# XuanHuang0/VANeRF

Measured on AMD Instinct MI355X. Metric: rendered rays/sec (64 samples/ray) + PSNR vs ref, 512x334 view, higher is better.
Workload: dtype bf16x3 (bf16 MFMA on hi+lo split operands, f32 accumulate; per-sample outputs within 3.3e-5 of the f32 kernel); 1 GPU; configs/vanerf.json eval view 512x334, 64 coarse + 64 importance samples/ray, two-hand mesh 1558 verts / 3108 faces, 1 source view 256x256, random trained-like weights; rays=171008, parallelism=single

## Files before the change

### vanerf_amd/csrc/api.cpp

```cpp
#include <algorithm>
#include <cstddef>

#include <cstring>

#include "common.h"

namespace vanerf {
static thread_local std::string g_last_error;
void set_last_error(const char* msg) { g_last_error = msg ? msg : ""; }
}

using namespace vanerf;

extern "C" int vanerf_abi_version(void) { return VANERF_ABI_VERSION; }

extern "C" const char* vanerf_last_error(void) { return g_last_error.c_str(); }

extern "C" int vanerf_weights_pack(const VanerfWeightTable* w, int mode, VanerfWeights** out)
{
    return guarded([&] {
        if (!w || !out) throw_error("vanerf_weights_pack: null argument");
        if (mode != 0 && mode != 1) throw_error("vanerf_weights_pack: mode %d not supported (0 = fp32 MFMA, 1 = split-bf16 x3)", mode);
        const float* const* ptrs = reinterpret_cast<const float* const*>(w);
        constexpr size_t n_ptrs = offsetof(VanerfWeightTable, sigmoid_beta) / sizeof(const float*);
        for (size_t i = 0; i < n_ptrs; ++i)
            if (!ptrs[i]) throw_error("vanerf_weights_pack: weight pointer #%d is null", (int)i);
        std::vector<float> host, host_bwd, host_h, eff;
        LayerOffsets offs{};
        pack_weights_host(*w, host, offs, mode, mode == 0 ? &host_bwd : nullptr, mode == 1 ? &host_h : nullptr, mode == 1 ? &eff : nullptr);
        auto* h = new VanerfWeights();
        h->n_floats_bwd = host_bwd.size();
        h->n_floats = host.size();
        h->n_floats_h = host_h.size();
        h->offs = offs;
        h->mode = mode;
        h->beta = w->sigmoid_beta < 2e-3f ? 2e-3f : w->sigmoid_beta;
        hipError_t e = hipGetDevice(&h->device);
        if (e == hipSuccess) e = hipMalloc(&h->dev, (host.size() + host_h.size()) * sizeof(float));
        if (e == hipSuccess) e = hipMemcpy(h->dev, host.data(), host.size() * sizeof(float), hipMemcpyHostToDevice);
        if (e == hipSuccess && !host_h.empty()) e = hipMemcpy(h->dev + host.size(), host_h.data(), host_h.size() * sizeof(float), hipMemcpyHostToDevice);
        if (e == hipSuccess && !eff.empty()) e = hipMalloc(&h->dev_eff, eff.size() * sizeof(float));
        if (e == hipSuccess && !eff.empty()) e = hipMemcpy(h->dev_eff, eff.data(), eff.size() * sizeof(float), hipMemcpyHostToDevice);
        if (e == hipSuccess && !host_bwd.empty()) e = hipMalloc(&h->dev_bwd, host_bwd.size() * sizeof(float));
        if (e == hipSuccess && !host_bwd.empty()) e = hipMemcpy(h->dev_bwd, host_bwd.data(), host_bwd.size() * sizeof(float), hipMemcpyHostToDevice);
        if (e == hipSuccess) e = hipMalloc(&h->stats, sizeof(unsigned long long));
        if (e == hipSuccess) e = hipMemset(h->stats, 0, sizeof(unsigned long long));
        if (e == hipSuccess) e = hipMalloc(&h->dev_beta, sizeof(float));
        if (e == hipSuccess) e = hipMemcpy(h->dev_beta, &h->beta, sizeof(float), hipMemcpyHostToDevice);
        if (e != hipSuccess) {
            if (h->dev) (void)hipFree(h->dev);
            if (h->dev_bwd) (void)hipFree(h->dev_bwd);
            if (h->stats) (void)hipFree(h->stats);
            if (h->dev_beta) (void)hipFree(h->dev_beta);
            if (h->dev_eff) (void)hipFree(h->dev_eff);
            delete h;
            hip_check(e, "vanerf_weights_pack: device upload");
        }
        *out = h;
    });
}

extern "C" int vanerf_weights_free(VanerfWeights* w)
{
    return guarded([&] {
        if (!w) return;
        if (w->dev) HIP_CHECK(hipFree(w->dev));
        if (w->dev_bwd) HIP_CHECK(hipFree(w->dev_bwd));
        if (w->stats) HIP_CHECK(hipFree(w->stats));
        if (w->dev_beta) HIP_CHECK(hipFree(w->dev_beta));
        if (w->dev_eff) HIP_CHECK(hipFree(w->dev_eff));
        delete w;
    });
}

extern "C" int vanerf_weights_pack_host(const VanerfWeightTable* w, float* out, int64_t cap, int64_t* n_out, unsigned* offsets)
{
    return guarded([&] {
        if (!w || !n_out) throw_error("vanerf_weights_pack_host: null argument");
        std::vector<float> host;
        LayerOffsets offs{};
        pack_weights_host(*w, host, offs);
        *n_out = (int64_t)host.size();
        if (offsets) std::copy_n(offs.off, (size_t)NUM_LAYERS, offsets);
        if (out) {
            if (cap < (int64_t)host.size()) throw_error("vanerf_weights_pack_host: buffer too small");
            std::copy(host.begin(), host.end(), out);
        }
    });
}

extern "C" int vanerf_weights_stream_host(const VanerfWeightTable* w, int which, float* out, int64_t cap, int64_t* n_out)
{
    return guarded([&] {
        if (!w || !n_out) throw_error("vanerf_weights_stream_host: null argument");
        if (which < 0 || which > 3) throw_error("vanerf_weights_stream_host: which = %d (0 fp32, 1 bf16x3, 2 backward, 3 hoisted bf16x3)", which);
        std::vector<float> host, bwd, hoisted;
        LayerOffsets offs{};
        pack_weights_host(*w, host, offs, which == 1 ? 1 : 0, which == 2 ? &bwd : nullptr, which == 3 ? &hoisted : nullptr);
        const std::vector<float>& src = which == 2 ? bwd : which == 3 ? hoisted : host;
        *n_out = (int64_t)src.size();
        if (out) {
            if (cap < (int64_t)src.size()) throw_error("vanerf_weights_stream_host: buffer too small");
            std::memcpy(out, src.data(), src.size() * sizeof(float));
        }
    });
}

extern "C" int vanerf_weights_download(const VanerfWeights* w, int which, float* out, int64_t cap, int64_t* n_out)
{
    return guarded([&] {
        if (!w || !n_out) throw_error("vanerf_weights_download: null argument");
        if (which != 0 && which != 2 && which != 3) throw_error("vanerf_weights_download: which = %d (0 forward, 2 backward, 3 hoisted bf16x3)", which);
        const float* src = which == 2 ? w->dev_bwd : which == 3 ? (w->n_floats_h ? w->dev + w->n_floats : nullptr) : w->dev;
        const size_t n = which == 2 ? w->n_floats_bwd : which == 3 ? w->n_floats_h : w->n_floats;
        if (!src) throw_error("vanerf_weights_download: the handle carries no such stream");
        *n_out = (int64_t)n;
        if (out) {
            if (cap < (int64_t)n) throw_error("vanerf_weights_download: buffer too small");
            HIP_CHECK(hipDeviceSynchronize());
            HIP_CHECK(hipMemcpy(out, src, n * sizeof(float), hipMemcpyDeviceToHost));
        }
    });
}

extern "C" int vanerf_weights_short_groups(const VanerfWeights* w, uint64_t* count)
{
    return guarded([&] {
        if (!w || !count) throw_error("vanerf_weights_short_groups: null argument");
        unsigned long long v = 0;
        HIP_CHECK(hipMemcpy(&v, w->stats, sizeof v, hipMemcpyDeviceToHost));
        *count = v;
    });
}
```

### vanerf_amd/csrc/common.h

```cpp
#pragma once
#include <hip/hip_runtime.h>

#include <atomic>
#include <cstdarg>
#include <cstdio>
#include <stdexcept>
#include <string>
#include <vector>

#include "../../include/vanerf_hip.h"
#include "layer_spec.h"

namespace vanerf {

struct Error : std::runtime_error {
    int code;
    Error(int c, const std::string& m) : std::runtime_error(m), code(c) {}
};

[[noreturn]] inline void throw_error(const char* fmt, ...)
{
    char buf[512];
    va_list ap;
    va_start(ap, fmt);
    vsnprintf(buf, sizeof buf, fmt, ap);
    va_end(ap);
    throw Error(VANERF_EINVAL, buf);
}

inline void hip_check(hipError_t e, const char* what)
{
    if (e != hipSuccess) {
        char buf[512];
        snprintf(buf, sizeof buf, "%s: %s", what, hipGetErrorString(e));
        throw Error(VANERF_EHIP, buf);
    }
}
#define HIP_CHECK(x) ::vanerf::hip_check((x), #x)

void set_last_error(const char* msg);

template <class F>
int guarded(F&& fn) noexcept
{
    try {
        fn();
        return VANERF_OK;
    } catch (const Error& e) {
        set_last_error(e.what());
        return e.code;
    } catch (const std::bad_alloc&) {
        set_last_error("out of host memory");
        return VANERF_ENOMEM;
    } catch (const std::exception& e) {
        set_last_error(e.what());
        return VANERF_EINVAL;
    } catch (...) {
        set_last_error("unknown error");
        return VANERF_EINVAL;
    }
}

void pack_weights_host(const VanerfWeightTable& w, std::vector<float>& out, LayerOffsets& offs, int mode = 0, std::vector<float>* bwd = nullptr,
                       std::vector<float>* hoisted = nullptr, std::vector<float>* eff_out = nullptr);
unsigned eff_layer_offset(int l);
struct LayerSrc {
    const float* w;
    const float* g;
    const float* b;
    int nout, kin;
    unsigned eff;
};
void layer_sources(const VanerfWeightTable& w, LayerSrc out[NUM_LAYERS]);
struct PackTables {
    std::vector<int> fwd, bwd, fwd_b, fwd_bh;
    LayerOffsets offs{};
    unsigned n_eff = 0;
};
const PackTables& pack_tables();
int layer_slots(int layer, int* k_of_slot, int cap);

constexpr long long VIEWS_MAX_ITEMS = 0x7fffffffLL;
void check_camera_source(const char* who, const VanerfPassDesc& d);

}

struct VanerfWeights {
    float* dev = nullptr;
    size_t n_floats_h = 0;
    float* dev_bwd = nullptr;
    size_t n_floats_bwd = 0;
    size_t n_floats = 0;
    vanerf::LayerOffsets offs{};
    int mode = 0;
    float beta = 0.1f;
    float* dev_beta = nullptr;
    float* dev_eff = nullptr;
    int device = 0;
    unsigned long long* stats = nullptr;
};
```

### vanerf_amd/csrc/layer_spec.h

```cpp
#pragma once

namespace vanerf {

enum Layer {
    L_GEO_AT0_A = 0, L_GEO_AT0_B, L_GEO_ATED0_A, L_GEO_ATED0_B,
    L_GEO_AT1_A, L_GEO_AT1_B, L_GEO_ATED1_A, L_GEO_ATED1_B,
    L_MLP0, L_MLP1, L_MLP2, L_MLP3, L_HEAD0, L_HEAD1, L_HEAD2, L_IBR,
    L_TEX_AT_A, L_TEX_AT_B, L_TEX_A, L_TEX_B, NUM_LAYERS
};

constexpr int kNB[NUM_LAYERS] = {1, 1, 2, 2, 1, 1, 1, 1, 4, 4, 4, 2, 2, 2, 1, 1, 3, 1, 3, 1};
constexpr int kT[NUM_LAYERS] = {
    98, 6, 98, 32,
    14, 6, 14, 4,
    147 + 32 + 1,
    64 + 1,
    64 + 4 + 1,
    60 + 1,
    64 + 1, 32 + 1, 32 + 1,
    64 + 1,
    49, 48, 49, 48
};

constexpr int PE_KPT_PER_HALF = 21;
constexpr int PE_FEATS = 7;

struct LayerOffsets {
    unsigned off[NUM_LAYERS];
};

constexpr unsigned layer_floats(int l) { return (unsigned)kT[l] * 64u * (unsigned)kNB[l]; }

constexpr unsigned layer_offset(int l)
{
    unsigned o = 0;
    for (int i = 0; i < l; ++i) o += layer_floats(i);
    return o;
}

constexpr int kT_b(int l, bool hoist)
{
    if (hoist && (l == L_GEO_AT0_A || l == L_GEO_ATED0_A)) return 32 + 2;
    if (hoist && l == L_TEX_AT_A) return 6 + 12 + 2;
    return kT[l];
}
constexpr int steps_b(int l, bool hoist = false) { return (kT_b(l, hoist) + 7) / 8; }
constexpr unsigned layer_dwords_b(int l, bool hoist = false) { return (unsigned)steps_b(l, hoist) * (unsigned)kNB[l] * 2u * 64u * 4u; }
constexpr unsigned layer_offset_b(int l, bool hoist = false)
{
    unsigned o = 0;
    for (int i = 0; i < l; ++i) o += layer_dwords_b(i, hoist);
    return o;
}

constexpr unsigned VP_NV = 1558u;
constexpr unsigned VP_A0_ROW = 16u, VP_N0_ROW = 64u, VP_P_ROW = 96u;
constexpr unsigned VP_A0 = 0u, VP_N0 = VP_A0 + VP_NV * VP_A0_ROW, VP_T0 = VP_N0 + VP_NV * VP_N0_ROW, VP_P = VP_T0 + VP_NV * VP_N0_ROW;
constexpr unsigned VP_FLOATS = VP_P + VP_NV * VP_P_ROW;

constexpr int kNOUT[NUM_LAYERS] = {10, 3, 64, 64, 10, 3, 8, 8, 128, 128, 120, 64, 64, 64, 2, 24, 96, 6, 96, 3};
constexpr int x_row_base(int l) { int o = 0; for (int i = 0; i < l; ++i) o += 2 * kT[i]; return o; }
constexpr int y_row_base(int l) { int o = 0; for (int i = 0; i < l; ++i) o += kNOUT[i]; return o; }
constexpr int X_ROWS = x_row_base(NUM_LAYERS), Y_ROWS = y_row_base(NUM_LAYERS);
constexpr int kBT[NUM_LAYERS] = {6, 3, 32, 32, 6, 3, 4, 4, 64, 64, 60, 32, 32, 32, 2, 12, 48, 4, 48, 3};
constexpr int kBLO[NUM_LAYERS] = {0, 0, 0, 0, 0, 0, 0, 0, 9, 0, 0, 0, 0, 0, 0, 0, 0, 0, 0, 0};
constexpr int kBNB[NUM_LAYERS] = {6, 1, 6, 2, 1, 1, 1, 1, 3, 4, 5, 4, 4, 2, 2, 4, 3, 3, 3, 3};
constexpr int bwd_pass_blocks(int l, int p) { return kBNB[l] - 4 * p > 4 ? 4 : kBNB[l] - 4 * p; }
constexpr unsigned bwd_layer_floats(int l) { return (unsigned)kBT[l] * 64u * (unsigned)kBNB[l]; }
constexpr unsigned bwd_layer_offset(int l) { unsigned o = 0; for (int i = 0; i < l; ++i) o += bwd_layer_floats(i); return o; }
constexpr unsigned bwd_pass_offset(int l, int p) { return bwd_layer_offset(l) + (unsigned)kBT[l] * 64u * 4u * (unsigned)p; }
enum AuxRow {
    AUX_G0 = 0,
    AUX_G1 = 3,
    AUX_TEX = 6,
    AUX_PW = 10,
    AUX_XV = 11,
    AUX_LAT = 43,
    AUX_COUNT = 55
};
constexpr int AUX_ROWS = 2 * AUX_COUNT;
constexpr int IG_GEO0 = 0;
constexpr int IG_GEO1 = 3 * 64;
constexpr int IG_TEX = IG_GEO1 + 24;
constexpr int IG_TEX_XY = IG_TEX + 64;
constexpr int IG_ROWS = IG_TEX_XY + 8;

}
```

### vanerf_amd/csrc/query_kernel.hip

```cpp
#include <algorithm>
#include <utility>

#include "common.h"
#include "mfma_chain.h"

using namespace vanerf;
using namespace vanerf_chain;


namespace {

constexpr int WAVES_PER_SIMD = 2;
constexpr int WAVES_PER_SIMD_SPILL = 1;
template <int MODE> constexpr int WPB = MODE == 1 ? 8 : 4;


#ifdef VANERF_STAMPS
#define STAMP(k)                                                                                  \
    do {                                                                                          \
        unsigned long long t_;                                                                    \
        __builtin_amdgcn_sched_barrier(0);                                                        \
        asm volatile("s_memtime %0\n\ts_waitcnt lgkmcnt(0)" : "=s"(t_)::"memory");               \
        __builtin_amdgcn_sched_barrier(0);                                                        \
        phase_cycles[k] += t_ - t_prev;                                                           \
        t_prev = t_;                                                                              \
    } while (0)
constexpr int N_PHASES = 12;
#else
#define STAMP(k) do { } while (0)
#endif

struct QueryParams {
    VanerfFrame f;
    const float* w;
    unsigned wbytes;
    const float* pts;
    const float* qsdf;
    const uint8_t* qvis;
    const float* noise;
    const int32_t* knn_in;
    const int32_t* order;
    int raw;
    long long n;
    float* out;
    uint8_t* valid;
    unsigned long long* stamps;
    unsigned* queue;
    unsigned long long* short_groups;
    float wm1[4], hm1[4];
    const float* vp;
    float *xs, *aux;
    long long npad;
};

typedef __bf16 bf16x8 __attribute__((ext_vector_type(8)));
typedef __bf16 bf16x2 __attribute__((ext_vector_type(2)));

struct FragB { u32x4 hi, lo; };

constexpr int LDS_FIRST = L_IBR;
template <bool HOIST> constexpr unsigned RES_BASE_DW = layer_offset_b(LDS_FIRST, HOIST);
template <bool HOIST> constexpr unsigned RES_DW = layer_offset_b(NUM_LAYERS, HOIST) - layer_offset_b(LDS_FIRST, HOIST);
constexpr unsigned RING_PHASE_PIECES = 16u, RING_BYTES = 2u * RING_PHASE_PIECES * 1024u;
constexpr unsigned LDS_KPT = 0u, LDS_CTRL = 2u * PE_KPT_PER_HALF * 16u, LDS_LAT0 = 768u, LDS_RING = 1024u, LDS_RES = LDS_RING + RING_BYTES;
template <bool HOIST> constexpr unsigned DYN_LDS_BYTES = LDS_RES + RES_DW<HOIST> * 4u;
template <bool HOIST> constexpr unsigned RING_PIECES = RES_BASE_DW<HOIST> / 256u;
template <bool HOIST> constexpr unsigned RING_STREAM_PHASES = (RING_PIECES<HOIST> + RING_PHASE_PIECES - 1u) / RING_PHASE_PIECES;
template <bool HOIST> constexpr unsigned RING_PHASES = (RING_STREAM_PHASES<HOIST> + 1u) / 2u * 2u;
static_assert(WPB<1> == 8, "the ring's DMA schedule deals 2 pieces of a phase to each of 8 waves");
static_assert(RING_PHASES<false> * RING_PHASE_PIECES * 256u <= layer_offset_b(NUM_LAYERS), "the last phase's DMA must stay inside the stream");
static_assert(RING_PHASES<true> * RING_PHASE_PIECES * 256u <= layer_offset_b(NUM_LAYERS, true), "the last phase's DMA must stay inside the hoisted stream");
static_assert(LDS_CTRL + 8u + 2u * 4u * WPB<1> <= LDS_LAT0 && LDS_LAT0 + 128u <= LDS_RING, "control words / constant latent overlap their neighbours");
static_assert(DYN_LDS_BYTES<false> <= 160u * 1024u && DYN_LDS_BYTES<true> <= DYN_LDS_BYTES<false>, "key points + control words + ring + resident fragments must fit the CU's 160 KB");
extern __shared__ __attribute__((aligned(16))) u32x4 s_dyn[];
typedef __attribute__((address_space(3))) u32x4 lds_u32x4_t;
typedef __attribute__((address_space(3))) unsigned lds_u32_t;
struct LAddr {
    unsigned w[3];
    unsigned dma_lds, dma_src;
};
__device__ __forceinline__ LAddr make_laddr(int lane, unsigned wv_uniform = 0u)
{
    LAddr a;
    a.dma_lds = LDS_RING + wv_uniform * 2048u; a.dma_src = wv_uniform * 2048u;
    a.w[0] = (unsigned)lane * 16u;
    asm volatile("" : "+v"(a.w[0]));
    a.w[1] = a.w[0] + 0x10000u; a.w[2] = a.w[0] + 0x20000u;
    asm volatile("" : "+v"(a.w[1]), "+v"(a.w[2]));
    return a;
}
template <unsigned BYTE> __device__ __forceinline__ u32x4 lds_frag(const LAddr& a)
{
    return *reinterpret_cast<const lds_u32x4_t*>((size_t)(a.w[BYTE >> 16] + (BYTE & 0xffffu)));
}
__device__ __forceinline__ lds_u32_t* lds_ctrl() { return reinterpret_cast<lds_u32_t*>((size_t)LDS_CTRL); }
template <int NB> struct RingDepthB { static constexpr int value = NB == 1 ? 1 : 2; };
template <int NB> struct RingB { FragB b[RingDepthB<NB>::value]; };

template <unsigned P> __device__ __forceinline__ void ring_dma(WRsrc rs, const LAddr& la)
{
    constexpr unsigned lds_off = (P % 2u) * RING_PHASE_PIECES * 1024u, src_off = P * RING_PHASE_PIECES * 1024u;
    unsigned keep, soff;
    asm volatile("s_mov_b32 %0, m0\n\ts_add_u32 m0, %2, %4\n\ts_add_u32 %1, %3, %5\n\ts_nop 0\n\t"
                 "buffer_load_dwordx4 %6, %7, %1 offen lds\n\tbuffer_load_dwordx4 %6, %7, %1 offen offset:1024 lds\n\ts_mov_b32 m0, %0"
                 : "=&s"(keep), "=&s"(soff)
                 : "s"(la.dma_lds), "s"(la.dma_src), "i"(lds_off), "i"(src_off), "v"(la.w[0]), "s"(rs)
                 : "memory");
}
template <bool HOIST, unsigned P> __device__ __forceinline__ void phase_begin(WRsrc rs, const LAddr& la)
{
    constexpr unsigned RING_PHASES = ::RING_PHASES<HOIST>;
    if constexpr (P > 0) asm volatile("s_waitcnt vmcnt(0) lgkmcnt(0)\n\ts_barrier" ::: "memory");
    ring_dma<(P + 1u) % RING_PHASES>(rs, la);
}

template <bool HOIST> __device__ __forceinline__ void ring_close(WRsrc rs, const LAddr& la)
{
    if constexpr (RING_STREAM_PHASES<HOIST> % 2u == 1u) phase_begin<HOIST, RING_PHASES<HOIST> - 1u>(rs, la);
}

template <bool HOIST, bool RES, unsigned DW> __device__ __forceinline__ FragB wload_blk(WRsrc rs, const LAddr& la)
{
    constexpr unsigned RING_PHASES = ::RING_PHASES<HOIST>, RES_BASE_DW = ::RES_BASE_DW<HOIST>;
    static_assert(RES == (DW >= RES_BASE_DW), "a layer's fragments are either resident or streamed through the ring: nothing is fetched per wave");
    FragB r;
    if constexpr (RES) {
        r.hi = lds_frag<LDS_RES + (DW - RES_BASE_DW) * 4u>(la);
        r.lo = lds_frag<LDS_RES + (DW - RES_BASE_DW + 256u) * 4u>(la);
    } else {
        constexpr unsigned q = DW / 256u;
        static_assert(q % 2u == 0 && q + 1u < RING_PHASES * RING_PHASE_PIECES, "block fragments are two consecutive pieces inside the streamed part");
        if constexpr (q % RING_PHASE_PIECES == 0) phase_begin<HOIST, q / RING_PHASE_PIECES>(rs, la);
        r.hi = lds_frag<LDS_RING + (q % (2u * RING_PHASE_PIECES)) * 1024u>(la);
        r.lo = lds_frag<LDS_RING + ((q + 1u) % (2u * RING_PHASE_PIECES)) * 1024u>(la);
    }
    return r;
}

template <bool HOIST, int NB, int T, bool RES, unsigned SBASE_DW> __device__ __forceinline__ RingB<NB> ring_start_b(WRsrc rs, const LAddr& la)
{
    constexpr int D = RingDepthB<NB>::value, S = (T + 7) / 8;
    RingB<NB> r;
    static_for<D>([&](auto ic) {
        constexpr int i = decltype(ic)::value;
        if constexpr (i < S * NB) r.b[i] = wload_blk<HOIST, RES, SBASE_DW + i * 512u>(rs, la);
    });
    __builtin_amdgcn_sched_barrier(0x000F);
    return r;
}

__device__ __forceinline__ unsigned pack_bf16(float a, float b)
{
    const bf16x2 v = {(__bf16)a, (__bf16)b};
    return __builtin_bit_cast(unsigned, v);
}

struct NoPre { template <class C> __device__ __forceinline__ void operator()(C) const {} };

template <bool HOIST, int NB, int T, bool RES, unsigned SBASE_DW, class Op, class Pre = NoPre>
__device__ __forceinline__ void run_layer_b(f32x16 (&acc)[NB], RingB<NB>& ring, WRsrc rs, const LAddr& la, Op&& operand,
                                            Pre&& pre = Pre{})
{
    constexpr int D = RingDepthB<NB>::value, S = (T + 7) / 8;
    constexpr int NCH = 4;
    auto split_pair = [&](auto sc, auto ic, u32x4& bh, u32x4& bl) {
        constexpr int s = decltype(sc)::value, i = decltype(ic)::value, t0 = 8 * s + 2 * i;
        float x0 = 0.0f, x1 = 0.0f;
        if constexpr (t0 < T) x0 = operand(std::integral_constant<int, t0>{});
        if constexpr (t0 + 1 < T) x1 = operand(std::integral_constant<int, t0 + 1>{});
        unsigned hpk = pack_bf16(x0, x1);
        asm("" : "+v"(hpk));
        bh[i] = hpk;
        bl[i] = pack_bf16(x0 - __uint_as_float(hpk << 16), x1 - __uint_as_float(hpk & 0xffff0000u));
    };
    u32x4 bh, bl;
    pre(std::integral_constant<int, 0>{});
    static_for<4>([&](auto ic) { split_pair(std::integral_constant<int, 0>{}, ic, bh, bl); });
    __builtin_amdgcn_sched_barrier(0);
    static_for<S>([&](auto sc) {
        constexpr int s = decltype(sc)::value;
        FragB a[NB];
        const bf16x8 xh = __builtin_bit_cast(bf16x8, bh), xl = __builtin_bit_cast(bf16x8, bl);
        u32x4 nh = {}, nl = {};
        static_for<NCH>([&](auto cc) {
            constexpr int c = decltype(cc)::value;
            static_for<3 * NB>([&](auto mc) {
                constexpr int m = decltype(mc)::value, ob = m / 3, pr = m % 3, idx = s * NB + ob;
                if constexpr (m * NCH / (3 * NB) == c) {
                    if constexpr (pr == 0) {
                        a[ob] = ring.b[idx % D];
                        if constexpr (idx + D < S * NB) ring.b[idx % D] = wload_blk<HOIST, RES, SBASE_DW + (idx + D) * 512u>(rs, la);
                    }
                    const bf16x8 wh = __builtin_bit_cast(bf16x8, a[ob].hi), wl = __builtin_bit_cast(bf16x8, a[ob].lo);
                    acc[ob] = __builtin_amdgcn_mfma_f32_32x32x16_bf16(pr == 2 ? wl : wh, pr == 1 ? xl : xh, acc[ob], 0, 0, 0);
                }
            });
            if constexpr (s + 1 < S) {
                if constexpr (c == 0) pre(std::integral_constant<int, s + 1>{});
                split_pair(std::integral_constant<int, s + 1>{}, cc, nh, nl);
            }
            __builtin_amdgcn_sched_barrier(0);
        });
        bh = nh; bl = nl;
    });
}

template <int MODE, int NB> struct RingSel { using type = Ring<NB>; };
template <int NB> struct RingSel<1, NB> { using type = RingB<NB>; };

struct LLane {
    int lane;
    WRsrc xs, aux;
    unsigned voff, row4;
    bool on;
};
constexpr unsigned SPILL_OFF = 0xfffffff0u;
template <int L, int t> __device__ __forceinline__ void spill_x(const LLane& la, float v)
{
    if (la.on) __builtin_amdgcn_raw_buffer_store_b32(__float_as_uint(v), la.xs, la.voff, (unsigned)(x_row_base(L) + 2 * t) * la.row4, 0);
}
template <int K> __device__ __forceinline__ void spill_aux(const LLane& la, float v)
{
    if (la.on) __builtin_amdgcn_raw_buffer_store_b32(__float_as_uint(v), la.aux, la.voff, (unsigned)(2 * K) * la.row4, 0);
}
template <int MODE> struct LaneSel { using type = LLane; };
template <> struct LaneSel<1> { using type = LAddr; };
__device__ __forceinline__ unsigned lane_of(const LLane& la) { return (unsigned)la.lane; }
template <int MODE, bool HOIST, int NB, int T, int L> __device__ __forceinline__ typename RingSel<MODE, NB>::type ring_start_m(WRsrc rs, const typename LaneSel<MODE>::type& la)
{
    if constexpr (MODE == 0) return ring_start<NB, T>(rs, layer_offset(L), lane_of(la) * NB * 4u);
    else return ring_start_b<HOIST, NB, T, (L >= LDS_FIRST), layer_offset_b(L, HOIST)>(rs, la);
}

template <int MODE, bool HOIST, int NB, int T, int L, class Op>
__device__ __forceinline__ void run_layer_m(f32x16 (&acc)[NB], typename RingSel<MODE, NB>::type& ring, WRsrc rs, const typename LaneSel<MODE>::type& la, Op&& operand)
{
    if constexpr (MODE == 0)
        run_layer<NB, T>(acc, ring, rs, layer_offset(L), lane_of(la) * NB * 4u, [&](auto tc) -> float {
            const float b = operand(tc);
            spill_x<L, decltype(tc)::value>(la, b);
            return b;
        });
    else run_layer_b<HOIST, NB, T, (L >= LDS_FIRST), layer_offset_b(L, HOIST)>(acc, ring, rs, la, static_cast<Op&&>(operand));
}

__device__ __forceinline__ int lane_id_fresh()
{
    int l;
    asm volatile("v_mbcnt_lo_u32_b32 %0, -1, 0\n\tv_mbcnt_hi_u32_b32 %0, -1, %0" : "=v"(l));
    return l;
}


__device__ __forceinline__ void block_barrier_lds() { asm volatile("s_waitcnt lgkmcnt(0)\n\ts_barrier" ::: "memory"); }

__device__ __forceinline__ float sigmoid_f(float x) { return __builtin_amdgcn_rcpf(1.0f + __builtin_amdgcn_exp2f(x * -1.44269504f)); }

__device__ __forceinline__ float relu_f(float x) { return __builtin_amdgcn_fmed3f(x, 0.0f, 3.0e38f); }

__device__ __forceinline__ float softplus100(float x)
{
    const float e = __builtin_amdgcn_exp2f(fabsf(x) * -144.269504f);
    return fmaf(__builtin_amdgcn_logf(1.0f + e), 6.93147181e-3f, relu_f(x));
}

template <int NB> __device__ __forceinline__ void relu(f32x16 (&a)[NB])
{
#pragma unroll
    for (int ob = 0; ob < NB; ++ob)
#pragma unroll
        for (int r = 0; r < 16; ++r) a[ob][r] = relu_f(a[ob][r]);
}

template <int NB> __device__ __forceinline__ void softplus(f32x16 (&a)[NB])
{
#pragma unroll
    for (int ob = 0; ob < NB; ++ob)
#pragma unroll
        for (int r = 0; r < 16; ++r) a[ob][r] = softplus100(a[ob][r]);
}

enum Act { ACT_RELU = 1, ACT_SOFTPLUS = 2 };
template <int MODE, int ACT> __device__ __forceinline__ float lazy_act(float v)
{
    if constexpr (MODE == 0) return v;
    else if constexpr (ACT == ACT_RELU) return relu_f(v);
    else return softplus100(v);
}

struct Bilin {
    int o00, o01, o10, o11;
    float w00, w01, w10, w11;
};

__device__ __forceinline__ Bilin bilin_setup(float x, float y, int H, int W, float wm1, float hm1)
{
    float ix = ((x + 1.0f) / 2.0f) * wm1;
    float iy = ((y + 1.0f) / 2.0f) * hm1;
    ix = fminf(wm1, fmaxf(ix, 0.0f));
    iy = fminf(hm1, fmaxf(iy, 0.0f));
    float fx = floorf(ix), fy = floorf(iy);
    float wx1 = ix - fx, wx0 = (fx + 1.0f) - ix;
    float wy1 = iy - fy, wy0 = (fy + 1.0f) - iy;
    int x0 = (int)fx, y0 = (int)fy;
    int x1 = min(x0 + 1, W - 1), y1 = min(y0 + 1, H - 1);
    Bilin b;
    b.o00 = y0 * W + x0; b.o01 = y0 * W + x1; b.o10 = y1 * W + x0; b.o11 = y1 * W + x1;
    b.w00 = wx0 * wy0; b.w01 = wx1 * wy0; b.w10 = wx0 * wy1; b.w11 = wx1 * wy1;
    return b;
}

__device__ __forceinline__ float bilin_mix(const Bilin& b, float v00, float v01, float v10, float v11)
{
    return ((v00 * b.w00 + v01 * b.w01) + v10 * b.w10) + v11 * b.w11;
}

template <class T> __device__ __forceinline__ T ld_off(const void* __restrict__ base, unsigned byte_off)
{
    return *reinterpret_cast<const T*>(reinterpret_cast<const char*>(base) + byte_off);
}

template <int C4> __device__ __forceinline__ void gather(const float* __restrict__ map, const Bilin& b, int C, int coff, float (&dst)[C4 * 4])
{
    const unsigned o00 = (unsigned)(b.o00 * C + coff) * 4u, o01 = (unsigned)(b.o01 * C + coff) * 4u, o10 = (unsigned)(b.o10 * C + coff) * 4u,
                   o11 = (unsigned)(b.o11 * C + coff) * 4u;
#pragma unroll
    for (int i = 0; i < C4; ++i) {
        const float4 a = ld_off<float4>(map, o00 + 16 * i), c = ld_off<float4>(map, o01 + 16 * i), d = ld_off<float4>(map, o10 + 16 * i),
                     e = ld_off<float4>(map, o11 + 16 * i);
        dst[4 * i + 0] = bilin_mix(b, a.x, c.x, d.x, e.x);
        dst[4 * i + 1] = bilin_mix(b, a.y, c.y, d.y, e.y);
        dst[4 * i + 2] = bilin_mix(b, a.z, c.z, d.z, e.z);
        dst[4 * i + 3] = bilin_mix(b, a.w, c.w, d.w, e.w);
    }
}

template <int C4> __device__ __forceinline__ void load_row(const float* __restrict__ table, unsigned elem_off, float (&dst)[C4 * 4])
{
#pragma unroll
    for (int i = 0; i < C4; ++i) {
        const float4 a = ld_off<float4>(table, elem_off * 4u + 16 * i);
        dst[4 * i] = a.x; dst[4 * i + 1] = a.y; dst[4 * i + 2] = a.z; dst[4 * i + 3] = a.w;
    }
}

struct Projected { float x, y, zn, mask; };
__device__ __forceinline__ Projected project_and_mask(const VanerfFrame& F, float wm1, float hm1, float px, float py, float pz)
{
    const float vx = fmaf(pz, F.KRT[2], fmaf(py, F.KRT[1], px * F.KRT[0])) + F.KRT[3];
    const float vy = fmaf(pz, F.KRT[6], fmaf(py, F.KRT[5], px * F.KRT[4])) + F.KRT[7];
    const float vz = fmaf(pz, F.KRT[10], fmaf(py, F.KRT[9], px * F.KRT[8])) + F.KRT[11];
    Projected r;
    r.x = 2.0f * ((vx / vz) / (F.width - 1.0f)) - 1.0f;
    r.y = 2.0f * ((vy / vz) / (F.height - 1.0f)) - 1.0f;
    r.zn = 2.0f * (vz - F.znear) / (F.zfar - F.znear) - 1.0f;
    const float eps = 1e-2f;
    const bool in_img = (r.x >= -1.0f - eps) && (r.x <= 1.0f + eps) && (r.y >= -1.0f - eps) && (r.y <= 1.0f + eps) && (r.zn >= -1.0f);
    const Bilin bi = bilin_setup(r.x, r.y, F.hi, F.wi, wm1, hm1);
    const float fg = bilin_mix(bi, ld_off<float>(F.mask, 4u * bi.o00), ld_off<float>(F.mask, 4u * bi.o01), ld_off<float>(F.mask, 4u * bi.o10),
                               ld_off<float>(F.mask, 4u * bi.o11));
    r.mask = (in_img && fg > 0.1f) ? 1.0f : 0.0f;
    return r;
}

template <int MODE, bool HOIST, int HC, int NBO, int NREG_MID, int l_at_a>
__device__ __forceinline__ void geo_scale(WRsrc W, int lane, const typename LaneSel<MODE>::type& la, typename RingSel<MODE, 1>::type& ring_at,
                                          float (&pix)[HC], float (&nn)[HC], float (&tw)[HC], float s0, float s1,
                                          f32x16 (&outacc)[NBO])
{
    constexpr int TIN = 3 * HC + 2;
    constexpr int TOUT = (NBO - 1) * 16 + NREG_MID;
    auto input = [&](auto tc) -> float {
        constexpr int t = decltype(tc)::value;
        if constexpr (t < HC) return pix[t];
        else if constexpr (t < 2 * HC) return nn[t - HC];
        else if constexpr (t < 3 * HC) return tw[t - 2 * HC];
        else if constexpr (t == 3 * HC) return s0;
        else return s1;
    };
    f32x16 at[1];
    zero<1>(at);
    run_layer_m<MODE, HOIST, 1, TIN, l_at_a>(at, ring_at, W, la, input);
    auto r_gate = ring_start_m<MODE, HOIST, 1, 6, l_at_a + 1>(W, la);
    auto r_mid = ring_start_m<MODE, HOIST, NBO, TIN, l_at_a + 2>(W, la);
    if constexpr (MODE == 0) relu<1>(at);
    f32x16 gate[1];
    zero<1>(gate);
    run_layer_m<MODE, HOIST, 1, 6, l_at_a + 1>(gate, r_gate, W, la, [&](auto tc) -> float { return lazy_act<MODE, ACT_RELU>(at[0][decltype(tc)::value]); });
    const float a0 = __shfl(sigmoid_f(gate[0][0]), lane & 31);
    const float a1 = __shfl(sigmoid_f(gate[0][1]), lane & 31);
    const float a2 = __shfl(sigmoid_f(gate[0][2]), lane & 31);
    if constexpr (MODE == 0) { constexpr int A = HC == 32 ? AUX_G0 : AUX_G1; spill_aux<A>(la, a0); spill_aux<A + 1>(la, a1); spill_aux<A + 2>(la, a2); }
#pragma unroll
    for (int t = 0; t < HC; ++t) { pix[t] *= a0; nn[t] *= a1; tw[t] *= a2; }
    f32x16 mid[NBO];
    zero<NBO>(mid);
    run_layer_m<MODE, HOIST, NBO, TIN, l_at_a + 2>(mid, r_mid, W, la, input);
    auto r_out = ring_start_m<MODE, HOIST, NBO, TOUT, l_at_a + 3>(W, la);
    if constexpr (MODE == 0) relu<NBO>(mid);
    zero<NBO>(outacc);
    run_layer_m<MODE, HOIST, NBO, TOUT, l_at_a + 3>(outacc, r_out, W, la,
                         [&](auto tc) -> float { constexpr int t = decltype(tc)::value; return lazy_act<MODE, ACT_RELU>(mid[t / 16][t % 16]); });
}

template <int MODE>
__device__ __forceinline__ void geo_scale0_vp(WRsrc W, int lane, const typename LaneSel<MODE>::type& la, typename RingSel<MODE, 1>::type& ring_at,
                                              float (&pix)[32], const float (&a0s)[8], const float (&n0)[32], const float (&t0)[32], float s0, float s1,
                                              f32x16 (&outacc)[2])
{
    constexpr int TIN = 32 + 2;
    auto input = [&](auto tc) -> float {
        constexpr int t = decltype(tc)::value;
        if constexpr (t < 32) return pix[t];
        else if constexpr (t == 32) return s0;
        else return s1;
    };
    f32x16 at[1];
    zero<1>(at);
#pragma unroll
    for (int r = 0; r < 8; ++r) at[0][r] = a0s[r];
    run_layer_m<MODE, true, 1, TIN, L_GEO_AT0_A>(at, ring_at, W, la, input);
    auto r_gate = ring_start_m<MODE, true, 1, 6, L_GEO_AT0_B>(W, la);
    auto r_mid = ring_start_m<MODE, true, 2, TIN, L_GEO_ATED0_A>(W, la);
    f32x16 gate[1];
    zero<1>(gate);
    run_layer_m<MODE, true, 1, 6, L_GEO_AT0_B>(gate, r_gate, W, la, [&](auto tc) -> float { return lazy_act<MODE, ACT_RELU>(at[0][decltype(tc)::value]); });
    const float a0 = __shfl(sigmoid_f(gate[0][0]), lane & 31);
    const float a1 = __shfl(sigmoid_f(gate[0][1]), lane & 31);
    const float a2 = __shfl(sigmoid_f(gate[0][2]), lane & 31);
    f32x16 mid[2];
#pragma unroll
    for (int t = 0; t < 32; ++t) { pix[t] *= a0; mid[t / 16][t % 16] = fmaf(a2, t0[t], a1 * n0[t]); }
    run_layer_m<MODE, true, 2, TIN, L_GEO_ATED0_A>(mid, r_mid, W, la, input);
    auto r_out = ring_start_m<MODE, true, 2, 32, L_GEO_ATED0_B>(W, la);
    zero<2>(outacc);
    run_layer_m<MODE, true, 2, 32, L_GEO_ATED0_B>(outacc, r_out, W, la,
                         [&](auto tc) -> float { constexpr int t = decltype(tc)::value; return lazy_act<MODE, ACT_RELU>(mid[t / 16][t % 16]); });
}

template <int NB> __device__ __forceinline__ void load_acc(const float* __restrict__ table, unsigned elem_off, f32x16 (&acc)[NB])
{
#pragma unroll
    for (int ob = 0; ob < NB; ++ob)
#pragma unroll
        for (int i = 0; i < 4; ++i) {
            const float4 a = ld_off<float4>(table, (elem_off + 16u * ob + 4u * i) * 4u);
            acc[ob][4 * i] = a.x; acc[ob][4 * i + 1] = a.y; acc[ob][4 * i + 2] = a.z; acc[ob][4 * i + 3] = a.w;
        }
}

template <int MODE, bool SPILL = false, bool HOIST = false>
__global__ __launch_bounds__(64 * WPB<MODE>, SPILL ? WAVES_PER_SIMD_SPILL : WAVES_PER_SIMD) void query_kernel(const QueryParams P)
{
    static_assert(!SPILL || MODE == 0, "the training spill runs on the fp32 kernel");
    static_assert(!HOIST || MODE == 1, "only the split-bf16 kernel has a hoisted variant");
    [[maybe_unused]] constexpr unsigned RES_BASE_DW = ::RES_BASE_DW<HOIST>, RES_DW = ::RES_DW<HOIST>;
    constexpr int T_GEO0 = kT_b(L_GEO_AT0_A, HOIST), T_TEX_AT = kT_b(L_TEX_AT_A, HOIST);
    constexpr int WAVES_PER_BLOCK = WPB<MODE>, BLOCK = 64 * WAVES_PER_BLOCK;

    const int lane_k = threadIdx.x & 63;
    [[maybe_unused]] const int lane = lane_k, j = lane & 31;
    [[maybe_unused]] const long long wave = (long long)blockIdx.x * WAVES_PER_BLOCK + (threadIdx.x >> 6);
    const long long ngroups = (P.n + 31) / 32;
    const VanerfFrame& F = P.f;
    const WRsrc W = __builtin_amdgcn_make_buffer_rsrc(const_cast<float*>(P.w), 0, P.wbytes, 0x00020000);
    [[maybe_unused]] WRsrc xs_rs = W, aux_rs = W;
    if constexpr (SPILL) {
        xs_rs = __builtin_amdgcn_make_buffer_rsrc(P.xs, 0, (unsigned)(X_ROWS * 4ll * P.npad), 0x00020000);
        aux_rs = __builtin_amdgcn_make_buffer_rsrc(P.aux, 0, (unsigned)(AUX_ROWS * 4ll * P.npad), 0x00020000);
    }

#ifdef VANERF_STAMPS
    unsigned long long phase_cycles[N_PHASES] = {};
    unsigned long long t_prev, rt0;
    asm volatile("s_memrealtime %0\n\ts_waitcnt lgkmcnt(0)" : "=s"(rt0)::"memory");
    asm volatile("s_memtime %0\n\ts_waitcnt lgkmcnt(0)" : "=s"(t_prev)::"memory");
#endif
    if constexpr (MODE == 1) {
        if (threadIdx.x < 2 * PE_KPT_PER_HALF) s_dyn[LDS_KPT / 16 + threadIdx.x] = reinterpret_cast<const u32x4*>(F.kpt_cam)[threadIdx.x];
    }
    unsigned short_groups = 0;
    struct SampleIn { float px, py, pz, sdf; int knn; unsigned char vis; };
    auto fetch = [&](unsigned grp, int j) {
        const long long sr = (long long)grp * 32 + j;
        long long sc = sr < P.n ? sr : P.n - 1;
        if (P.order) sc = P.order[sc];
        SampleIn in;
        in.px = P.pts[3 * sc]; in.py = P.pts[3 * sc + 1]; in.pz = P.pts[3 * sc + 2];
        in.sdf = P.qsdf[sc]; in.knn = P.knn_in[sc]; in.vis = P.qvis[sc];
        return in;
    };
    __shared__ unsigned s_ctrl0[MODE == 0 ? 2 + 2 * WAVES_PER_BLOCK : 1];
    auto s_base = [&](unsigned i) -> auto& { if constexpr (MODE == 0) return s_ctrl0[i]; else return lds_ctrl()[i]; };
    auto s_valid = [&](unsigned pp, unsigned k) -> auto& { if constexpr (MODE == 0) return s_ctrl0[2 + pp * WAVES_PER_BLOCK + k]; else return lds_ctrl()[2 + pp * WAVES_PER_BLOCK + k]; };
    const unsigned wv = threadIdx.x >> 6;
    [[maybe_unused]] const unsigned wv_u = (unsigned)__builtin_amdgcn_readfirstlane((int)wv);
    unsigned pending = 0, par = 1;
    if (threadIdx.x == 0) s_base(0) = atomicAdd(P.queue, (unsigned)WAVES_PER_BLOCK);
    if constexpr (MODE == 1) {
        const u32x4* __restrict__ src = reinterpret_cast<const u32x4*>(P.w) + RES_BASE_DW / 4;
        for (unsigned i = threadIdx.x; i < RES_DW / 4; i += BLOCK) s_dyn[LDS_RES / 16 + i] = src[i];
        const LAddr la0 = make_laddr(lane, wv_u);
        ring_dma<0>(W, la0);
        asm volatile("s_waitcnt vmcnt(0)" ::: "memory");
    }
    __syncthreads();
    if constexpr (MODE == 1) {
        if (wv_u == 0u) {
            const LAddr la0 = make_laddr(lane, wv_u);
            auto r0 = ring_start_m<MODE, HOIST, 1, 65, L_IBR>(W, la0);
            f32x16 lat0[1];
            zero<1>(lat0);
            const float one0 = (lane >> 5) ? 0.0f : 1.0f;
            run_layer_m<MODE, HOIST, 1, 65, L_IBR>(lat0, r0, W, la0, [&](auto tc) -> float { return decltype(tc)::value < 64 ? 0.0f : one0; });
            if ((lane & 31) == 0)
                static_for<16>([&](auto rc) { constexpr int r = decltype(rc)::value; reinterpret_cast<lds_u32_t*>((size_t)LDS_LAT0)[(lane >> 5) * 16 + r] = __float_as_uint(lat0[0][r]); });
        }
        __syncthreads();
    }
    unsigned base_cur = s_base(0);
    if (threadIdx.x == 0) pending = atomicAdd(P.queue, (unsigned)WAVES_PER_BLOCK);
    SampleIn in_next = fetch(base_cur + wv, j);
    while (base_cur < (unsigned)ngroups) {
        const long long g = (long long)base_cur + wv;
        const SampleIn in = in_next;
        const int lane = MODE == 1 ? lane_id_fresh() : lane_k, j = lane & 31, h = lane >> 5;
        const float one_h0 = h ? 0.0f : 1.0f;
        typename LaneSel<MODE>::type la;
        [[maybe_unused]] unsigned kp_lds = 0;
        if constexpr (MODE == 1) { la = make_laddr(lane, wv_u); kp_lds = LDS_KPT + ((la.w[0] >> 9) & 1u) * (PE_KPT_PER_HALF * 16u); }
        else {
            la.lane = lane; la.voff = SPILL_OFF; la.row4 = 0; la.on = SPILL;
            if constexpr (SPILL) {
                la.xs = xs_rs; la.aux = aux_rs;
                unsigned r4 = (unsigned)P.npad * 4u;
                asm volatile("" : "+s"(r4));
                la.row4 = r4;
                if (g < ngroups) la.voff = 4u * ((unsigned)g * 32u + (unsigned)j) + (unsigned)h * r4;
            }
        }
        const long long s_raw = g * 32 + j;
        const bool live = s_raw < P.n;
        long long s = live ? s_raw : P.n - 1;
        if (P.order) s = P.order[s];
        const float px = in.px, py = in.py, pz = in.pz;
        const float q_sdf = in.sdf;
        const float q_vis = in.vis ? 1.0f : 0.0f;

        const Projected pr = project_and_mask(F, P.wm1[0], P.hm1[0], px, py, pz);
        const float x = pr.x, y = pr.y, zn = pr.zn, mask = pr.mask;
        const bool wave_valid = __builtin_amdgcn_ballot_w64(mask > 0.0f) != 0ull;
        if (lane == 0) s_valid(par, wv) = wave_valid ? 1u : 0u;
        if (threadIdx.x == 0) s_base(par) = pending;
        block_barrier_lds();
        const unsigned base_next = (unsigned)__builtin_amdgcn_readfirstlane((int)s_base(par));
        unsigned anyv = 0;
#pragma unroll
        for (int k = 0; k < WAVES_PER_BLOCK; ++k) anyv |= s_valid(par, k);
        const bool any_valid = SPILL || __builtin_amdgcn_readfirstlane((int)anyv) != 0;
        par ^= 1u;
        if (threadIdx.x == 0) pending = atomicAdd(P.queue, (unsigned)WAVES_PER_BLOCK);
        in_next = fetch(base_next + wv, j);
        base_cur = base_next;
        __builtin_amdgcn_sched_barrier(0x000F);
        const Bilin bi = bilin_setup(x, y, F.hi, F.wi, P.wm1[0], P.hm1[0]);
        float pw;
        {
            float ux = 0.5f * x + 0.5f, uy = 0.5f * y + 0.5f, uz = 0.5f * zn + 0.5f;
            float dx = fminf(ux, 1.0f - ux), dy = fminf(uy, 1.0f - uy), dz = fminf(uz, 1.0f - uz);
            float wx = sigmoid_f(5.0f * (dx * 10.0f - 1.0f)), wy = sigmoid_f(5.0f * (dy * 10.0f - 1.0f)),
                  wz = sigmoid_f(5.0f * (dz * 10.0f - 1.0f));
            float p = (wx * wy) * wz * mask;
            pw = p / (p + 1e-6f);
        }
        if constexpr (MODE == 0) spill_aux<AUX_PW>(la, pw);

        STAMP(0);
        const int nn_idx = in.knn;
        const int tw_idx = nn_idx >= VANERF_NV_HAND ? nn_idx - VANERF_NV_HAND : nn_idx + VANERF_NV_HAND;
        const float vis_nn = ld_off<float>(F.vert_vis, 4u * nn_idx), vis_tw = ld_off<float>(F.vert_vis, 4u * tw_idx);
        const float sc0 = h ? q_vis : q_sdf;
        const float sc1 = h ? vis_tw : vis_nn;

        STAMP(1);
        [[maybe_unused]] const unsigned v4 = (unsigned)lane * 16u;
        auto chain = [&](auto& src, auto tc, auto nsteps) -> float {
            constexpr int t = decltype(tc)::value;
            if constexpr (t < decltype(nsteps)::value) return src[t / 16][t % 16];
            else return one_h0;
        };
        auto chain_sp = [&](auto& src, auto tc, auto nsteps) -> float {
            constexpr int t = decltype(tc)::value;
            if constexpr (t < decltype(nsteps)::value) return lazy_act<MODE, ACT_SOFTPLUS>(src[t / 16][t % 16]);
            else return one_h0;
        };
        float row[32];
        float qi[4], qt[8];
        auto tex_gathers = [&]() {
            load_row<8>(F.vfeat_tex, (unsigned)((h ? tw_idx : nn_idx) * 32), row);
            gather<1>(F.img, bi, 4, 0, qi);
            const Bilin bt = bilin_setup(x, y, F.ht, F.wt, P.wm1[1], P.hm1[1]);
            gather<2>(F.tex, bt, 8, 0, qt);
        };
        f32x16 pool[4];
        f32x16 head[1];
        if (any_valid) {
            auto r_at0 = ring_start_m<MODE, HOIST, 1, T_GEO0, L_GEO_AT0_A>(W, la);
            f32x16 g64[2], g8[1];
            float pix8[4], nn8[4], tw8[4];
            {
                float pix[32], nn[32], tw[32];
                const Bilin b0 = bilin_setup(x, y, F.h0, F.w0, P.wm1[2], P.hm1[2]);
                gather<8>(F.geo0, b0, 64, 32 * h, pix);
                [[maybe_unused]] float a0s[8];
                if constexpr (HOIST) {
                    load_row<2>(P.vp + VP_A0, (unsigned)(nn_idx * (int)VP_A0_ROW + 8 * h), a0s);
                    load_row<8>(P.vp + VP_N0, (unsigned)(nn_idx * (int)VP_N0_ROW + 32 * h), nn);
                    load_row<8>(P.vp + VP_T0, (unsigned)(nn_idx * (int)VP_N0_ROW + 32 * h), tw);
                } else {
                    load_row<8>(F.vfeat0, (unsigned)(nn_idx * 64 + 32 * h), nn);
                    load_row<8>(F.vfeat0, (unsigned)(tw_idx * 64 + 32 * h), tw);
                }
                auto geo1_gathers = [&]() {
                    const Bilin b1 = bilin_setup(x, y, F.h1, F.w1, P.wm1[3], P.hm1[3]);
                    gather<1>(F.geo1, b1, 8, 4 * h, pix8);
                    load_row<1>(F.vfeat1, (unsigned)(nn_idx * 8 + 4 * h), nn8);
                    load_row<1>(F.vfeat1, (unsigned)(tw_idx * 8 + 4 * h), tw8);
                };
                if constexpr (MODE == 0) geo1_gathers();
                STAMP(2);
                if constexpr (HOIST) geo_scale0_vp<MODE>(W, lane, la, r_at0, pix, a0s, nn, tw, sc0, sc1, g64);
                else geo_scale<MODE, HOIST, 32, 2, 16, L_GEO_AT0_A>(W, lane, la, r_at0, pix, nn, tw, sc0, sc1, g64);
                if constexpr (MODE == 1) geo1_gathers();
                STAMP(3);
            }
            constexpr unsigned base0 = layer_offset(L_MLP0);
            constexpr int D0 = PE_FEATS;
            WFrag<4> ring0[D0];
            RingB<4> ring0b;
            {
                auto r_at1 = ring_start_m<MODE, HOIST, 1, 14, L_GEO_AT1_A>(W, la);
                if constexpr (MODE == 0) {
                    static_for<D0>([&](auto fc) { constexpr int f = decltype(fc)::value; ring0[f] = wload<4>(W, (base0 + f * 256) * 4u, v4); });
                }
                geo_scale<MODE, HOIST, 4, 1, 4, L_GEO_AT1_A>(W, lane, la, r_at1, pix8, nn8, tw8, sc0, sc1, g8);
                if constexpr (MODE == 1) ring0b = ring_start_b<HOIST, 4, 180, false, layer_offset_b(L_MLP0, HOIST)>(W, la);
                STAMP(4);
            }


            f32x16 xv[2];
            {
                f32x16 a0[4];
                zero<4>(a0);
                {
                    float cx = fmaf(pz, F.extrin[2], fmaf(py, F.extrin[1], px * F.extrin[0])) + F.extrin[3];
                    float cy = fmaf(pz, F.extrin[6], fmaf(py, F.extrin[5], px * F.extrin[4])) + F.extrin[7];
                    float cz = fmaf(pz, F.extrin[10], fmaf(py, F.extrin[9], px * F.extrin[8])) + F.extrin[11];
                    const float4* __restrict__ kpg = reinterpret_cast<const float4*>(F.kpt_cam);
                    auto pe_features = [&](int i, float (&feat)[PE_FEATS]) {
                        float kx, ky, kz;
                        if constexpr (MODE == 1) {
                            const u32x4 k = *reinterpret_cast<const lds_u32x4_t*>((size_t)(kp_lds + 16u * i));
                            kx = __uint_as_float(k.x); ky = __uint_as_float(k.y); kz = __uint_as_float(k.z);
                        } else {
                            const float4 k0 = kpg[i], k1 = kpg[PE_KPT_PER_HALF + i];
                            kx = h ? k1.x : k0.x; ky = h ? k1.y : k0.y; kz = h ? k1.z : k0.z;
                        }
                        const float ddx = cx - kx, ddy = cy - ky, ddz = cz - kz;
                        const float d2 = (ddx * ddx + ddy * ddy) + ddz * ddz;
                        const float wk = __expf(-d2 * F.pe_inv_2sigma2);
                        const float dz = F.pe_scale * ddz;
                        const float s0 = __builtin_amdgcn_sinf(0.5f * dz), c0 = __builtin_amdgcn_cosf(0.5f * dz);
                        const float s1 = __builtin_amdgcn_sinf(dz), c1 = __builtin_amdgcn_cosf(dz);
                        const float s2 = __builtin_amdgcn_sinf(2.0f * dz), c2 = __builtin_amdgcn_cosf(2.0f * dz);
                        feat[0] = dz * wk; feat[1] = s0 * wk; feat[2] = c0 * wk; feat[3] = s1 * wk; feat[4] = c1 * wk;
                        feat[5] = s2 * wk; feat[6] = c2 * wk;
                    };
                    if constexpr (MODE == 0) {
                        static_for<PE_KPT_PER_HALF>([&](auto ic) {
                            constexpr int i = decltype(ic)::value;
                            float feat[PE_FEATS];
                            pe_features(i, feat);
                            static_for<D0>([&](auto fc) {
                                constexpr int f = decltype(fc)::value;
                                const WFrag<4> a = ring0[f];
                                ring0[f] = wload<4>(W, (base0 + ((i + 1) * D0 + f) * 256) * 4u, v4);
                                spill_x<L_MLP0, i * D0 + f>(la, feat[f]);
                                mfma_step<4>(a0, a, feat[f]);
                            });
                        });
                        constexpr unsigned nextp = base0 + (PE_KPT_PER_HALF + 1) * D0 * 256;
                        constexpr int TREM = 33;
                        static_for<TREM>([&](auto tc) {
                            constexpr int t = decltype(tc)::value;
                            const float b = chain(g64, tc, std::integral_constant<int, 32>{});
                            const WFrag<4> a = ring0[t % D0];
                            if constexpr (t + D0 < TREM) ring0[t % D0] = wload<4>(W, (nextp + t * 256) * 4u, v4);
                            spill_x<L_MLP0, PE_KPT_PER_HALF * D0 + t>(la, b);
                            mfma_step<4>(a0, a, b);
                        });
                    } else {
                        float feat[PE_KPT_PER_HALF][PE_FEATS];
                        run_layer_b<HOIST, 4, 180, false, layer_offset_b(L_MLP0, HOIST)>(a0, ring0b, W, la,
                            [&](auto tc) -> float {
                                constexpr int t = decltype(tc)::value;
                                if constexpr (t < 147) return feat[t / 7][t % 7];
                                else return chain(g64, std::integral_constant<int, t - 147>{}, std::integral_constant<int, 32>{});
                            },
                            [&](auto sc) {
                                constexpr int s_ = decltype(sc)::value;
                                constexpr int lo_k = s_ == 0 ? 0 : (8 * s_ - 1) / 7 + 1, hi_k = (8 * s_ + 7) / 7;
                                static_for<(hi_k < PE_KPT_PER_HALF ? hi_k : PE_KPT_PER_HALF - 1) - lo_k + 1 < 0 ? 0 : (hi_k < PE_KPT_PER_HALF ? hi_k : PE_KPT_PER_HALF - 1) - lo_k + 1>([&](auto dc) {
                                    constexpr int i = lo_k + decltype(dc)::value;
                                    pe_features(i, feat[i]);
                                });
                            });
                    }
                }
                STAMP(5);
                auto r1 = ring_start_m<MODE, HOIST, 4, 65, L_MLP1>(W, la);
                if constexpr (MODE == 0) softplus<4>(a0);
                f32x16 a1[4];
                zero<4>(a1);
                run_layer_m<MODE, HOIST, 4, 65, L_MLP1>(a1, r1, W, la, [&](auto tc) -> float { return chain_sp(a0, tc, std::integral_constant<int, 64>{}); });
                auto r2 = ring_start_m<MODE, HOIST, 4, 69, L_MLP2>(W, la);
                if constexpr (MODE == 0) softplus<4>(a1);
                zero<4>(a0);
                run_layer_m<MODE, HOIST, 4, 69, L_MLP2>(a0, r2, W, la, [&](auto tc) -> float {
                    constexpr int t = decltype(tc)::value;
                    if constexpr (t < 64) return lazy_act<MODE, ACT_SOFTPLUS>(a1[t / 16][t % 16]);
                    else if constexpr (t < 68) return g8[0][t - 64];
                    else return one_h0;
                });
                auto r3 = ring_start_m<MODE, HOIST, 2, 61, L_MLP3>(W, la);
                if constexpr (MODE == 0) softplus<4>(a0);
                zero<2>(xv);
                run_layer_m<MODE, HOIST, 2, 61, L_MLP3>(xv, r3, W, la, [&](auto tc) -> float { return chain_sp(a0, tc, std::integral_constant<int, 60>{}); });
            }
            STAMP(6);
            if constexpr (MODE == 0) tex_gathers();
            auto rh0 = ring_start_m<MODE, HOIST, 2, 65, L_HEAD0>(W, la);
            if constexpr (MODE == 0)
                static_for<32>([&](auto rc) { constexpr int r = decltype(rc)::value; spill_aux<AUX_XV + r>(la, xv[r / 16][r % 16]); });
    #pragma unroll
            for (int b = 0; b < 2; ++b)
    #pragma unroll
                for (int r = 0; r < 16; ++r) {
                    float m = pw * xv[b][r];
                    float d = xv[b][r] - m;
                    pool[b][r] = m;
                    pool[2 + b][r] = pw * (d * d);
                }
            {
                f32x16 m0[2], m1[2];
                zero<2>(m0);
                run_layer_m<MODE, HOIST, 2, 65, L_HEAD0>(m0, rh0, W, la, [&](auto tc) -> float { return chain(pool, tc, std::integral_constant<int, 64>{}); });
                auto rh1 = ring_start_m<MODE, HOIST, 2, 33, L_HEAD1>(W, la);
                if constexpr (MODE == 0) softplus<2>(m0);
                zero<2>(m1);
                run_layer_m<MODE, HOIST, 2, 33, L_HEAD1>(m1, rh1, W, la, [&](auto tc) -> float { return chain_sp(m0, tc, std::integral_constant<int, 32>{}); });
                auto rh2 = ring_start_m<MODE, HOIST, 1, 33, L_HEAD2>(W, la);
                if constexpr (MODE == 0) softplus<2>(m1);
                zero<1>(head);
                run_layer_m<MODE, HOIST, 1, 33, L_HEAD2>(head, rh2, W, la, [&](auto tc) -> float { return chain_sp(m1, tc, std::integral_constant<int, 32>{}); });
                static_assert(LDS_FIRST == L_HEAD2 + 1, "the ring is closed behind its last streamed layer");
                if constexpr (MODE == 1) ring_close<HOIST>(W, la);
            }
        } else {
            if constexpr (MODE == 0) tex_gathers();
            zero<4>(pool);
            zero<1>(head);
        }
        if (!wave_valid && lane == 0 && g < ngroups) ++short_groups;
        if constexpr (MODE == 1) tex_gathers();
        STAMP(7);
        f32x16 lat[1];
        typename RingSel<MODE, 3>::type r_ta;
        if (MODE == 1 && !any_valid) {
            r_ta = ring_start_m<MODE, HOIST, 3, T_TEX_AT, L_TEX_AT_A>(W, la);
            if constexpr (MODE == 1)
                static_for<16>([&](auto rc) { constexpr int r = decltype(rc)::value; lat[0][r] = __uint_as_float(reinterpret_cast<const lds_u32_t*>((size_t)LDS_LAT0)[h * 16 + r]); });
        } else {
            auto r_ibr = ring_start_m<MODE, HOIST, 1, 65, L_IBR>(W, la);
            r_ta = ring_start_m<MODE, HOIST, 3, T_TEX_AT, L_TEX_AT_A>(W, la);
            zero<1>(lat);
            run_layer_m<MODE, HOIST, 1, 65, L_IBR>(lat, r_ibr, W, la, [&](auto tc) -> float { return chain(pool, tc, std::integral_constant<int, 64>{}); });
        }
        STAMP(8);
        f32x16 rgb[1];
        {
            float q[6];
            q[0] = h ? qt[3] : qi[0]; q[1] = h ? qt[4] : qi[1]; q[2] = h ? qt[5] : qi[2];
            q[3] = h ? qt[6] : qt[0]; q[4] = h ? qt[7] : qt[1]; q[5] = h ? 0.0f : qt[2];
            const float t0 = h ? vis_nn : q_vis;
            const float t1 = h ? 0.0f : vis_tw;
            f32x16 latg = lat[0];
            auto tex_in = [&](auto tc) -> float {
                constexpr int t = decltype(tc)::value;
                if constexpr (t < 29) return row[t];
                else if constexpr (t < 35) return q[t - 29];
                else if constexpr (t < 47) return latg[t - 35];
                else if constexpr (t == 47) return t0;
                else return t1;
            };
            auto from_ta = [&](auto& ta_) { return [&](auto tc) -> float { constexpr int t = decltype(tc)::value; return lazy_act<MODE, ACT_RELU>(ta_[t / 16][t % 16]); }; };
            auto tex_at_in = [&](auto tc) -> float {
                constexpr int t = decltype(tc)::value;
                if constexpr (!HOIST) return tex_in(tc);
                else if constexpr (t < 6) return q[t];
                else if constexpr (t < 18) return latg[t - 6];
                else if constexpr (t == 18) return t0;
                else return t1;
            };
            f32x16 ta[3];
            if constexpr (HOIST) load_acc<3>(P.vp + VP_P, (unsigned)(nn_idx * (int)VP_P_ROW + 48 * h), ta);
            else zero<3>(ta);
            run_layer_m<MODE, HOIST, 3, T_TEX_AT, L_TEX_AT_A>(ta, r_ta, W, la, tex_at_in);
            auto r_tg = ring_start_m<MODE, HOIST, 1, 48, L_TEX_AT_B>(W, la);
            if constexpr (MODE == 0) relu<3>(ta);
            f32x16 tg[1];
            zero<1>(tg);
            run_layer_m<MODE, HOIST, 1, 48, L_TEX_AT_B>(tg, r_tg, W, la, from_ta(ta));
            auto r_tb = ring_start_m<MODE, HOIST, 3, 49, L_TEX_A>(W, la);
            float m0 = sigmoid_f(tg[0][0]), m1 = sigmoid_f(tg[0][1]), m2 = sigmoid_f(tg[0][2]), m3 = sigmoid_f(tg[0][3]);
            float o0 = __shfl_xor(m0, 32), o1 = __shfl_xor(m1, 32), o2 = __shfl_xor(m2, 32);
            const float gq = h ? o0 : m0;
            const float g11 = h ? o2 : m1;
            const float ggf = h ? m0 : m3;
            const float glat = h ? m1 : o1;
            if constexpr (MODE == 0) {
                spill_aux<AUX_TEX>(la, gq); spill_aux<AUX_TEX + 1>(la, g11); spill_aux<AUX_TEX + 2>(la, ggf); spill_aux<AUX_TEX + 3>(la, glat);
                static_for<12>([&](auto rc) { constexpr int r = decltype(rc)::value; spill_aux<AUX_LAT + r>(la, lat[0][r]); });
            }
#pragma unroll
            for (int t = 0; t < 11; ++t) row[t] *= g11;
#pragma unroll
            for (int t = 11; t < 29; ++t) row[t] *= ggf;
#pragma unroll
            for (int t = 0; t < 6; ++t) q[t] *= gq;
#pragma unroll
            for (int r = 0; r < 12; ++r) latg[r] = lat[0][r] * glat;
            zero<3>(ta);
            run_layer_m<MODE, HOIST, 3, 49, L_TEX_A>(ta, r_tb, W, la, tex_in);
            auto r_rgb = ring_start_m<MODE, HOIST, 1, 48, L_TEX_B>(W, la);
            if constexpr (MODE == 0) relu<3>(ta);
            zero<1>(rgb);
            run_layer_m<MODE, HOIST, 1, 48, L_TEX_B>(rgb, r_rgb, W, la, from_ta(ta));
        }
        STAMP(9);
        if constexpr (MODE == 1) asm volatile("s_waitcnt vmcnt(0)" ::: "memory");
        if (live && h == 0) {
            float rad = head[0][1];
            if (P.noise) rad += P.noise[s];
            float* o = P.out + 5 * s;
            o[0] = P.raw ? head[0][0] : mask * fmaxf(rad, 0.0f);
            o[1] = P.raw ? head[0][1] : mask * head[0][0] + (1.0f - mask) * F.invalid_sdf;
            o[2] = rgb[0][0];
            o[3] = rgb[0][1];
            o[4] = rgb[0][2];
            if (P.valid) P.valid[s] = mask > 0.0f;
        }
        STAMP(10);
    }
    if (P.short_groups && (MODE == 1 ? lane_id_fresh() : lane) == 0 && short_groups) atomicAdd(P.short_groups, (unsigned long long)short_groups);
#ifdef VANERF_STAMPS
    unsigned long long rt1;
    asm volatile("s_memrealtime %0\n\ts_waitcnt lgkmcnt(0)" : "=s"(rt1)::"memory");
    phase_cycles[N_PHASES - 1] = rt1 - rt0;
    if (P.stamps && lane == 0)
        for (int k = 0; k < N_PHASES; ++k) P.stamps[wave * N_PHASES + k] = phase_cycles[k];
#endif
}

void check_queue_word(const char* who, const void* queue_word)
{
    if (!queue_word || (reinterpret_cast<uintptr_t>(queue_word) & 7u)) throw_error("%s: queue_word must be 8 bytes of device memory, 8-byte aligned", who);
}
void check_frame_pointers(const char* who, const VanerfFrame& f)
{
    if (!f.geo0 || !f.geo1 || !f.tex || !f.img || !f.mask || !f.verts || !f.vfeat0 || !f.vfeat1 || !f.vfeat_tex || !f.vert_vis || !f.kpt_cam)
        throw_error("%s: frame has a null pointer", who);
}

QueryParams query_params(const VanerfFrame& f, const float* stream_w, size_t stream_floats, const float* pts, const float* query_sdf,
                         const uint8_t* query_vis, const int32_t* knn_idx, int raw, int64_t n, float* out)
{
    QueryParams P = {};
    P.f = f; P.w = stream_w; P.wbytes = (unsigned)(stream_floats * sizeof(float));
    P.pts = pts; P.qsdf = query_sdf; P.qvis = query_vis; P.knn_in = knn_idx; P.raw = raw; P.n = n; P.out = out;
    const int ws[4] = {f.wi, f.wt, f.w0, f.w1}, hs[4] = {f.hi, f.ht, f.h0, f.h1};
    for (int i = 0; i < 4; ++i) { P.wm1[i] = (float)(ws[i] - 1); P.hm1[i] = (float)(hs[i] - 1); }
    return P;
}

struct QueryLaunch { void (*kernel)(QueryParams); int wpb, blocks_per_cu; unsigned lds_bytes; };
template <int MODE, bool SPILL = false, bool HOIST = false> QueryLaunch query_launch()
{
    return {query_kernel<MODE, SPILL, HOIST>, WPB<MODE>, (SPILL ? WAVES_PER_SIMD_SPILL : WAVES_PER_SIMD) * 4 / WPB<MODE>, MODE == 1 ? DYN_LDS_BYTES<HOIST> : 0u};
}

long long query_blocks(const QueryLaunch& L, int64_t n)
{
    const long long ngroups = (n + 31) / 32;
    int dev = 0, cus = 256;
    HIP_CHECK(hipGetDevice(&dev));
    HIP_CHECK(hipDeviceGetAttribute(&cus, hipDeviceAttributeMultiprocessorCount, dev));
    return std::min<long long>((ngroups + L.wpb - 1) / L.wpb, (long long)cus * L.blocks_per_cu);
}

void launch_query(const QueryLaunch& L, long long blocks, QueryParams& P, void* queue_word, void* stream)
{
    P.queue = static_cast<unsigned*>(queue_word);
    HIP_CHECK(hipMemsetAsync(P.queue, 0, 8, (hipStream_t)stream));
    if (L.lds_bytes) HIP_CHECK(hipFuncSetAttribute(reinterpret_cast<const void*>(L.kernel), hipFuncAttributeMaxDynamicSharedMemorySize, (int)L.lds_bytes));
    hipLaunchKernelGGL(L.kernel, dim3((unsigned)blocks), dim3(64 * L.wpb), L.lds_bytes, (hipStream_t)stream, P);
    HIP_CHECK(hipGetLastError());
}

}

extern "C" int vanerf_query_samples(const VanerfWeights* w, const VanerfFrame* frame, const float* pts, const float* query_sdf,
                                    const uint8_t* query_vis, const int32_t* knn_idx, const float* noise, const int32_t* order, int raw, int64_t n,
                                    float* out, uint8_t* valid, void* queue_word, const float* vertex_products, void* stream)
{
    return guarded([&] {
        if (n < 0) throw_error("vanerf_query_samples: n = %lld < 0", (long long)n);
        if (n == 0) return;
        if (!w || !w->dev || !frame || !pts || !query_sdf || !query_vis || !knn_idx || !out) throw_error("vanerf_query_samples: null argument");
        check_queue_word("vanerf_query_samples", queue_word);
        if ((n + 31) / 32 >= 0xffffff00LL) throw_error("vanerf_query_samples: n = %lld too large for one launch", (long long)n);
        const VanerfFrame& f = *frame;
        check_frame_pointers("vanerf_query_samples", f);
        if (f.h0 < 1 || f.w0 < 1 || f.h1 < 1 || f.w1 < 1 || f.ht < 1 || f.wt < 1 || f.hi < 1 || f.wi < 1)
            throw_error("vanerf_query_samples: feature-map sizes must be positive");
        const bool hoist = vertex_products != nullptr;
        if (hoist && (w->mode != 1 || !w->n_floats_h)) throw_error("vanerf_query_samples: a table of vertex products needs a bf16x3 weight handle");
        if (hoist && (reinterpret_cast<uintptr_t>(vertex_products) & 15u)) throw_error("vanerf_query_samples: the table must be 16-byte aligned");
        QueryParams P = query_params(f, hoist ? w->dev + w->n_floats : w->dev, hoist ? w->n_floats_h : w->n_floats, pts, query_sdf, query_vis, knn_idx, raw, n, out);
        P.noise = noise; P.order = order; P.valid = valid; P.short_groups = w->stats; P.vp = vertex_products;
        const QueryLaunch L = w->mode == 1 && hoist ? query_launch<1, false, true>() : w->mode == 1 ? query_launch<1>() : query_launch<0>();
        launch_query(L, query_blocks(L, n), P, queue_word, stream);
    });
}

extern "C" int vanerf_query_forward_spill(const VanerfWeights* w, const VanerfFrame* frame, const float* pts, const float* query_sdf,
                                          const uint8_t* query_vis, const int32_t* knn_idx, int64_t n, int64_t npad, float* out_raw, uint8_t* valid,
                                          float* xs, float* aux, void* queue_word, void* stream)
{
    return guarded([&] {
        if (n <= 0) throw_error("vanerf_query_forward_spill: n = %lld", (long long)n);
        if (!w || !w->dev || w->mode != 0) throw_error("vanerf_query_forward_spill: needs an fp32 weight handle (vanerf_weights_pack mode 0)");
        if (!frame || !pts || !query_sdf || !query_vis || !knn_idx || !out_raw || !xs || !aux) throw_error("vanerf_query_forward_spill: null argument");
        check_queue_word("vanerf_query_forward_spill", queue_word);
        if (npad < n || npad % 32 != 0) throw_error("vanerf_query_forward_spill: npad = %lld must be a multiple of 32 and >= n = %lld", (long long)npad, (long long)n);
        if ((long long)X_ROWS * 4 * npad >= (long long)SPILL_OFF)
            throw_error("vanerf_query_forward_spill: a block of %lld samples spills more than 4 GB (the kernels address the spills with 32-bit offsets): at most %lld",
                        (long long)npad, (long long)SPILL_OFF / (4 * X_ROWS) / 32 * 32);
        const VanerfFrame& f = *frame;
        check_frame_pointers("vanerf_query_forward_spill", f);
        QueryParams P = query_params(f, w->dev, w->n_floats, pts, query_sdf, query_vis, knn_idx, 1, n, out_raw);
        P.valid = valid; P.xs = xs; P.aux = aux; P.npad = npad;
        const QueryLaunch L = query_launch<0, true>();
        launch_query(L, query_blocks(L, n), P, queue_word, stream);
    });
}

constexpr int CP_BLOCK = 1024;

__global__ __launch_bounds__(CP_BLOCK) void order_count_kernel(const VanerfFrame F, float wm1, float hm1, const float* __restrict__ pts, long long n,
                                                               uint8_t* __restrict__ flags, unsigned* __restrict__ block_valid)
{
    const long long s = (long long)blockIdx.x * CP_BLOCK + threadIdx.x;
    int valid = 0;
    if (s < n) {
        valid = project_and_mask(F, wm1, hm1, pts[3 * s], pts[3 * s + 1], pts[3 * s + 2]).mask > 0.0f;
        flags[s] = (uint8_t)valid;
    }
    const int cnt = __syncthreads_count(valid);
    if (threadIdx.x == 0) block_valid[blockIdx.x] = (unsigned)cnt;
}

__global__ __launch_bounds__(CP_BLOCK) void order_scan_kernel(unsigned* __restrict__ block_valid, int nblocks)
{
    __shared__ unsigned s_sum[CP_BLOCK];
    const int per = (nblocks + CP_BLOCK - 1) / CP_BLOCK;
    const int b0 = threadIdx.x * per, b1 = min(b0 + per, nblocks);
    unsigned loc = 0;
    for (int b = b0; b < b1; ++b) loc += block_valid[b];
    s_sum[threadIdx.x] = loc;
    __syncthreads();
    for (int d = 1; d < CP_BLOCK; d <<= 1) {
        const unsigned v = threadIdx.x >= (unsigned)d ? s_sum[threadIdx.x - d] : 0u;
        __syncthreads();
        s_sum[threadIdx.x] += v;
        __syncthreads();
    }
    unsigned run = s_sum[threadIdx.x] - loc;
    for (int b = b0; b < b1; ++b) { const unsigned c = block_valid[b]; block_valid[b] = run; run += c; }
    if (threadIdx.x == CP_BLOCK - 1) block_valid[nblocks] = s_sum[CP_BLOCK - 1];
}

__global__ __launch_bounds__(CP_BLOCK) void order_scatter_kernel(const uint8_t* __restrict__ flags, long long n, const unsigned* __restrict__ block_off,
                                                                 int nblocks, int32_t* __restrict__ order)
{
    __shared__ unsigned s_wave[CP_BLOCK / 64];
    const long long s = (long long)blockIdx.x * CP_BLOCK + threadIdx.x;
    const int lane = threadIdx.x & 63, wv = threadIdx.x >> 6;
    const bool live = s < n;
    const bool valid = live && flags[s] != 0;
    const unsigned long long m = __ballot(valid);
    const unsigned below = (unsigned)__builtin_popcountll(m & ((1ull << lane) - 1ull));
    if (lane == 0) s_wave[wv] = (unsigned)__builtin_popcountll(m);
    __syncthreads();
    unsigned wbase = 0;
    for (int k = 0; k < wv; ++k) wbase += s_wave[k];
    if (!live) return;
    const unsigned rank_valid = wbase + below;
    const unsigned off_valid = block_off[blockIdx.x], total_valid = block_off[nblocks];
    const unsigned long long before = (unsigned long long)blockIdx.x * CP_BLOCK;
    const unsigned long long pos = valid ? (unsigned long long)off_valid + rank_valid
                                         : (unsigned long long)total_valid + (before - off_valid) + (threadIdx.x - rank_valid);
    order[pos] = (int32_t)s;
}

extern "C" int vanerf_query_order(const VanerfFrame* frame, const float* pts, int64_t n, int32_t* order, void* scratch, int64_t scratch_bytes,
                                  void* stream)
{
    return guarded([&] {
        if (n < 0) throw_error("vanerf_query_order: n = %lld < 0", (long long)n);
        if (n == 0) return;
        if (!frame || !pts || !order || !scratch) throw_error("vanerf_query_order: null argument");
        if (n >= 0x7fffffffLL) throw_error("vanerf_query_order: n = %lld does not fit a 32-bit index", (long long)n);
        const VanerfFrame& f = *frame;
        if (!f.mask || f.hi < 1 || f.wi < 1) throw_error("vanerf_query_order: frame has no mask");
        const int nblocks = (int)((n + CP_BLOCK - 1) / CP_BLOCK);
        const int64_t need = n + 4 * ((int64_t)nblocks + 1) + 16;
        if (scratch_bytes < need) throw_error("vanerf_query_order: scratch of %lld bytes, %lld needed (vanerf_query_order_scratch)", (long long)scratch_bytes, (long long)need);
        uint8_t* flags = static_cast<uint8_t*>(scratch);
        unsigned* block_off = reinterpret_cast<unsigned*>(flags + ((n + 15) / 16) * 16);
        const hipStream_t st = (hipStream_t)stream;
        hipLaunchKernelGGL(order_count_kernel, dim3(nblocks), dim3(CP_BLOCK), 0, st, f, (float)(f.wi - 1), (float)(f.hi - 1), pts, (long long)n, flags, block_off);
        hipLaunchKernelGGL(order_scan_kernel, dim3(1), dim3(CP_BLOCK), 0, st, block_off, nblocks);
        hipLaunchKernelGGL(order_scatter_kernel, dim3(nblocks), dim3(CP_BLOCK), 0, st, flags, (long long)n, block_off, nblocks, order);
        HIP_CHECK(hipGetLastError());
    });
}

extern "C" int64_t vanerf_query_order_scratch(int64_t n) { return n + 4 * ((n + CP_BLOCK - 1) / CP_BLOCK + 1) + 32; }

#ifdef VANERF_STAMPS
extern "C" int vanerf_debug_query_stamps(const VanerfWeights* w, const VanerfFrame* frame, const float* pts, const float* query_sdf,
                                         const uint8_t* query_vis, const int32_t* knn_idx, int64_t n, float* out, unsigned long long* stamps, int* n_waves, void* queue_word, void* stream)
{
    return guarded([&] {
        QueryParams P = query_params(*frame, w->dev, w->n_floats, pts, query_sdf, query_vis, knn_idx, 0, n, out);
        P.stamps = stamps;
        const QueryLaunch L = w->mode == 1 ? query_launch<1>() : query_launch<0>();
        const long long blocks = query_blocks(L, n);
        *n_waves = (int)blocks * L.wpb;
        if (stamps) launch_query(L, blocks, P, queue_word, stream);
    });
}
#endif
```

### vanerf_amd/csrc/weights_pack.cpp

```cpp
#include <hip/hip_runtime.h>

#include <cmath>
#include <cstring>
#include <utility>
#include <vector>

#include "common.h"
#include "layer_spec.h"

using namespace vanerf;

namespace {

constexpr int BIAS = -2;
constexpr int ZERO = -1;

using Pairs = std::vector<std::pair<int, int>>;

inline int row0(int reg) { return (reg & 3) + 8 * (reg >> 2); }

void chain(Pairs& p, int nb, int nregs_last, int base, int kin_limit)
{
    for (int ob = 0; ob < nb; ++ob) {
        int nr = (ob == nb - 1) ? nregs_last : 16;
        for (int r = 0; r < nr; ++r) {
            int k0 = ob * 32 + row0(r), k1 = k0 + 4;
            p.emplace_back(k0 < kin_limit ? base + k0 : ZERO, k1 < kin_limit ? base + k1 : ZERO);
        }
    }
}

void bias_pair(Pairs& p) { p.emplace_back(BIAS, ZERO); }

struct Mat {
    std::vector<float> w;
    std::vector<float> b;
    int nout, kin;
};

struct WordB { int id0, id1, part; };

struct Shape { int nout, kin, bias, wn; };
constexpr Shape kShape[NUM_LAYERS] = {
    {10, 196, 0, 0}, {3, 10, 0, 0}, {64, 196, 0, 0}, {64, 64, 0, 0}, {10, 28, 0, 0}, {3, 10, 0, 0}, {8, 28, 0, 0}, {8, 8, 0, 0},
    {128, 358, 1, 1}, {128, 128, 1, 1}, {120, 136, 1, 1}, {64, 120, 1, 0}, {64, 128, 1, 1}, {64, 64, 1, 1}, {2, 64, 1, 0}, {24, 128, 1, 0},
    {96, 96, 0, 0}, {6, 96, 0, 0}, {96, 96, 0, 0},
    {3, 96, 0, 0},
};
constexpr unsigned eff_offset(int l)
{
    unsigned o = 0;
    for (int i = 0; i < l; ++i) o += (unsigned)(kShape[i].nout * kShape[i].kin + (kShape[i].bias ? kShape[i].nout : 0));
    return o;
}
static_assert(eff_offset(NUM_LAYERS) < (1u << 24), "ids must be exact in fp32");

Mat id_matrix(int l)
{
    const Shape sh = kShape[l];
    if (sh.nout != kNOUT[l]) throw_error("internal: layer %d has %d outputs, spec says %d", l, sh.nout, kNOUT[l]);
    Mat m{std::vector<float>((size_t)sh.nout * sh.kin), {}, sh.nout, sh.kin};
    const unsigned base = eff_offset(l) + 1u;
    for (size_t i = 0; i < m.w.size(); ++i) m.w[i] = (float)(base + i);
    if (sh.bias) {
        m.b.resize(sh.nout);
        for (int o = 0; o < sh.nout; ++o) m.b[o] = (float)(base + m.w.size() + o);
    }
    return m;
}

void emit(std::vector<float>& out, int layer, const Mat& m, const Pairs& pairs)
{
    const int nb = kNB[layer], T = kT[layer];
    if ((int)pairs.size() != T) throw_error("internal: layer %d has %d k-pairs, spec says %d", layer, (int)pairs.size(), T);
    if (m.nout > nb * 32) throw_error("internal: layer %d: %d outputs do not fit %d blocks", layer, m.nout, nb);
    size_t base = out.size();
    out.resize(base + (size_t)T * 64 * nb, 0.0f);
    for (int t = 0; t < T; ++t)
        for (int lane = 0; lane < 64; ++lane) {
            int k = (lane >> 5) ? pairs[t].second : pairs[t].first;
            if (k == ZERO) continue;
            if (k != BIAS && (k < 0 || k >= m.kin)) throw_error("internal: layer %d k-index %d out of range", layer, k);
            for (int ob = 0; ob < nb; ++ob) {
                int o = ob * 32 + (lane & 31);
                if (o >= m.nout) continue;
                float v = (k == BIAS) ? (m.b.empty() ? 0.0f : m.b[o]) : m.w[(size_t)o * m.kin + k];
                out[base + ((size_t)t * 64 + lane) * nb + ob] = v;
            }
        }
}

void emit_b_ids(std::vector<WordB>& out, int layer, const Mat& m, const Pairs& pairs, bool hoist)
{
    const int nb = kNB[layer], T = kT_b(layer, hoist), S = steps_b(layer, hoist);
    if ((int)pairs.size() != T) throw_error("internal: layer %d has %d k-pairs, spec says %d", layer, (int)pairs.size(), T);
    size_t base = out.size();
    out.resize(base + layer_dwords_b(layer, hoist), WordB{0, 0, 0});
    WordB* dst = out.data() + base;
    for (int s = 0; s < S; ++s)
        for (int ob = 0; ob < nb; ++ob)
            for (int lane = 0; lane < 64; ++lane) {
                const int o = ob * 32 + (lane & 31);
                int id[8] = {};
                for (int j = 0; j < 8; ++j) {
                    const int t = 8 * s + j;
                    if (t >= T || o >= m.nout) continue;
                    const int k = (lane >> 5) ? pairs[t].second : pairs[t].first;
                    if (k == ZERO) continue;
                    id[j] = (int)((k == BIAS) ? (m.b.empty() ? 0.0f : m.b[o]) : m.w[(size_t)o * m.kin + k]);
                }
                for (int part = 0; part < 2; ++part) {
                    WordB* q = dst + ((((size_t)s * nb + ob) * 2 + part) * 64 + lane) * 4;
                    for (int i = 0; i < 4; ++i) q[i] = WordB{id[2 * i], id[2 * i + 1], part};
                }
            }
}

Pairs geo_input_pairs(int c, bool hoist = false)
{
    Pairs p;
    int hc = c / 2;
    for (int grp = 0; grp < (hoist ? 1 : 3); ++grp)
        for (int t = 0; t < hc; ++t) p.emplace_back(grp * c + t, grp * c + hc + t);
    p.emplace_back(3 * c + 0, 3 * c + 1);
    p.emplace_back(3 * c + 2, 3 * c + 3);
    return p;
}

Pairs tex_input_pairs(bool hoist = false)
{
    Pairs p;
    if (!hoist) {
        for (int t = 0; t < 11; ++t) p.emplace_back(11 + t, 22 + t);
        for (int t = 0; t < 18; ++t) p.emplace_back(33 + t, 51 + t);
    }
    for (int u = 0; u < 6; ++u) p.emplace_back(u, u < 5 ? 6 + u : ZERO);
    chain(p, 1, 12, 69, 24);
    p.emplace_back(93, 94);
    p.emplace_back(95, ZERO);
    return p;
}

}

namespace {

Pairs layer_pairs(int l, bool hoist = false)
{
    Pairs p;
    switch (l) {
    case L_GEO_AT0_A: case L_GEO_ATED0_A: return geo_input_pairs(64, hoist);
    case L_GEO_AT1_A: case L_GEO_ATED1_A: return geo_input_pairs(8);
    case L_GEO_AT0_B: case L_GEO_AT1_B: chain(p, 1, 6, 0, 10); return p;
    case L_GEO_ATED0_B: chain(p, 2, 16, 0, 64); return p;
    case L_GEO_ATED1_B: chain(p, 1, 4, 0, 8); return p;
    case L_MLP0:
        for (int i = 0; i < PE_KPT_PER_HALF; ++i)
            for (int f = 0; f < PE_FEATS; ++f) p.emplace_back(f * 42 + i, f * 42 + PE_KPT_PER_HALF + i);
        chain(p, 2, 16, 294, 64);
        bias_pair(p);
        return p;
    case L_MLP1: chain(p, 4, 16, 0, 128); bias_pair(p); return p;
    case L_MLP2: chain(p, 4, 16, 0, 128); chain(p, 1, 4, 128, 8); bias_pair(p); return p;
    case L_MLP3: chain(p, 4, 12, 0, 120); bias_pair(p); return p;
    case L_HEAD0: case L_IBR: chain(p, 2, 16, 0, 64); chain(p, 2, 16, 64, 64); bias_pair(p); return p;
    case L_HEAD1: case L_HEAD2: chain(p, 2, 16, 0, 64); bias_pair(p); return p;
    case L_TEX_AT_A: return tex_input_pairs(hoist);
    case L_TEX_A: return tex_input_pairs();
    case L_TEX_AT_B: case L_TEX_B: chain(p, 3, 16, 0, 96); return p;
    }
    throw_error("internal: no layer %d", l);
}

void sources(const VanerfWeightTable& w, vanerf::LayerSrc out[NUM_LAYERS])
{
    auto set = [&](int l, const float* ww, const float* g, const float* b) {
        const Shape sh = kShape[l];
        if (!ww || (sh.wn && !g) || (sh.bias && !b)) throw_error("weight table: a pointer of layer %d is null", l);
        out[l] = vanerf::LayerSrc{ww, sh.wn ? g : nullptr, sh.bias ? b : nullptr, sh.nout, sh.kin, eff_offset(l)};
    };
    set(L_GEO_AT0_A, w.geo_at0_w1, nullptr, nullptr);
    set(L_GEO_AT0_B, w.geo_at0_w2, nullptr, nullptr);
    set(L_GEO_ATED0_A, w.geo_ated0_w1, nullptr, nullptr);
    set(L_GEO_ATED0_B, w.geo_ated0_w2, nullptr, nullptr);
    set(L_GEO_AT1_A, w.geo_at1_w1, nullptr, nullptr);
    set(L_GEO_AT1_B, w.geo_at1_w2, nullptr, nullptr);
    set(L_GEO_ATED1_A, w.geo_ated1_w1, nullptr, nullptr);
    set(L_GEO_ATED1_B, w.geo_ated1_w2, nullptr, nullptr);
    set(L_MLP0, w.l1_v[0], w.l1_g[0], w.l1_b[0]);
    set(L_MLP1, w.l1_v[1], w.l1_g[1], w.l1_b[1]);
    set(L_MLP2, w.l1_v[2], w.l1_g[2], w.l1_b[2]);
    set(L_MLP3, w.l1_w3, nullptr, w.l1_b3);
    set(L_HEAD0, w.l2_v[0], w.l2_g[0], w.l2_b[0]);
    set(L_HEAD1, w.l2_v[1], w.l2_g[1], w.l2_b[1]);
    set(L_HEAD2, w.l2_w2, nullptr, w.l2_b2);
    set(L_IBR, w.ibr_w, nullptr, w.ibr_b);
    set(L_TEX_AT_A, w.tex_at_w1, nullptr, nullptr);
    set(L_TEX_AT_B, w.tex_at_w2, nullptr, nullptr);
    set(L_TEX_A, w.tex_w1, nullptr, nullptr);
    set(L_TEX_B, w.tex_w2, nullptr, nullptr);
}

void fold_host(const VanerfWeightTable& w, std::vector<float>& eff)
{
    vanerf::LayerSrc src[NUM_LAYERS];
    sources(w, src);
    eff.assign(eff_offset(NUM_LAYERS), 0.0f);
    for (int l = 0; l < NUM_LAYERS; ++l) {
        const vanerf::LayerSrc& s = src[l];
        float* e = eff.data() + s.eff;
        for (int o = 0; o < s.nout; ++o) {
            const float* v = s.w + (size_t)o * s.kin;
            if (s.g) {
                double sum = 0.0;
                for (int k = 0; k < s.kin; ++k) sum += (double)v[k] * (double)v[k];
                const float scale = s.g[o] / (float)std::sqrt(sum);
                for (int k = 0; k < s.kin; ++k) e[(size_t)o * s.kin + k] = v[k] * scale;
            } else {
                for (int k = 0; k < s.kin; ++k) e[(size_t)o * s.kin + k] = v[k];
            }
            if (s.b) e[(size_t)s.nout * s.kin + o] = s.b[o];
        }
    }
}

void emit_bwd(std::vector<float>& out, int layer, const Mat& m, const Pairs& pairs)
{
    const int T = kT[layer], BT = kBT[layer], nbt = kBNB[layer], blo = kBLO[layer];
    if (m.nout != kNOUT[layer]) throw_error("internal: layer %d has %d outputs, spec says %d", layer, m.nout, kNOUT[layer]);
    Pairs kk;
    chain(kk, (m.nout + 31) / 32, 16, 0, m.nout);
    for (int t = BT; t < (int)kk.size(); ++t)
        if (kk[t].first != ZERO || kk[t].second != ZERO) throw_error("internal: layer %d: output row beyond its %d backward k-pairs", layer, BT);
    const size_t base = out.size();
    if (base != bwd_layer_offset(layer)) throw_error("internal: backward stream of layer %d starts at %zu, spec says %u", layer, base, bwd_layer_offset(layer));
    out.resize(base + bwd_layer_floats(layer), 0.0f);
    for (int p = 0; 4 * p < nbt; ++p) {
        const int nb = bwd_pass_blocks(layer, p);
        float* dst = out.data() + bwd_pass_offset(layer, p);
        for (int t2 = 0; t2 < BT; ++t2)
            for (int lane = 0; lane < 64; ++lane) {
                const int o = (lane >> 5) ? kk[t2].second : kk[t2].first;
                if (o == ZERO) continue;
                const int jj = lane & 31, hs = (jj >> 2) & 1, reg = (jj & 3) + 4 * (jj >> 3);
                for (int ib = 0; ib < nb; ++ib) {
                    const int t = 16 * (blo + 4 * p + ib) + reg;
                    if (t >= T) continue;
                    const int c = hs ? pairs[t].second : pairs[t].first;
                    if (c < 0) continue;
                    dst[((size_t)t2 * 64 + lane) * nb + ib] = m.w[(size_t)o * m.kin + c];
                }
            }
    }
}

}

namespace vanerf {

inline unsigned short bf16_rne(float f)
{
    unsigned u;
    std::memcpy(&u, &f, 4);
    if ((u & 0x7fffffffu) > 0x7f800000u) return 0x7fc0;
    return (unsigned short)((u + 0x7fffu + ((u >> 16) & 1u)) >> 16);
}
inline float bf16_to_f32(unsigned short b)
{
    unsigned u = (unsigned)b << 16;
    float f;
    std::memcpy(&f, &u, 4);
    return f;
}
inline unsigned short bf16_part(float v, int part)
{
    const unsigned short hi = bf16_rne(v);
    return part ? bf16_rne(v - bf16_to_f32(hi)) : hi;
}

const PackTables& pack_tables()
{
    static const PackTables tables = [] {
        PackTables t;
        std::vector<float> fwd, bwd;
        std::vector<WordB> fwd_b, fwd_bh;
        for (int l = 0; l < NUM_LAYERS; ++l) {
            t.offs.off[l] = (unsigned)fwd.size();
            if (fwd.size() != layer_offset(l)) throw_error("internal: layer %d starts at %zu, layer_spec.h says %u", l, fwd.size(), layer_offset(l));
            if (fwd_b.size() != layer_offset_b(l)) throw_error("internal: layer %d (bf16x3) starts at %zu, layer_spec.h says %u", l, fwd_b.size(), layer_offset_b(l));
            const Mat m = id_matrix(l);
            const Pairs p = layer_pairs(l);
            emit(fwd, l, m, p);
            emit_b_ids(fwd_b, l, m, p, false);
            if (fwd_bh.size() != layer_offset_b(l, true)) throw_error("internal: layer %d (hoisted bf16x3) starts at %zu, layer_spec.h says %u", l, fwd_bh.size(), layer_offset_b(l, true));
            emit_b_ids(fwd_bh, l, m, layer_pairs(l, true), true);
            emit_bwd(bwd, l, m, p);
        }
        fwd.resize(fwd.size() + 2 * 64 * 4, 0.0f);
        bwd.resize(bwd.size() + 2 * 64 * 4, 0.0f);
        fwd_b.resize(fwd_b.size() + 2 * 64 * 4, WordB{0, 0, 0});
        fwd_bh.resize(fwd_bh.size() + 2 * 64 * 4, WordB{0, 0, 0});
        t.fwd.assign(fwd.begin(), fwd.end());
        t.bwd.assign(bwd.begin(), bwd.end());
        for (auto [src, dst] : {std::pair{&fwd_b, &t.fwd_b}, std::pair{&fwd_bh, &t.fwd_bh}}) {
            dst->resize(2 * src->size());
            for (size_t i = 0; i < src->size(); ++i) {
                (*dst)[2 * i] = (*src)[i].id0 | ((*src)[i].part << 30);
                (*dst)[2 * i + 1] = (*src)[i].id1;
            }
        }
        t.n_eff = eff_offset(NUM_LAYERS);
        for (const std::vector<int>* v : {&t.fwd, &t.bwd, &t.fwd_b, &t.fwd_bh})
            for (int id : *v)
                if ((id & 0x3fffffff) > (int)t.n_eff) throw_error("internal: placement id %d beyond the %u effective weights", id, t.n_eff);
        return t;
    }();
    return tables;
}

void layer_sources(const VanerfWeightTable& w, LayerSrc out[NUM_LAYERS]) { sources(w, out); }

unsigned eff_layer_offset(int l) { return eff_offset(l); }

void pack_weights_host(const VanerfWeightTable& w, std::vector<float>& out, LayerOffsets& offs, int mode, std::vector<float>* bwd, std::vector<float>* hoisted,
                       std::vector<float>* eff_out)
{
    const PackTables& t = pack_tables();
    std::vector<float> eff;
    fold_host(w, eff);
    auto value = [&](int id) { return id ? eff[(size_t)id - 1] : 0.0f; };
    for (int l = 0; l < NUM_LAYERS; ++l) offs.off[l] = mode ? layer_offset_b(l) : t.offs.off[l];
    auto place_b = [&](const std::vector<int>& tab, std::vector<float>& o) {
        const size_t n = tab.size() / 2;
        o.resize(n);
        unsigned* dst = reinterpret_cast<unsigned*>(o.data());
        for (size_t i = 0; i < n; ++i) {
            const int a = tab[2 * i], part = (a >> 30) & 1;
            dst[i] = (unsigned)bf16_part(value(a & 0x3fffffff), part) | ((unsigned)bf16_part(value(tab[2 * i + 1]), part) << 16);
        }
    };
    if (hoisted) place_b(t.fwd_bh, *hoisted);
    if (mode) {
        place_b(t.fwd_b, out);
    } else {
        out.resize(t.fwd.size());
        for (size_t i = 0; i < out.size(); ++i) out[i] = value(t.fwd[i]);
    }
    if (bwd) {
        bwd->resize(t.bwd.size());
        for (size_t i = 0; i < bwd->size(); ++i) (*bwd)[i] = value(t.bwd[i]);
    }
    if (eff_out) *eff_out = std::move(eff);
}

int layer_slots(int l, int* k_of_slot, int cap)
{
    if (l < 0 || l >= NUM_LAYERS) throw_error("vanerf_layer_slots: layer %d", l);
    const Pairs p = layer_pairs(l);
    if ((int)p.size() != kT[l]) throw_error("internal: layer %d has %d k-pairs, spec says %d", l, (int)p.size(), kT[l]);
    if (k_of_slot) {
        if (cap < 2 * kT[l]) throw_error("vanerf_layer_slots: room for %d slots, layer %d has %d", cap, l, 2 * kT[l]);
        for (int t = 0; t < kT[l]; ++t) { k_of_slot[2 * t] = p[t].first; k_of_slot[2 * t + 1] = p[t].second; }
    }
    return 2 * kT[l];
}

}
```

### vanerf_amd/csrc/weights_update.hip

```cpp
#include <hip/hip_runtime.h>

#include <mutex>

#include "common.h"

using namespace vanerf;

namespace {

struct FoldArgs {
    LayerSrc l[NUM_LAYERS];
};

__global__ __launch_bounds__(64) void fold_kernel(FoldArgs a, float* __restrict__ eff, const float* __restrict__ beta_src, float* __restrict__ beta_dst)
{
    const LayerSrc L = a.l[blockIdx.y];
    const int o = blockIdx.x;
    if (blockIdx.x == 0 && blockIdx.y == 0 && threadIdx.x == 0 && beta_src) beta_dst[0] = fmaxf(beta_src[0], 2e-3f);
    if (o >= L.nout) return;
    const float* v = L.w + (size_t)o * L.kin;
    float* e = eff + L.eff + (size_t)o * L.kin;
    __shared__ float s_scale;
    if (L.g) {
        if (threadIdx.x == 0) {
            double sum = 0.0;
            for (int k = 0; k < L.kin; ++k) sum += (double)v[k] * (double)v[k];
            s_scale = L.g[o] / (float)sqrt(sum);
        }
        __syncthreads();
        const float scale = s_scale;
        for (int k = threadIdx.x; k < L.kin; k += 64) e[k] = v[k] * scale;
    } else {
        for (int k = threadIdx.x; k < L.kin; k += 64) e[k] = v[k];
    }
    if (L.b && threadIdx.x == 0) eff[L.eff + (size_t)L.nout * L.kin + o] = L.b[o];
}

__global__ void place_f32_kernel(const int* __restrict__ tab, const float* __restrict__ eff, float* __restrict__ out, unsigned n)
{
    const unsigned i = blockIdx.x * blockDim.x + threadIdx.x;
    if (i >= n) return;
    const int id = tab[i];
    out[i] = id ? eff[id - 1] : 0.0f;
}

__device__ inline unsigned bf16_rne(float f)
{
    const unsigned u = __float_as_uint(f);
    if ((u & 0x7fffffffu) > 0x7f800000u) return 0x7fc0u;
    return (u + 0x7fffu + ((u >> 16) & 1u)) >> 16;
}
__device__ inline unsigned bf16_part(float v, int part)
{
    const unsigned hi = bf16_rne(v);
    return (part ? bf16_rne(v - __uint_as_float(hi << 16)) : hi) & 0xffffu;
}

__global__ void place_b_kernel(const int2* __restrict__ tab, const float* __restrict__ eff, unsigned* __restrict__ out, unsigned n)
{
    const unsigned i = blockIdx.x * blockDim.x + threadIdx.x;
    if (i >= n) return;
    const int2 t = tab[i];
    const int part = (t.x >> 30) & 1, id0 = t.x & 0x3fffffff, id1 = t.y;
    const float v0 = id0 ? eff[id0 - 1] : 0.0f, v1 = id1 ? eff[id1 - 1] : 0.0f;
    out[i] = bf16_part(v0, part) | (bf16_part(v1, part) << 16);
}

struct DeviceTables {
    int* fwd = nullptr;
    int* bwd = nullptr;
    int* fwd_b = nullptr;
    int* fwd_bh = nullptr;
};
const DeviceTables& device_tables(int device)
{
    static std::mutex mu;
    static DeviceTables per_device[64];
    if (device < 0 || device >= 64) throw_error("vanerf_weights_update: device %d", device);
    std::lock_guard<std::mutex> lock(mu);
    DeviceTables& t = per_device[device];
    if (!t.fwd) {
        const PackTables& p = pack_tables();
        auto upload = [](const std::vector<int>& v) {
            int* d = nullptr;
            HIP_CHECK(hipMalloc(&d, v.size() * sizeof(int)));
            HIP_CHECK(hipMemcpy(d, v.data(), v.size() * sizeof(int), hipMemcpyHostToDevice));
            return d;
        };
        t.bwd = upload(p.bwd);
        t.fwd_b = upload(p.fwd_b);
        t.fwd_bh = upload(p.fwd_bh);
        t.fwd = upload(p.fwd);
    }
    return t;
}

}

extern "C" int vanerf_weights_update(VanerfWeights* h, const VanerfWeightTable* dev, const float* sigmoid_beta_dev, void* stream)
{
    return guarded([&] {
        if (!h || !dev) throw_error("vanerf_weights_update: null argument");
        int device = -1;
        HIP_CHECK(hipGetDevice(&device));
        if (device != h->device) throw_error("vanerf_weights_update: handle packed on device %d, current device %d", h->device, device);
        const PackTables& p = pack_tables();
        if (h->n_floats != (h->mode ? p.fwd_b.size() / 2 : p.fwd.size()) || (h->dev_bwd && h->n_floats_bwd != p.bwd.size()) ||
            h->n_floats_h != (h->mode ? p.fwd_bh.size() / 2 : 0))
            throw_error("internal: handle and placement tables disagree on the stream sizes");
        FoldArgs a;
        layer_sources(*dev, a.l);
        const DeviceTables& t = device_tables(device);
        if (!h->dev_eff) HIP_CHECK(hipMalloc(&h->dev_eff, (size_t)p.n_eff * sizeof(float)));
        hipStream_t s = (hipStream_t)stream;
        hipLaunchKernelGGL(fold_kernel, dim3(128, NUM_LAYERS), dim3(64), 0, s, a, h->dev_eff, sigmoid_beta_dev, h->dev_beta);
        const unsigned n = (unsigned)h->n_floats;
        if (h->mode) {
            hipLaunchKernelGGL(place_b_kernel, dim3((n + 255) / 256), dim3(256), 0, s, reinterpret_cast<const int2*>(t.fwd_b), h->dev_eff,
                               reinterpret_cast<unsigned*>(h->dev), n);
            const unsigned nh = (unsigned)h->n_floats_h;
            hipLaunchKernelGGL(place_b_kernel, dim3((nh + 255) / 256), dim3(256), 0, s, reinterpret_cast<const int2*>(t.fwd_bh), h->dev_eff,
                               reinterpret_cast<unsigned*>(h->dev + h->n_floats), nh);
        } else
            hipLaunchKernelGGL(place_f32_kernel, dim3((n + 255) / 256), dim3(256), 0, s, t.fwd, h->dev_eff, h->dev, n);
        if (h->dev_bwd) {
            const unsigned nb = (unsigned)h->n_floats_bwd;
            hipLaunchKernelGGL(place_f32_kernel, dim3((nb + 255) / 256), dim3(256), 0, s, t.bwd, h->dev_eff, h->dev_bwd, nb);
        }
        HIP_CHECK(hipGetLastError());
        if (!sigmoid_beta_dev) {
            h->beta = dev->sigmoid_beta < 2e-3f ? 2e-3f : dev->sigmoid_beta;
            HIP_CHECK(hipMemcpyAsync(h->dev_beta, &h->beta, sizeof(float), hipMemcpyHostToDevice, s));
        }
    });
}
```

### vanerf_amd/renderer.py

```python
import ctypes
import dataclasses
import os
import weakref
from ctypes import byref, c_float, c_int64, c_uint, c_void_p

import torch
import torch.nn.functional as F

from . import _ffi
from ._ffi import VanerfFrame, VanerfMeshAccel, VanerfPassDesc, VanerfPassOut, VanerfWeightTable, check, lib

NV, NV_HAND, NKPT = 1558, 779, 42


def _ptr(t, dtype=None, cuda=True):
    if t is None:
        return None
    if dtype is not None and t.dtype != dtype:
        raise TypeError(f"expected {dtype}, got {t.dtype}")
    if cuda and not t.is_cuda:
        raise ValueError("the HIP render path needs device tensors (no CPU fallback)")
    if not t.is_contiguous():
        raise ValueError("tensor must be contiguous")
    return c_void_p(t.data_ptr())


def _stream():
    return c_void_p(torch.cuda.current_stream().cuda_stream)


def _farr(values, n):
    vals = [float(v) for v in values]
    assert len(vals) == n, (len(vals), n)
    return (c_float * n)(*vals)


_CONV_KEYS = {
    "geo_at0_w1": "geo_vis_fusion.fconv_at.0.weight", "geo_at0_w2": "geo_vis_fusion.fconv_at.2.weight",
    "geo_ated0_w1": "geo_vis_fusion.fconv_ated.0.weight", "geo_ated0_w2": "geo_vis_fusion.fconv_ated.2.weight",
    "geo_at1_w1": "geo_vis_fusion.fconv_at1.0.weight", "geo_at1_w2": "geo_vis_fusion.fconv_at1.2.weight",
    "geo_ated1_w1": "geo_vis_fusion.fconv_ated1.0.weight", "geo_ated1_w2": "geo_vis_fusion.fconv_ated1.2.weight",
    "tex_at_w1": "tex_vis_fusion.fconv_at.0.weight", "tex_at_w2": "tex_vis_fusion.fconv_at.2.weight",
    "tex_w1": "tex_vis_fusion.fconv.0.weight", "tex_w2": "tex_vis_fusion.fconv.2.weight",
    "l1_w3": "mlp_geo.layers1.layers.3.linear.weight", "l1_b3": "mlp_geo.layers1.layers.3.linear.bias",
    "l2_w2": "mlp_geo.layers2.layers.2.linear.weight", "l2_b2": "mlp_geo.layers2.layers.2.linear.bias",
    "ibr_w": "ibr_compress_gfeat.weight", "ibr_b": "ibr_compress_gfeat.bias",
}
_EXPECT = {
    "geo_at0_w1": (10, 196), "geo_at0_w2": (3, 10), "geo_ated0_w1": (64, 196), "geo_ated0_w2": (64, 64),
    "geo_at1_w1": (10, 28), "geo_at1_w2": (3, 10), "geo_ated1_w1": (8, 28), "geo_ated1_w2": (8, 8),
    "tex_at_w1": (96, 96), "tex_at_w2": (6, 96), "tex_w1": (96, 96), "tex_w2": (40, 96),
    "l1_w3": (64, 120), "l1_b3": (64,), "l2_w2": (2, 64), "l2_b2": (2,), "ibr_w": (24, 128), "ibr_b": (24,),
}
_L1 = [(128, 358), (128, 128), (120, 136)]
_L2 = [(64, 128), (64, 64)]


def weight_table(sd, on_device=False):
    keep = []

    def host(key, shape):
        t = sd[key].detach()
        if on_device:
            n = 1
            for d in shape:
                n *= d
            if not (t.is_cuda and t.dtype == torch.float32 and t.is_contiguous() and t.numel() == n):
                raise ValueError(f"{key}: the device packer takes contiguous fp32 device tensors of {n} elements")
            keep.append(t)
            return c_void_p(t.data_ptr())
        t = t.to("cpu", torch.float32)
        if t.dim() == 3 and t.shape[-1] == 1:
            t = t[:, :, 0]
        t = t.reshape(shape).contiguous()
        keep.append(t)
        return c_void_p(t.data_ptr())

    tab = VanerfWeightTable()
    for field, key in _CONV_KEYS.items():
        setattr(tab, field, host(key, _EXPECT[field]))
    for i, (o, k) in enumerate(_L1):
        p = f"mlp_geo.layers1.layers.{i}.linear."
        tab.l1_v[i], tab.l1_g[i], tab.l1_b[i] = host(p + "weight_v", (o, k)), host(p + "weight_g", (o,)), host(p + "bias", (o,))
    for i, (o, k) in enumerate(_L2):
        p = f"mlp_geo.layers2.layers.{i}.linear."
        tab.l2_v[i], tab.l2_g[i], tab.l2_b[i] = host(p + "weight_v", (o, k)), host(p + "weight_g", (o,)), host(p + "bias", (o,))
    if on_device:
        tab.sigmoid_beta = 0.0
        keep.append(sd["sigmoid_beta"].detach())
    else:
        tab.sigmoid_beta = float(sd["sigmoid_beta"].detach().reshape(-1)[0])
    return tab, keep


PRECISIONS = {"fp32": 0, "bf16x3": 1}


class PackedWeights:

    def __init__(self, sd, mode=0):
        mode = PRECISIONS.get(mode, mode)
        if mode not in (0, 1):
            raise ValueError(f"precision must be one of {sorted(PRECISIONS)}")
        self.mode = mode
        tab, keep = weight_table(sd)
        h = c_void_p()
        check(lib.vanerf_weights_pack(byref(tab), mode, byref(h)))
        self.handle = h
        self.device_index = torch.cuda.current_device() if torch.cuda.is_available() else None
        self._beta = max(float(tab.sigmoid_beta), 2e-3)
        self._beta_src = None
        self.version = 0

    @property
    def beta(self):
        if self._beta_src is not None:
            self._beta = max(float(self._beta_src.reshape(-1)[0]), 2e-3)
        return self._beta

    def update(self, sd):
        tab, keep = weight_table(sd, on_device=True)
        beta = keep[-1]
        if not (beta.is_cuda and beta.dtype == torch.float32):
            raise ValueError("sigmoid_beta: the device packer takes an fp32 device tensor")
        check(lib.vanerf_weights_update(self.handle, byref(tab), c_void_p(beta.data_ptr()), _stream()))
        self._beta_src = beta
        self.version += 1
        return self

    def short_groups(self):
        n = ctypes.c_uint64()
        check(lib.vanerf_weights_short_groups(self.handle, byref(n)))
        return int(n.value)

    def close(self):
        if getattr(self, "handle", None) and lib is not None:
            lib.vanerf_weights_free(self.handle)
            self.handle = None

    __del__ = close


def stream_host(sd, which):
    tab, keep = weight_table(sd)
    n = c_int64()
    check(lib.vanerf_weights_stream_host(byref(tab), which, None, 0, byref(n)))
    out = torch.empty(n.value, dtype=torch.float32)
    check(lib.vanerf_weights_stream_host(byref(tab), which, c_void_p(out.data_ptr()), n.value, byref(n)))
    return out.view(torch.int32)


def stream_device(weights, which):
    n = c_int64()
    check(lib.vanerf_weights_download(weights.handle, which, None, 0, byref(n)))
    out = torch.empty(n.value, dtype=torch.float32)
    check(lib.vanerf_weights_download(weights.handle, which, c_void_p(out.data_ptr()), n.value, byref(n)))
    return out.view(torch.int32)


def pack_weights_host(sd):
    tab, keep = weight_table(sd)
    n = c_int64()
    offs = (c_uint * _ffi.NUM_LAYERS)()
    check(lib.vanerf_weights_pack_host(byref(tab), None, 0, byref(n), offs))
    out = torch.empty(n.value, dtype=torch.float32)
    check(lib.vanerf_weights_pack_host(byref(tab), c_void_p(out.data_ptr()), n.value, byref(n), offs))
    return out, list(offs)


def _grid_sample(feat, uv):
    out = F.grid_sample(feat, uv[:, :, None], mode="bilinear", padding_mode="border", align_corners=True)
    return out.view(*out.shape[:2], -1).permute(0, 2, 1)


def _project(pts, KRT):
    vh = pts @ KRT[:, :3, :3].transpose(1, 2) + KRT[:, :3, 3][:, None]
    return vh[..., :2], vh[..., 2:3]


_POOL3 = {}


def _avg_pool3(x):
    def bins(n, dev):
        key = (n, dev)
        if key not in _POOL3:
            m = torch.zeros(n, 3)
            for i in range(3):
                a, b = (i * n) // 3, -((-(i + 1) * n) // 3)
                m[a:b, i] = 1.0 / (b - a)
            _POOL3[key] = m.to(dev)
        return _POOL3[key]

    return bins(x.shape[-2], x.device).t() @ (x @ bins(x.shape[-1], x.device))


def tex_global_vertex_feature(sd, feat_tex, img, pre="tex_vis_fusion."):
    def conv3x3(x, w):
        B, C, H, W = x.shape
        cols = F.unfold(x, 3, padding=1)
        return (w.reshape(w.shape[0], -1) @ cols).view(B, w.shape[0], H, W)

    def stack(x, name, hw):
        x = conv3x3(x, sd[pre + name + ".0.weight"])
        x = torch.relu(F.layer_norm(x, [hw, hw], sd[pre + name + ".1.weight"], sd[pre + name + ".1.bias"], 1e-6))
        x = conv3x3(x, sd[pre + name + ".3.weight"])
        x = torch.relu(F.layer_norm(x, [hw, hw], sd[pre + name + ".4.weight"], sd[pre + name + ".4.bias"], 1e-6))
        return _avg_pool3(x)

    gf = stack(feat_tex, "fconv3", feat_tex.shape[-1]).reshape(feat_tex.shape[0], 42, -1)
    gf_img = stack(img, "fconv4", img.shape[-1]).reshape(img.shape[0], 42, -1)
    gf = torch.cat([gf_img, gf], -1)
    def conv1d_k3(x, w):
        xp = F.pad(x, (1, 1))
        cols = torch.stack([xp[..., 0:-2], xp[..., 1:-1], xp[..., 2:]], 2).reshape(x.shape[0], -1, x.shape[-1])
        return w.reshape(w.shape[0], -1) @ cols

    x = conv1d_k3(gf, sd[pre + "fconv_gt.0.weight"])
    x = torch.relu(F.layer_norm(x, [18], sd[pre + "fconv_gt.1.weight"], sd[pre + "fconv_gt.1.bias"], 1e-6))
    x = conv1d_k3(x, sd[pre + "fconv_gt.3.weight"])
    return torch.relu(F.layer_norm(x, [18], sd[pre + "fconv_gt.4.weight"], sd[pre + "fconv_gt.4.bias"], 1e-6))


class MeshAccel:
    CL = lib.vanerf_mesh_cluster_size()

    def __init__(self, verts3, faces_i32, grid=64, cell_capacity=None):
        if not (verts3.is_cuda and verts3.dtype == torch.float32 and verts3.is_contiguous() and faces_i32.dtype == torch.int32 and faces_i32.is_contiguous()):
            raise ValueError("MeshAccel needs contiguous device tensors: verts (NV,3) fp32, faces (NF,3) int32")
        nv, nf = verts3.shape[0], faces_i32.shape[0]
        cap = int(cell_capacity) if cell_capacity is not None else 64 * nf
        nbytes = lib.vanerf_mesh_accel_bytes(nv, nf, int(grid), cap)
        check(min(int(nbytes), 0))
        self.tables = torch.empty(int(nbytes), dtype=torch.uint8, device=verts3.device)
        self.verts3, self.faces = verts3, faces_i32
        self.c = VanerfMeshAccel()
        check(lib.vanerf_mesh_accel_build(_ptr(verts3, torch.float32), nv, _ptr(faces_i32, torch.int32), nf, int(grid), cap, _ptr(self.tables),
                                          int(nbytes), byref(self.c), _stream()))

    def table(self, name, dtype, shape):
        off = getattr(self.c, name) - self.tables.data_ptr()
        n = int(torch.tensor(shape).prod()) * torch.empty((), dtype=dtype).element_size()
        return self.tables[off:off + n].view(dtype).view(*shape)


@dataclasses.dataclass(eq=False)
class _VertexProducts:
    weights: weakref.ref
    table: torch.Tensor = None
    version: int = None
    stream: torch.cuda.Stream = None
    event: torch.cuda.Event = None


class FrameData:

    def __init__(self, sd, img, feat_geo, feat_tex, fg_mask, cam_in, targets, sp_data, sp_args=None, gf=None):
        sp_args = sp_args or {"scale": 1.0, "sigma": 0.1}
        dev = img.device
        if not img.is_cuda:
            raise ValueError("FrameData needs device tensors (no CPU fallback)")
        if img.shape[0] != 1 or cam_in["KRT"].shape[0] != 1:
            raise AssertionError("n_views == 1 and batch == 1 (src/networks.py:86,94 is single-view)")
        f32 = torch.float32
        KRT = cam_in["KRT"].to(dev, f32)
        verts = targets["vert_world"].to(dev, f32)
        faces = targets["face_world"].to(dev).long()
        assert verts.shape == (1, NV, 3), verts.shape
        if faces.numel() == 0:
            raise ValueError("face_world is empty")
        ext = sp_data["extrin"].to(dev, f32)
        host = torch.cat([KRT[0, :3, :4].reshape(-1), ext[0, :3, :4].reshape(-1), faces.min().to(f32)[None], faces.max().to(f32)[None]]).tolist()
        if host[24] < 0 or host[25] >= NV:
            raise ValueError("face_world holds vertex indices outside [0, 1558)")
        W, H = float(cam_in["width"]), float(cam_in["height"])
        znear, zfar = float(cam_in["znear"]), float(cam_in["zfar"])
        vxy, vz = _project(verts, KRT)
        vxy = vxy / (vz + 1e-8)
        vert_uv = torch.stack([2.0 * (vxy[..., 0] / (W - 1.0)) - 1.0, 2.0 * (vxy[..., 1] / (H - 1.0)) - 1.0], -1)
        self.vert_xy01 = torch.stack([vxy[..., 0] / (W - 1.0), vxy[..., 1] / (H - 1.0)], -1)[0].contiguous()
        self.vert_z01 = ((vz - znear) / (zfar - znear))[0, :, 0].contiguous()
        self.faces = faces[0].to(torch.int32).contiguous()
        self.verts3 = verts[0].contiguous()
        self.vert_vis = vertex_visibility(self.vert_xy01, self.vert_z01, self.faces)
        self.accel = MeshAccel(self.verts3, self.faces)
        vis = self.vert_vis[None, :, None]
        img = img.to(f32)
        self.vfeat0 = (_grid_sample(feat_geo[0], vert_uv) * vis)[0].contiguous()
        self.vfeat1 = (_grid_sample(feat_geo[1], vert_uv) * vis)[0].contiguous()
        if gf is None:
            gf = tex_global_vertex_feature(sd, feat_tex, img)
        vt = torch.cat([_grid_sample(img, vert_uv), _grid_sample(feat_tex, vert_uv), gf, torch.zeros(1, NV, 3, device=dev)], 2) * vis
        self.vfeat_tex = vt[0].contiguous()
        assert self.vfeat0.shape == (NV, 64) and self.vfeat1.shape == (NV, 8) and self.vfeat_tex.shape == (NV, 32)
        self.geo0 = feat_geo[0][0].permute(1, 2, 0).contiguous()
        self.geo1 = feat_geo[1][0].permute(1, 2, 0).contiguous()
        self.tex = feat_tex[0].permute(1, 2, 0).contiguous()
        self.img = torch.cat([img[0], torch.zeros_like(img[0, :1])], 0).permute(1, 2, 0).contiguous()
        self.mask = fg_mask.reshape(fg_mask.shape[-2], fg_mask.shape[-1]).to(dev, f32).contiguous()
        assert self.geo0.shape[-1] == 64 and self.geo1.shape[-1] == 8 and self.tex.shape[-1] == 8
        assert self.mask.shape == self.img.shape[:2]
        self.verts4 = torch.cat([verts[0], torch.zeros(NV, 1, device=dev)], 1).contiguous()
        kpt = sp_data["kpt3d"].to(dev, f32)
        assert kpt.shape == (1, NKPT, 3), kpt.shape
        kc = kpt @ ext[:, :3, :3].transpose(1, 2) + ext[:, :3, 3][:, None]
        self.kpt_cam = torch.cat([kc[0], torch.zeros(NKPT, 1, device=dev)], 1).contiguous()

        c = VanerfFrame()
        c.geo0, c.geo1, c.tex, c.img, c.mask = (_ptr(t, f32) for t in (self.geo0, self.geo1, self.tex, self.img, self.mask))
        c.h0, c.w0 = self.geo0.shape[:2]
        c.h1, c.w1 = self.geo1.shape[:2]
        c.ht, c.wt = self.tex.shape[:2]
        c.hi, c.wi = self.img.shape[:2]
        c.verts, c.vfeat0, c.vfeat1, c.vfeat_tex = (_ptr(t, f32) for t in (self.verts4, self.vfeat0, self.vfeat1, self.vfeat_tex))
        c.vert_vis, c.kpt_cam = _ptr(self.vert_vis, f32), _ptr(self.kpt_cam, f32)
        c.KRT = _farr(host[:12], 12)
        c.extrin = _farr(host[12:24], 12)
        c.width, c.height, c.znear, c.zfar = W, H, znear, zfar
        c.invalid_sdf = 0.1 / float(cam_in["nml_scale"])
        c.pe_scale = float(sp_args.get("scale", 1.0))
        c.pe_inv_2sigma2 = 1.0 / (2.0 * float(sp_args.get("sigma", 0.1)) ** 2)
        self.c = c
        self._vertex_products = []

    def vertex_products(self, weights):
        if weights.mode != 1 or not vertex_products_enabled():
            return None
        self._vertex_products = [e for e in self._vertex_products if e.weights() is not None]
        stream = torch.cuda.current_stream()
        for e in self._vertex_products:
            if e.weights() is weights:
                if e.version != weights.version:
                    self._build_vertex_products(weights, e)
                elif e.stream != stream:
                    stream.wait_event(e.event)
                    e.table.record_stream(stream)
                return e.table
        e = _VertexProducts(weakref.ref(weights))
        self._build_vertex_products(weights, e)
        self._vertex_products.append(e)
        return e.table

    def _build_vertex_products(self, weights, e):
        stream = torch.cuda.current_stream()
        if e.stream is not None and e.stream != stream:
            e.table.record_stream(stream)
        e.table = build_vertex_products(weights, self, e.table)
        e.version, e.stream, e.event = weights.version, stream, torch.cuda.Event()
        e.event.record(stream)


GEO_NN_COLS, GEO_TWIN_COLS = tuple(range(64, 128)), tuple(range(128, 192))
TEX_NN_COLS = tuple(range(11, 22)) + tuple(range(33, 51))
TEX_TWIN_COLS = tuple(range(22, 33)) + tuple(range(51, 69))
VERTEX_PRODUCT_PARTS = (("A0", 10, 1, 8), ("N0", 64, 2, 16), ("T0", 64, 2, 16), ("P", 96, 3, 16))


def twin_vertex(i):
    return (i + NV_HAND) % NV


def vertex_products_reference(w_at, w_ated, w_tex, vfeat0, vfeat_tex):
    tw = twin_vertex(torch.arange(NV, device=vfeat0.device))
    nn_c, tw_c, tn_c, tt_c = (list(c) for c in (GEO_NN_COLS, GEO_TWIN_COLS, TEX_NN_COLS, TEX_TWIN_COLS))
    return {"A0": vfeat0 @ w_at[:, nn_c].T + vfeat0[tw] @ w_at[:, tw_c].T,
            "N0": vfeat0 @ w_ated[:, nn_c].T, "T0": vfeat0[tw] @ w_ated[:, tw_c].T,
            "P": vfeat_tex[:, :29] @ w_tex[:, tn_c].T + vfeat_tex[tw, :29] @ w_tex[:, tt_c].T}


def vertex_products_unpack(table):
    out, at, pad = {}, 0, 0.0
    for name, rows, nb, nr in VERTEX_PRODUCT_PARTS:
        width = 2 * nb * nr
        part = table[at:at + NV * width].view(NV, 2, nb, nr)
        at += NV * width
        h, ob, r = torch.meshgrid(torch.arange(2), torch.arange(nb), torch.arange(nr), indexing="ij")
        row = (32 * ob + (r & 3) + 8 * (r >> 2) + 4 * h).to(table.device)
        flat = part.reshape(NV, width)
        keep = (row < rows).reshape(-1)
        res = torch.zeros(NV, rows, dtype=table.dtype, device=table.device)
        res[:, row.reshape(-1)[keep]] = flat[:, keep]
        assert int(keep.sum()) == rows
        if (~keep).any():
            pad = max(pad, float(flat[:, ~keep].abs().max()))
        out[name] = res
    assert at == table.numel()
    return out, pad


def build_vertex_products(weights, frame, table=None):
    if table is None:
        table = torch.empty(int(lib.vanerf_vertex_products(None, None, None, 0, None)), dtype=torch.float32, device=frame.vfeat0.device)
    check(lib.vanerf_vertex_products(weights.handle, byref(frame.c), _ptr(table, torch.float32), table.numel(), _stream()))
    return table


def vertex_products_enabled():
    return os.environ.get("VANERF_VERTEX_PRODUCTS", "1") != "0"


def vertex_visibility(vert_xy01, vert_z01, faces_i32, raster=256):
    nv = vert_xy01.shape[0]
    vis = torch.empty(nv, dtype=torch.float32, device=vert_xy01.device)
    scratch = torch.empty(raster * raster, dtype=torch.int32, device=vert_xy01.device)
    check(lib.vanerf_vertex_visibility(_ptr(vert_xy01, torch.float32), _ptr(vert_z01, torch.float32), nv, _ptr(faces_i32, torch.int32),
                                       faces_i32.shape[0], raster, _ptr(scratch), _ptr(vis), _stream()))
    return vis


def render_vis(verts3, faces_i32, vert_vis, R, T, focal, princpt, H=256, W=256, want_raster=False):
    dev = verts3.device
    f32 = torch.float32
    nv = verts3.shape[0]
    scratch = torch.empty(nv * 16, dtype=f32, device=dev)
    rgb = torch.empty(3, H, W, dtype=f32, device=dev)
    vis = torch.empty(H, W, dtype=f32, device=dev)
    p2f = torch.empty(H, W, dtype=torch.int32, device=dev) if want_raster else None
    zbuf = torch.empty(H, W, dtype=f32, device=dev) if want_raster else None
    check(lib.vanerf_render_vis(_ptr(verts3, f32), nv, _ptr(faces_i32, torch.int32), faces_i32.shape[0], _ptr(vert_vis, f32), _ptr(R, f32),
                                _ptr(T, f32), _ptr(focal, f32), _ptr(princpt, f32), int(H), int(W), _ptr(scratch), scratch.numel() * 4, _ptr(rgb),
                                _ptr(vis), _ptr(p2f), _ptr(zbuf), _stream()))
    return (rgb, vis, p2f, zbuf) if want_raster else (rgb, vis)


def mesh_query(verts3, faces_i32, vert_vis, pts, want_face=False):
    n = pts.shape[0]
    sdf = torch.empty(n, dtype=torch.float32, device=pts.device)
    vis = torch.empty(n, dtype=torch.uint8, device=pts.device)
    face = torch.empty(n, dtype=torch.int32, device=pts.device) if want_face else None
    check(lib.vanerf_mesh_query(_ptr(verts3, torch.float32), verts3.shape[0], _ptr(faces_i32, torch.int32), faces_i32.shape[0],
                                _ptr(vert_vis, torch.float32), _ptr(pts, torch.float32), n, _ptr(sdf), _ptr(vis), _ptr(face), _stream()))
    return (sdf, vis, face) if want_face else (sdf, vis)


def _queue_word(dev):
    return torch.empty(2, dtype=torch.int32, device=dev)


MESH_TILE_ORDER_MAX_S = 128
MESH_TILE_ORDER_DEFAULT = 3


def mesh_tile_order_mode():
    e = os.environ.get("VANERF_MESH_TILE_ORDER", "")
    return int(e) if e in ("0", "1", "2", "3") else MESH_TILE_ORDER_DEFAULT


def mesh_tile_order(z, nx, ny):
    S = z.shape[1]
    if z.shape[0] != nx * ny:
        raise ValueError(f"mesh_tile_order: {z.shape[0]} rays for a {nx} x {ny} grid")
    order = torch.empty(((nx + 7) // 8) * ((ny + 7) // 8), S, 64, dtype=torch.int32, device=z.device)
    check(lib.vanerf_mesh_tile_order(_ptr(z, torch.float32), int(nx), int(ny), int(S), _ptr(order), _stream()))
    return order


def mesh_query_accel(accel, verts3, faces_i32, vert_vis, pts, want_face=False, want_knn=True, grid=None, item_order=None):
    gnx, gny, gs = grid if grid is not None else (0, 0, 0)
    if item_order is not None and item_order.numel() != ((gnx + 7) // 8) * ((gny + 7) // 8) * 64 * gs:
        raise ValueError("mesh_query_accel: item_order does not have 64 * S slots per 8 x 8 pixel tile of the grid")
# ... 466 lines not shown
```

Before: 12.08 million rays/s.

## Add lean bf16x3 weight stream with folded matrices and LDS bias table

Adds a third packing level for the split-bf16 MLP weight stream. Two attention-B layers are algebraically folded into the following MLP layers by precomputing matrix products on device. Bias rows for several layers are dropped from the MFMA K dimension and applied from a small LDS-resident bias table. More layers are kept resident in LDS. The streamed portion shrinks from about 486 KB to 426 KB per block, cutting ring DMA traffic and MFMA steps, at the cost of extra LDS use and a more complex pack/update path that must stay consistent.

```diff
diff --git a/vanerf_amd/csrc/api.cpp b/vanerf_amd/csrc/api.cpp
--- a/vanerf_amd/csrc/api.cpp
+++ b/vanerf_amd/csrc/api.cpp
@@ -25,20 +25,25 @@
         constexpr size_t n_ptrs = offsetof(VanerfWeightTable, sigmoid_beta) / sizeof(const float*);
         for (size_t i = 0; i < n_ptrs; ++i)
             if (!ptrs[i]) throw_error("vanerf_weights_pack: weight pointer #%d is null", (int)i);
-        std::vector<float> host, host_bwd, host_h, eff;
+        std::vector<float> host, host_bwd, host_h, eff, host_l, bias;
         LayerOffsets offs{};
-        pack_weights_host(*w, host, offs, mode, mode == 0 ? &host_bwd : nullptr, mode == 1 ? &host_h : nullptr, mode == 1 ? &eff : nullptr);
+        pack_weights_host(*w, host, offs, mode, mode == 0 ? &host_bwd : nullptr, mode == 1 ? &host_h : nullptr, mode == 1 ? &eff : nullptr,
+                          mode == 1 ? &host_l : nullptr, mode == 1 ? &bias : nullptr);
+        host_l.insert(host_l.end(), bias.begin(), bias.end());
         auto* h = new VanerfWeights();
         h->n_floats_bwd = host_bwd.size();
         h->n_floats = host.size();
         h->n_floats_h = host_h.size();
+        h->n_floats_l = host_l.size() - bias.size();
         h->offs = offs;
         h->mode = mode;
         h->beta = w->sigmoid_beta < 2e-3f ? 2e-3f : w->sigmoid_beta;
         hipError_t e = hipGetDevice(&h->device);
-        if (e == hipSuccess) e = hipMalloc(&h->dev, (host.size() + host_h.size()) * sizeof(float));
+        if (e == hipSuccess) e = hipMalloc(&h->dev, (host.size() + host_h.size() + host_l.size()) * sizeof(float));
         if (e == hipSuccess) e = hipMemcpy(h->dev, host.data(), host.size() * sizeof(float), hipMemcpyHostToDevice);
         if (e == hipSuccess && !host_h.empty()) e = hipMemcpy(h->dev + host.size(), host_h.data(), host_h.size() * sizeof(float), hipMemcpyHostToDevice);
+        if (e == hipSuccess && !host_l.empty())
+            e = hipMemcpy(h->dev + host.size() + host_h.size(), host_l.data(), host_l.size() * sizeof(float), hipMemcpyHostToDevice);
         if (e == hipSuccess && !eff.empty()) e = hipMalloc(&h->dev_eff, eff.size() * sizeof(float));
         if (e == hipSuccess && !eff.empty()) e = hipMemcpy(h->dev_eff, eff.data(), eff.size() * sizeof(float), hipMemcpyHostToDevice);
         if (e == hipSuccess && !host_bwd.empty()) e = hipMalloc(&h->dev_bwd, host_bwd.size() * sizeof(float));
@@ -93,11 +98,14 @@
 {
     return guarded([&] {
         if (!w || !n_out) throw_error("vanerf_weights_stream_host: null argument");
-        if (which < 0 || which > 3) throw_error("vanerf_weights_stream_host: which = %d (0 fp32, 1 bf16x3, 2 backward, 3 hoisted bf16x3)", which);
-        std::vector<float> host, bwd, hoisted;
+        if (which < 0 || which > 6)
+            throw_error("vanerf_weights_stream_host: which = %d (0 fp32, 1 bf16x3, 2 backward, 3 hoisted bf16x3, 4 lean bf16x3, 5 its bias table, 6 its folded matrices)", which);
+        std::vector<float> host, bwd, hoisted, lean, bias, eff;
         LayerOffsets offs{};
-        pack_weights_host(*w, host, offs, which == 1 ? 1 : 0, which == 2 ? &bwd : nullptr, which == 3 ? &hoisted : nullptr);
-        const std::vector<float>& src = which == 2 ? bwd : which == 3 ? hoisted : host;
+        pack_weights_host(*w, host, offs, which == 1 ? 1 : 0, which == 2 ? &bwd : nullptr, which == 3 ? &hoisted : nullptr, which == 6 ? &eff : nullptr,
+                          which == 4 ? &lean : nullptr, which == 5 ? &bias : nullptr);
+        if (which == 6) eff.erase(eff.begin(), eff.begin() + eff_fold_offset());
+        const std::vector<float>& src = which == 2 ? bwd : which == 3 ? hoisted : which == 4 ? lean : which == 5 ? bias : which == 6 ? eff : host;
         *n_out = (int64_t)src.size();
         if (out) {
             if (cap < (int64_t)src.size()) throw_error("vanerf_weights_stream_host: buffer too small");
@@ -110,9 +118,13 @@
 {
     return guarded([&] {
         if (!w || !n_out) throw_error("vanerf_weights_download: null argument");
-        if (which != 0 && which != 2 && which != 3) throw_error("vanerf_weights_download: which = %d (0 forward, 2 backward, 3 hoisted bf16x3)", which);
-        const float* src = which == 2 ? w->dev_bwd : which == 3 ? (w->n_floats_h ? w->dev + w->n_floats : nullptr) : w->dev;
-        const size_t n = which == 2 ? w->n_floats_bwd : which == 3 ? w->n_floats_h : w->n_floats;
+        if (which != 0 && (which < 2 || which > 6))
+            throw_error("vanerf_weights_download: which = %d (0 forward, 2 backward, 3 hoisted bf16x3, 4 lean bf16x3, 5 its bias table, 6 its folded matrices)", which);
+        const float* lean = w->n_floats_l ? w->dev + w->n_floats + w->n_floats_h : nullptr;
+        const float* src = which == 2 ? w->dev_bwd : which == 3 ? (w->n_floats_h ? w->dev + w->n_floats : nullptr) : which == 4 ? lean
+                           : which == 5 ? (lean ? lean + w->n_floats_l : nullptr) : which == 6 ? (lean && w->dev_eff ? w->dev_eff + eff_fold_offset() : nullptr) : w->dev;
+        const size_t n = which == 2 ? w->n_floats_bwd : which == 3 ? w->n_floats_h : which == 4 ? w->n_floats_l : which == 5 ? (size_t)BIAS_TABLE_FLOATS
+                         : which == 6 ? (size_t)FOLD_FLOATS : w->n_floats;
         if (!src) throw_error("vanerf_weights_download: the handle carries no such stream");
         *n_out = (int64_t)n;
         if (out) {
diff --git a/vanerf_amd/csrc/common.h b/vanerf_amd/csrc/common.h
--- a/vanerf_amd/csrc/common.h
+++ b/vanerf_amd/csrc/common.h
@@ -62,8 +62,10 @@
 }
 
 void pack_weights_host(const VanerfWeightTable& w, std::vector<float>& out, LayerOffsets& offs, int mode = 0, std::vector<float>* bwd = nullptr,
-                       std::vector<float>* hoisted = nullptr, std::vector<float>* eff_out = nullptr);
+                       std::vector<float>* hoisted = nullptr, std::vector<float>* eff_out = nullptr, std::vector<float>* lean = nullptr,
+                       std::vector<float>* bias = nullptr);
 unsigned eff_layer_offset(int l);
+unsigned eff_fold_offset();
 struct LayerSrc {
     const float* w;
     const float* g;
@@ -74,6 +76,7 @@
 void layer_sources(const VanerfWeightTable& w, LayerSrc out[NUM_LAYERS]);
 struct PackTables {
     std::vector<int> fwd, bwd, fwd_b, fwd_bh;
+    std::vector<int> fwd_bl, bias;
     LayerOffsets offs{};
     unsigned n_eff = 0;
 };
@@ -88,6 +91,7 @@
 struct VanerfWeights {
     float* dev = nullptr;
     size_t n_floats_h = 0;
+    size_t n_floats_l = 0;
     float* dev_bwd = nullptr;
     size_t n_floats_bwd = 0;
     size_t n_floats = 0;
diff --git a/vanerf_amd/csrc/layer_spec.h b/vanerf_amd/csrc/layer_spec.h
--- a/vanerf_amd/csrc/layer_spec.h
+++ b/vanerf_amd/csrc/layer_spec.h
@@ -38,20 +38,35 @@
     return o;
 }
 
-constexpr int kT_b(int l, bool hoist)
+constexpr bool lean_no_bias_pair(int l) { return l == L_MLP1 || l == L_HEAD0 || l == L_HEAD1 || l == L_HEAD2 || l == L_IBR; }
+constexpr int kT_b(int l, int level)
 {
-    if (hoist && (l == L_GEO_AT0_A || l == L_GEO_ATED0_A)) return 32 + 2;
-    if (hoist && l == L_TEX_AT_A) return 6 + 12 + 2;
+    if (level >= 1 && (l == L_GEO_AT0_A || l == L_GEO_ATED0_A)) return 32 + 2;
+    if (level >= 1 && l == L_TEX_AT_A) return 6 + 12 + (level == 2 ? 1 : 2);
+    if (level == 2 && (l == L_GEO_ATED0_B || l == L_GEO_ATED1_B)) return 0;
+    if (level == 2 && lean_no_bias_pair(l)) return kT[l] - 1;
+    if (level == 2 && l == L_TEX_A) return 48;
     return kT[l];
 }
-constexpr int steps_b(int l, bool hoist = false) { return (kT_b(l, hoist) + 7) / 8; }
-constexpr unsigned layer_dwords_b(int l, bool hoist = false) { return (unsigned)steps_b(l, hoist) * (unsigned)kNB[l] * 2u * 64u * 4u; }
-constexpr unsigned layer_offset_b(int l, bool hoist = false)
+constexpr int steps_b(int l, int level = 0) { return (kT_b(l, level) + 7) / 8; }
+constexpr unsigned layer_dwords_b(int l, int level = 0) { return (unsigned)steps_b(l, level) * (unsigned)kNB[l] * 2u * 64u * 4u; }
+constexpr unsigned layer_offset_b(int l, int level = 0)
 {
     unsigned o = 0;
-    for (int i = 0; i < l; ++i) o += layer_dwords_b(i, hoist);
+    for (int i = 0; i < l; ++i) o += layer_dwords_b(i, level);
     return o;
 }
+constexpr unsigned bias_table_floats(int l) { return lean_no_bias_pair(l) ? 2u * (unsigned)kNB[l] * 16u : 0u; }
+constexpr unsigned bias_table_offset(int l)
+{
+    unsigned o = 0;
+    for (int i = 0; i < l; ++i) o += bias_table_floats(i);
+    return o;
+}
+constexpr unsigned BIAS_TABLE_FLOATS = bias_table_offset(NUM_LAYERS);
+constexpr unsigned STREAM_SLACK_DW = 2u * 64u * 4u;
+constexpr unsigned FOLD0_ROWS = 128u, FOLD0_COLS = 64u, FOLD1_ROWS = 120u, FOLD1_COLS = 8u;
+constexpr unsigned FOLD_FLOATS = FOLD0_ROWS * FOLD0_COLS + FOLD1_ROWS * FOLD1_COLS;
 
 constexpr unsigned VP_NV = 1558u;
 constexpr unsigned VP_A0_ROW = 16u, VP_N0_ROW = 64u, VP_P_ROW = 96u;
diff --git a/vanerf_amd/csrc/query_kernel.hip b/vanerf_amd/csrc/query_kernel.hip
--- a/vanerf_amd/csrc/query_kernel.hip
+++ b/vanerf_amd/csrc/query_kernel.hip
@@ -1,4 +1,5 @@
 #include <algorithm>
+#include <cstdlib>
 #include <utility>
 
 #include "common.h"
@@ -58,20 +59,25 @@
 
 struct FragB { u32x4 hi, lo; };
 
-constexpr int LDS_FIRST = L_IBR;
-template <bool HOIST> constexpr unsigned RES_BASE_DW = layer_offset_b(LDS_FIRST, HOIST);
-template <bool HOIST> constexpr unsigned RES_DW = layer_offset_b(NUM_LAYERS, HOIST) - layer_offset_b(LDS_FIRST, HOIST);
+template <int LEVEL> constexpr int LDS_FIRST = LEVEL == 2 ? L_HEAD1 : L_IBR;
+template <int LEVEL> constexpr unsigned RES_BASE_DW = layer_offset_b(LDS_FIRST<LEVEL>, LEVEL);
+template <int LEVEL> constexpr unsigned RES_DW = layer_offset_b(NUM_LAYERS, LEVEL) - layer_offset_b(LDS_FIRST<LEVEL>, LEVEL);
 constexpr unsigned RING_PHASE_PIECES = 16u, RING_BYTES = 2u * RING_PHASE_PIECES * 1024u;
 constexpr unsigned LDS_KPT = 0u, LDS_CTRL = 2u * PE_KPT_PER_HALF * 16u, LDS_LAT0 = 768u, LDS_RING = 1024u, LDS_RES = LDS_RING + RING_BYTES;
-template <bool HOIST> constexpr unsigned DYN_LDS_BYTES = LDS_RES + RES_DW<HOIST> * 4u;
-template <bool HOIST> constexpr unsigned RING_PIECES = RES_BASE_DW<HOIST> / 256u;
-template <bool HOIST> constexpr unsigned RING_STREAM_PHASES = (RING_PIECES<HOIST> + RING_PHASE_PIECES - 1u) / RING_PHASE_PIECES;
-template <bool HOIST> constexpr unsigned RING_PHASES = (RING_STREAM_PHASES<HOIST> + 1u) / 2u * 2u;
+template <int LEVEL> constexpr unsigned LDS_BIAS = LDS_RES + RES_DW<LEVEL> * 4u;
+template <int LEVEL> constexpr unsigned DYN_LDS_BYTES = LDS_BIAS<LEVEL> + (LEVEL == 2 ? BIAS_TABLE_FLOATS * 4u : 0u);
+template <int LEVEL> constexpr unsigned RING_PIECES = RES_BASE_DW<LEVEL> / 256u;
+template <int LEVEL> constexpr unsigned RING_STREAM_PHASES = (RING_PIECES<LEVEL> + RING_PHASE_PIECES - 1u) / RING_PHASE_PIECES;
+template <int LEVEL> constexpr unsigned RING_PHASES = (RING_STREAM_PHASES<LEVEL> + 1u) / 2u * 2u;
 static_assert(WPB<1> == 8, "the ring's DMA schedule deals 2 pieces of a phase to each of 8 waves");
-static_assert(RING_PHASES<false> * RING_PHASE_PIECES * 256u <= layer_offset_b(NUM_LAYERS), "the last phase's DMA must stay inside the stream");
-static_assert(RING_PHASES<true> * RING_PHASE_PIECES * 256u <= layer_offset_b(NUM_LAYERS, true), "the last phase's DMA must stay inside the hoisted stream");
+static_assert(RING_PHASES<0> * RING_PHASE_PIECES * 256u <= layer_offset_b(NUM_LAYERS), "the last phase's DMA must stay inside the stream");
+static_assert(RING_PHASES<1> * RING_PHASE_PIECES * 256u <= layer_offset_b(NUM_LAYERS, 1), "the last phase's DMA must stay inside the hoisted stream");
+static_assert(RING_PHASES<2> * RING_PHASE_PIECES * 256u <= layer_offset_b(NUM_LAYERS, 2), "the last phase's DMA must stay inside the lean stream");
+static_assert(RING_STREAM_PHASES<1> == 31u && RING_STREAM_PHASES<2> == 27u, "the streamed parts: 486 KB hoisted, 426 KB lean");
 static_assert(LDS_CTRL + 8u + 2u * 4u * WPB<1> <= LDS_LAT0 && LDS_LAT0 + 128u <= LDS_RING, "control words / constant latent overlap their neighbours");
-static_assert(DYN_LDS_BYTES<false> <= 160u * 1024u && DYN_LDS_BYTES<true> <= DYN_LDS_BYTES<false>, "key points + control words + ring + resident fragments must fit the CU's 160 KB");
+static_assert(DYN_LDS_BYTES<0> <= 160u * 1024u && DYN_LDS_BYTES<1> <= DYN_LDS_BYTES<0> && DYN_LDS_BYTES<2> <= 160u * 1024u,
+              "key points + control words + ring + resident fragments (+ bias table) must fit the CU's 160 KB");
+static_assert(LDS_BIAS<2> % 16u == 0, "the bias table is read 16 bytes at a time");
 extern __shared__ __attribute__((aligned(16))) u32x4 s_dyn[];
 typedef __attribute__((address_space(3))) u32x4 lds_u32x4_t;
 typedef __attribute__((address_space(3))) unsigned lds_u32_t;
@@ -107,21 +113,21 @@
                  : "s"(la.dma_lds), "s"(la.dma_src), "i"(lds_off), "i"(src_off), "v"(la.w[0]), "s"(rs)
                  : "memory");
 }
-template <bool HOIST, unsigned P> __device__ __forceinline__ void phase_begin(WRsrc rs, const LAddr& la)
-{
-    constexpr unsigned RING_PHASES = ::RING_PHASES<HOIST>;
+template <int LEVEL, unsigned P> __device__ __forceinline__ void phase_begin(WRsrc rs, const LAddr& la)
+{
+    constexpr unsigned RING_PHASES = ::RING_PHASES<LEVEL>;
     if constexpr (P > 0) asm volatile("s_waitcnt vmcnt(0) lgkmcnt(0)\n\ts_barrier" ::: "memory");
     ring_dma<(P + 1u) % RING_PHASES>(rs, la);
 }
 
-template <bool HOIST> __device__ __forceinline__ void ring_close(WRsrc rs, const LAddr& la)
-{
-    if constexpr (RING_STREAM_PHASES<HOIST> % 2u == 1u) phase_begin<HOIST, RING_PHASES<HOIST> - 1u>(rs, la);
-}
-
-template <bool HOIST, bool RES, unsigned DW> __device__ __forceinline__ FragB wload_blk(WRsrc rs, const LAddr& la)
-{
-    constexpr unsigned RING_PHASES = ::RING_PHASES<HOIST>, RES_BASE_DW = ::RES_BASE_DW<HOIST>;
+template <int LEVEL> __device__ __forceinline__ void ring_close(WRsrc rs, const LAddr& la)
+{
+    if constexpr (RING_STREAM_PHASES<LEVEL> % 2u == 1u) phase_begin<LEVEL, RING_PHASES<LEVEL> - 1u>(rs, la);
+}
+
+template <int LEVEL, bool RES, unsigned DW> __device__ __forceinline__ FragB wload_blk(WRsrc rs, const LAddr& la)
+{
+    constexpr unsigned RING_PHASES = ::RING_PHASES<LEVEL>, RES_BASE_DW = ::RES_BASE_DW<LEVEL>;
     static_assert(RES == (DW >= RES_BASE_DW), "a layer's fragments are either resident or streamed through the ring: nothing is fetched per wave");
     FragB r;
     if constexpr (RES) {
@@ -130,20 +136,20 @@
     } else {
         constexpr unsigned q = DW / 256u;
         static_assert(q % 2u == 0 && q + 1u < RING_PHASES * RING_PHASE_PIECES, "block fragments are two consecutive pieces inside the streamed part");
-        if constexpr (q % RING_PHASE_PIECES == 0) phase_begin<HOIST, q / RING_PHASE_PIECES>(rs, la);
+        if constexpr (q % RING_PHASE_PIECES == 0) phase_begin<LEVEL, q / RING_PHASE_PIECES>(rs, la);
         r.hi = lds_frag<LDS_RING + (q % (2u * RING_PHASE_PIECES)) * 1024u>(la);
         r.lo = lds_frag<LDS_RING + ((q + 1u) % (2u * RING_PHASE_PIECES)) * 1024u>(la);
     }
     return r;
 }
 
-template <bool HOIST, int NB, int T, bool RES, unsigned SBASE_DW> __device__ __forceinline__ RingB<NB> ring_start_b(WRsrc rs, const LAddr& la)
+template <int LEVEL, int NB, int T, bool RES, unsigned SBASE_DW> __device__ __forceinline__ RingB<NB> ring_start_b(WRsrc rs, const LAddr& la)
 {
     constexpr int D = RingDepthB<NB>::value, S = (T + 7) / 8;
     RingB<NB> r;
     static_for<D>([&](auto ic) {
         constexpr int i = decltype(ic)::value;
-        if constexpr (i < S * NB) r.b[i] = wload_blk<HOIST, RES, SBASE_DW + i * 512u>(rs, la);
+        if constexpr (i < S * NB) r.b[i] = wload_blk<LEVEL, RES, SBASE_DW + i * 512u>(rs, la);
     });
     __builtin_amdgcn_sched_barrier(0x000F);
     return r;
@@ -157,7 +163,7 @@
 
 struct NoPre { template <class C> __device__ __forceinline__ void operator()(C) const {} };
 
-template <bool HOIST, int NB, int T, bool RES, unsigned SBASE_DW, class Op, class Pre = NoPre>
+template <int LEVEL, int NB, int T, bool RES, unsigned SBASE_DW, class Op, class Pre = NoPre>
 __device__ __forceinline__ void run_layer_b(f32x16 (&acc)[NB], RingB<NB>& ring, WRsrc rs, const LAddr& la, Op&& operand,
                                             Pre&& pre = Pre{})
 {
@@ -189,7 +195,7 @@
                 if constexpr (m * NCH / (3 * NB) == c) {
                     if constexpr (pr == 0) {
                         a[ob] = ring.b[idx % D];
-                        if constexpr (idx + D < S * NB) ring.b[idx % D] = wload_blk<HOIST, RES, SBASE_DW + (idx + D) * 512u>(rs, la);
+                        if constexpr (idx + D < S * NB) ring.b[idx % D] = wload_blk<LEVEL, RES, SBASE_DW + (idx + D) * 512u>(rs, la);
                     }
                     const bf16x8 wh = __builtin_bit_cast(bf16x8, a[ob].hi), wl = __builtin_bit_cast(bf16x8, a[ob].lo);
                     acc[ob] = __builtin_amdgcn_mfma_f32_32x32x16_bf16(pr == 2 ? wl : wh, pr == 1 ? xl : xh, acc[ob], 0, 0, 0);
@@ -226,13 +232,13 @@
 template <int MODE> struct LaneSel { using type = LLane; };
 template <> struct LaneSel<1> { using type = LAddr; };
 __device__ __forceinline__ unsigned lane_of(const LLane& la) { return (unsigned)la.lane; }
-template <int MODE, bool HOIST, int NB, int T, int L> __device__ __forceinline__ typename RingSel<MODE, NB>::type ring_start_m(WRsrc rs, const typename LaneSel<MODE>::type& la)
+template <int MODE, int LEVEL, int NB, int T, int L> __device__ __forceinline__ typename RingSel<MODE, NB>::type ring_start_m(WRsrc rs, const typename LaneSel<MODE>::type& la)
 {
     if constexpr (MODE == 0) return ring_start<NB, T>(rs, layer_offset(L), lane_of(la) * NB * 4u);
-    else return ring_start_b<HOIST, NB, T, (L >= LDS_FIRST), layer_offset_b(L, HOIST)>(rs, la);
-}
-
-template <int MODE, bool HOIST, int NB, int T, int L, class Op>
+    else return ring_start_b<LEVEL, NB, T, (L >= LDS_FIRST<LEVEL>), layer_offset_b(L, LEVEL)>(rs, la);
+}
+
+template <int MODE, int LEVEL, int NB, int T, int L, class Op>
 __device__ __forceinline__ void run_layer_m(f32x16 (&acc)[NB], typename RingSel<MODE, NB>::type& ring, WRsrc rs, const typename LaneSel<MODE>::type& la, Op&& operand)
 {
     if constexpr (MODE == 0)
@@ -241,7 +247,10 @@
             spill_x<L, decltype(tc)::value>(la, b);
             return b;
         });
-    else run_layer_b<HOIST, NB, T, (L >= LDS_FIRST), layer_offset_b(L, HOIST)>(acc, ring, rs, la, static_cast<Op&&>(operand));
+    else {
+        static_assert(MODE == 0 || T == kT_b(L, LEVEL), "the kernel and the packed stream agree on the layer's k-pairs");
+        run_layer_b<LEVEL, NB, T, (L >= LDS_FIRST<LEVEL>), layer_offset_b(L, LEVEL)>(acc, ring, rs, la, static_cast<Op&&>(operand));
+    }
 }
 
 __device__ __forceinline__ int lane_id_fresh()
@@ -363,7 +372,7 @@
     return r;
 }
 
-template <int MODE, bool HOIST, int HC, int NBO, int NREG_MID, int l_at_a>
+template <int MODE, int LEVEL, int HC, int NBO, int NREG_MID, int l_at_a>
 __device__ __forceinline__ void geo_scale(WRsrc W, int lane, const typename LaneSel<MODE>::type& la, typename RingSel<MODE, 1>::type& ring_at,
                                           float (&pix)[HC], float (&nn)[HC], float (&tw)[HC], float s0, float s1,
                                           f32x16 (&outacc)[NBO])
@@ -380,30 +389,35 @@
     };
     f32x16 at[1];
     zero<1>(at);
-    run_layer_m<MODE, HOIST, 1, TIN, l_at_a>(at, ring_at, W, la, input);
-    auto r_gate = ring_start_m<MODE, HOIST, 1, 6, l_at_a + 1>(W, la);
-    auto r_mid = ring_start_m<MODE, HOIST, NBO, TIN, l_at_a + 2>(W, la);
+    run_layer_m<MODE, LEVEL, 1, TIN, l_at_a>(at, ring_at, W, la, input);
+    auto r_gate = ring_start_m<MODE, LEVEL, 1, 6, l_at_a + 1>(W, la);
+    auto r_mid = ring_start_m<MODE, LEVEL, NBO, TIN, l_at_a + 2>(W, la);
     if constexpr (MODE == 0) relu<1>(at);
     f32x16 gate[1];
     zero<1>(gate);
-    run_layer_m<MODE, HOIST, 1, 6, l_at_a + 1>(gate, r_gate, W, la, [&](auto tc) -> float { return lazy_act<MODE, ACT_RELU>(at[0][decltype(tc)::value]); });
+    run_layer_m<MODE, LEVEL, 1, 6, l_at_a + 1>(gate, r_gate, W, la, [&](auto tc) -> float { return lazy_act<MODE, ACT_RELU>(at[0][decltype(tc)::value]); });
     const float a0 = __shfl(sigmoid_f(gate[0][0]), lane & 31);
     const float a1 = __shfl(sigmoid_f(gate[0][1]), lane & 31);
     const float a2 = __shfl(sigmoid_f(gate[0][2]), lane & 31);
     if constexpr (MODE == 0) { constexpr int A = HC == 32 ? AUX_G0 : AUX_G1; spill_aux<A>(la, a0); spill_aux<A + 1>(la, a1); spill_aux<A + 2>(la, a2); }
 #pragma unroll
     for (int t = 0; t < HC; ++t) { pix[t] *= a0; nn[t] *= a1; tw[t] *= a2; }
-    f32x16 mid[NBO];
-    zero<NBO>(mid);
-    run_layer_m<MODE, HOIST, NBO, TIN, l_at_a + 2>(mid, r_mid, W, la, input);
-    auto r_out = ring_start_m<MODE, HOIST, NBO, TOUT, l_at_a + 3>(W, la);
-    if constexpr (MODE == 0) relu<NBO>(mid);
-    zero<NBO>(outacc);
-    run_layer_m<MODE, HOIST, NBO, TOUT, l_at_a + 3>(outacc, r_out, W, la,
-                         [&](auto tc) -> float { constexpr int t = decltype(tc)::value; return lazy_act<MODE, ACT_RELU>(mid[t / 16][t % 16]); });
-}
-
-template <int MODE>
+    if constexpr (LEVEL == 2) {
+        zero<NBO>(outacc);
+        run_layer_m<MODE, LEVEL, NBO, TIN, l_at_a + 2>(outacc, r_mid, W, la, input);
+    } else {
+        f32x16 mid[NBO];
+        zero<NBO>(mid);
+        run_layer_m<MODE, LEVEL, NBO, TIN, l_at_a + 2>(mid, r_mid, W, la, input);
+        auto r_out = ring_start_m<MODE, LEVEL, NBO, TOUT, l_at_a + 3>(W, la);
+        if constexpr (MODE == 0) relu<NBO>(mid);
+        zero<NBO>(outacc);
+        run_layer_m<MODE, LEVEL, NBO, TOUT, l_at_a + 3>(outacc, r_out, W, la,
+                             [&](auto tc) -> float { constexpr int t = decltype(tc)::value; return lazy_act<MODE, ACT_RELU>(mid[t / 16][t % 16]); });
+    }
+}
+
+template <int MODE, int LEVEL>
 __device__ __forceinline__ void geo_scale0_vp(WRsrc W, int lane, const typename LaneSel<MODE>::type& la, typename RingSel<MODE, 1>::type& ring_at,
                                               float (&pix)[32], const float (&a0s)[8], const float (&n0)[32], const float (&t0)[32], float s0, float s1,
                                               f32x16 (&outacc)[2])
@@ -419,23 +433,29 @@
     zero<1>(at);
 #pragma unroll
     for (int r = 0; r < 8; ++r) at[0][r] = a0s[r];
-    run_layer_m<MODE, true, 1, TIN, L_GEO_AT0_A>(at, ring_at, W, la, input);
-    auto r_gate = ring_start_m<MODE, true, 1, 6, L_GEO_AT0_B>(W, la);
-    auto r_mid = ring_start_m<MODE, true, 2, TIN, L_GEO_ATED0_A>(W, la);
+    run_layer_m<MODE, LEVEL, 1, TIN, L_GEO_AT0_A>(at, ring_at, W, la, input);
+    auto r_gate = ring_start_m<MODE, LEVEL, 1, 6, L_GEO_AT0_B>(W, la);
+    auto r_mid = ring_start_m<MODE, LEVEL, 2, TIN, L_GEO_ATED0_A>(W, la);
     f32x16 gate[1];
     zero<1>(gate);
-    run_layer_m<MODE, true, 1, 6, L_GEO_AT0_B>(gate, r_gate, W, la, [&](auto tc) -> float { return lazy_act<MODE, ACT_RELU>(at[0][decltype(tc)::value]); });
+    run_layer_m<MODE, LEVEL, 1, 6, L_GEO_AT0_B>(gate, r_gate, W, la, [&](auto tc) -> float { return lazy_act<MODE, ACT_RELU>(at[0][decltype(tc)::value]); });
     const float a0 = __shfl(sigmoid_f(gate[0][0]), lane & 31);
     const float a1 = __shfl(sigmoid_f(gate[0][1]), lane & 31);
     const float a2 = __shfl(sigmoid_f(gate[0][2]), lane & 31);
-    f32x16 mid[2];
-#pragma unroll
-    for (int t = 0; t < 32; ++t) { pix[t] *= a0; mid[t / 16][t % 16] = fmaf(a2, t0[t], a1 * n0[t]); }
-    run_layer_m<MODE, true, 2, TIN, L_GEO_ATED0_A>(mid, r_mid, W, la, input);
-    auto r_out = ring_start_m<MODE, true, 2, 32, L_GEO_ATED0_B>(W, la);
-    zero<2>(outacc);
-    run_layer_m<MODE, true, 2, 32, L_GEO_ATED0_B>(outacc, r_out, W, la,
-                         [&](auto tc) -> float { constexpr int t = decltype(tc)::value; return lazy_act<MODE, ACT_RELU>(mid[t / 16][t % 16]); });
+    if constexpr (LEVEL == 2) {
+#pragma unroll
+        for (int t = 0; t < 32; ++t) { pix[t] *= a0; outacc[t / 16][t % 16] = fmaf(a2, t0[t], a1 * n0[t]); }
+        run_layer_m<MODE, LEVEL, 2, TIN, L_GEO_ATED0_A>(outacc, r_mid, W, la, input);
+    } else {
+        f32x16 mid[2];
+#pragma unroll
+        for (int t = 0; t < 32; ++t) { pix[t] *= a0; mid[t / 16][t % 16] = fmaf(a2, t0[t], a1 * n0[t]); }
+        run_layer_m<MODE, LEVEL, 2, TIN, L_GEO_ATED0_A>(mid, r_mid, W, la, input);
+        auto r_out = ring_start_m<MODE, LEVEL, 2, 32, L_GEO_ATED0_B>(W, la);
+        zero<2>(outacc);
+        run_layer_m<MODE, LEVEL, 2, 32, L_GEO_ATED0_B>(outacc, r_out, W, la,
+                             [&](auto tc) -> float { constexpr int t = decltype(tc)::value; return lazy_act<MODE, ACT_RELU>(mid[t / 16][t % 16]); });
+    }
 }
 
 template <int NB> __device__ __forceinline__ void load_acc(const float* __restrict__ table, unsigned elem_off, f32x16 (&acc)[NB])
@@ -449,13 +469,31 @@
         }
 }
 
-template <int MODE, bool SPILL = false, bool HOIST = false>
+template <int L, int NB> __device__ __forceinline__ void load_bias(int h, f32x16 (&acc)[NB])
+{
+    static_assert(bias_table_floats(L) == 2u * NB * 16u, "the layer has a row in the bias table");
+    unsigned a = (unsigned)h * (NB * 64u) + (LDS_BIAS<2> + bias_table_offset(L) * 4u);
+    asm volatile("" : "+v"(a));
+#pragma unroll
+    for (int ob = 0; ob < NB; ++ob)
+#pragma unroll
+        for (int i = 0; i < 4; ++i) {
+            const u32x4 v = *reinterpret_cast<const lds_u32x4_t*>((size_t)(a + 64u * ob + 16u * i));
+            acc[ob][4 * i] = __uint_as_float(v.x); acc[ob][4 * i + 1] = __uint_as_float(v.y);
+            acc[ob][4 * i + 2] = __uint_as_float(v.z); acc[ob][4 * i + 3] = __uint_as_float(v.w);
+        }
+}
+
+template <int MODE, bool SPILL = false, int LEVEL = 0>
 __global__ __launch_bounds__(64 * WPB<MODE>, SPILL ? WAVES_PER_SIMD_SPILL : WAVES_PER_SIMD) void query_kernel(const QueryParams P)
 {
     static_assert(!SPILL || MODE == 0, "the training spill runs on the fp32 kernel");
-    static_assert(!HOIST || MODE == 1, "only the split-bf16 kernel has a hoisted variant");
-    [[maybe_unused]] constexpr unsigned RES_BASE_DW = ::RES_BASE_DW<HOIST>, RES_DW = ::RES_DW<HOIST>;
-    constexpr int T_GEO0 = kT_b(L_GEO_AT0_A, HOIST), T_TEX_AT = kT_b(L_TEX_AT_A, HOIST);
+    static_assert(LEVEL >= 0 && LEVEL <= 2 && (LEVEL == 0 || MODE == 1), "only the split-bf16 kernel has a hoisted and a lean variant");
+    constexpr bool HOIST = LEVEL >= 1, LEAN = LEVEL == 2;
+    [[maybe_unused]] constexpr unsigned RES_BASE_DW = ::RES_BASE_DW<LEVEL>, RES_DW = ::RES_DW<LEVEL>;
+    constexpr int LDS_FIRST = ::LDS_FIRST<LEVEL>;
+    constexpr int T_GEO0 = kT_b(L_GEO_AT0_A, LEVEL), T_TEX_AT = kT_b(L_TEX_AT_A, LEVEL), T_TEX = kT_b(L_TEX_A, LEVEL);
+    constexpr int T_MLP1 = kT_b(L_MLP1, LEVEL), T_HEAD0 = kT_b(L_HEAD0, LEVEL), T_HEAD1 = kT_b(L_HEAD1, LEVEL), T_HEAD2 = kT_b(L_HEAD2, LEVEL), T_IBR = kT_b(L_IBR, LEVEL);
     constexpr int WAVES_PER_BLOCK = WPB<MODE>, BLOCK = 64 * WAVES_PER_BLOCK;
 
     const int lane_k = threadIdx.x & 63;
@@ -500,6 +538,10 @@
     if constexpr (MODE == 1) {
         const u32x4* __restrict__ src = reinterpret_cast<const u32x4*>(P.w) + RES_BASE_DW / 4;
         for (unsigned i = threadIdx.x; i < RES_DW / 4; i += BLOCK) s_dyn[LDS_RES / 16 + i] = src[i];
+        if constexpr (LEAN) {
+            const u32x4* __restrict__ bsrc = reinterpret_cast<const u32x4*>(P.w) + (layer_offset_b(NUM_LAYERS, LEVEL) + STREAM_SLACK_DW) / 4;
+            if (threadIdx.x < BIAS_TABLE_FLOATS / 4) s_dyn[LDS_BIAS<LEVEL> / 16 + threadIdx.x] = bsrc[threadIdx.x];
+        }
         const LAddr la0 = make_laddr(lane, wv_u);
         ring_dma<0>(W, la0);
         asm volatile("s_waitcnt vmcnt(0)" ::: "memory");
@@ -508,11 +550,12 @@
     if constexpr (MODE == 1) {
         if (wv_u == 0u) {
             const LAddr la0 = make_laddr(lane, wv_u);
-            auto r0 = ring_start_m<MODE, HOIST, 1, 65, L_IBR>(W, la0);
+            auto r0 = ring_start_m<MODE, LEVEL, 1, T_IBR, L_IBR>(W, la0);
             f32x16 lat0[1];
-            zero<1>(lat0);
+            if constexpr (LEAN) load_bias<L_IBR, 1>(lane >> 5, lat0);
+            else zero<1>(lat0);
             const float one0 = (lane >> 5) ? 0.0f : 1.0f;
-            run_layer_m<MODE, HOIST, 1, 65, L_IBR>(lat0, r0, W, la0, [&](auto tc) -> float { return decltype(tc)::value < 64 ? 0.0f : one0; });
+            run_layer_m<MODE, LEVEL, 1, T_IBR, L_IBR>(lat0, r0, W, la0, [&](auto tc) -> float { return decltype(tc)::value < 64 ? 0.0f : one0; });
             if ((lane & 31) == 0)
                 static_for<16>([&](auto rc) { constexpr int r = decltype(rc)::value; reinterpret_cast<lds_u32_t*>((size_t)LDS_LAT0)[(lane >> 5) * 16 + r] = __float_as_uint(lat0[0][r]); });
         }
@@ -605,7 +648,7 @@
         f32x16 pool[4];
         f32x16 head[1];
         if (any_valid) {
-            auto r_at0 = ring_start_m<MODE, HOIST, 1, T_GEO0, L_GEO_AT0_A>(W, la);
+            auto r_at0 = ring_start_m<MODE, LEVEL, 1, T_GEO0, L_GEO_AT0_A>(W, la);
             f32x16 g64[2], g8[1];
             float pix8[4], nn8[4], tw8[4];
             {
@@ -629,8 +672,8 @@
                 };
                 if constexpr (MODE == 0) geo1_gathers();
                 STAMP(2);
-                if constexpr (HOIST) geo_scale0_vp<MODE>(W, lane, la, r_at0, pix, a0s, nn, tw, sc0, sc1, g64);
-                else geo_scale<MODE, HOIST, 32, 2, 16, L_GEO_AT0_A>(W, lane, la, r_at0, pix, nn, tw, sc0, sc1, g64);
+                if constexpr (HOIST) geo_scale0_vp<MODE, LEVEL>(W, lane, la, r_at0, pix, a0s, nn, tw, sc0, sc1, g64);
+                else geo_scale<MODE, LEVEL, 32, 2, 16, L_GEO_AT0_A>(W, lane, la, r_at0, pix, nn, tw, sc0, sc1, g64);
                 if constexpr (MODE == 1) geo1_gathers();
                 STAMP(3);
             }
@@ -639,12 +682,12 @@
             WFrag<4> ring0[D0];
             RingB<4> ring0b;
             {
-                auto r_at1 = ring_start_m<MODE, HOIST, 1, 14, L_GEO_AT1_A>(W, la);
+                auto r_at1 = ring_start_m<MODE, LEVEL, 1, 14, L_GEO_AT1_A>(W, la);
                 if constexpr (MODE == 0) {
                     static_for<D0>([&](auto fc) { constexpr int f = decltype(fc)::value; ring0[f] = wload<4>(W, (base0 + f * 256) * 4u, v4); });
                 }
-                geo_scale<MODE, HOIST, 4, 1, 4, L_GEO_AT1_A>(W, lane, la, r_at1, pix8, nn8, tw8, sc0, sc1, g8);
-                if constexpr (MODE == 1) ring0b = ring_start_b<HOIST, 4, 180, false, layer_offset_b(L_MLP0, HOIST)>(W, la);
+                geo_scale<MODE, LEVEL, 4, 1, 4, L_GEO_AT1_A>(W, lane, la, r_at1, pix8, nn8, tw8, sc0, sc1, g8);
+                if constexpr (MODE == 1) ring0b = ring_start_b<LEVEL, 4, 180, false, layer_offset_b(L_MLP0, LEVEL)>(W, la);
                 STAMP(4);
             }
 
@@ -702,10 +745,11 @@
                         });
                     } else {
                         float feat[PE_KPT_PER_HALF][PE_FEATS];
-                        run_layer_b<HOIST, 4, 180, false, layer_offset_b(L_MLP0, HOIST)>(a0, ring0b, W, la,
+                        run_layer_b<LEVEL, 4, 180, false, layer_offset_b(L_MLP0, LEVEL)>(a0, ring0b, W, la,
                             [&](auto tc) -> float {
                                 constexpr int t = decltype(tc)::value;
                                 if constexpr (t < 147) return feat[t / 7][t % 7];
+                                else if constexpr (LEAN && t < 179) return lazy_act<MODE, ACT_RELU>(g64[(t - 147) / 16][(t - 147) % 16]);
                                 else return chain(g64, std::integral_constant<int, t - 147>{}, std::integral_constant<int, 32>{});
                             },
                             [&](auto sc) {
@@ -719,28 +763,29 @@
                     }
                 }
                 STAMP(5);
-                auto r1 = ring_start_m<MODE, HOIST, 4, 65, L_MLP1>(W, la);
+                auto r1 = ring_start_m<MODE, LEVEL, 4, T_MLP1, L_MLP1>(W, la);
                 if constexpr (MODE == 0) softplus<4>(a0);
                 f32x16 a1[4];
-                zero<4>(a1);
-                run_layer_m<MODE, HOIST, 4, 65, L_MLP1>(a1, r1, W, la, [&](auto tc) -> float { return chain_sp(a0, tc, std::integral_constant<int, 64>{}); });
-                auto r2 = ring_start_m<MODE, HOIST, 4, 69, L_MLP2>(W, la);
+                if constexpr (LEAN) load_bias<L_MLP1, 4>(h, a1);
+                else zero<4>(a1);
+                run_layer_m<MODE, LEVEL, 4, T_MLP1, L_MLP1>(a1, r1, W, la, [&](auto tc) -> float { return chain_sp(a0, tc, std::integral_constant<int, 64>{}); });
+                auto r2 = ring_start_m<MODE, LEVEL, 4, 69, L_MLP2>(W, la);
                 if constexpr (MODE == 0) softplus<4>(a1);
                 zero<4>(a0);
-                run_layer_m<MODE, HOIST, 4, 69, L_MLP2>(a0, r2, W, la, [&](auto tc) -> float {
+                run_layer_m<MODE, LEVEL, 4, 69, L_MLP2>(a0, r2, W, la, [&](auto tc) -> float {
                     constexpr int t = decltype(tc)::value;
                     if constexpr (t < 64) return lazy_act<MODE, ACT_SOFTPLUS>(a1[t / 16][t % 16]);
-                    else if constexpr (t < 68) return g8[0][t - 64];
+                    else if constexpr (t < 68) return LEAN ? lazy_act<MODE, ACT_RELU>(g8[0][t - 64]) : g8[0][t - 64];
                     else return one_h0;
                 });
-                auto r3 = ring_start_m<MODE, HOIST, 2, 61, L_MLP3>(W, la);
+                auto r3 = ring_start_m<MODE, LEVEL, 2, 61, L_MLP3>(W, la);
                 if constexpr (MODE == 0) softplus<4>(a0);
                 zero<2>(xv);
-                run_layer_m<MODE, HOIST, 2, 61, L_MLP3>(xv, r3, W, la, [&](auto tc) -> float { return chain_sp(a0, tc, std::integral_constant<int, 60>{}); });
+                run_layer_m<MODE, LEVEL, 2, 61, L_MLP3>(xv, r3, W, la, [&](auto tc) -> float { return chain_sp(a0, tc, std::integral_constant<int, 60>{}); });
             }
             STAMP(6);
             if constexpr (MODE == 0) tex_gathers();
-            auto rh0 = ring_start_m<MODE, HOIST, 2, 65, L_HEAD0>(W, la);
+            auto rh0 = ring_start_m<MODE, LEVEL, 2, T_HEAD0, L_HEAD0>(W, la);
             if constexpr (MODE == 0)
                 static_for<32>([&](auto rc) { constexpr int r = decltype(rc)::value; spill_aux<AUX_XV + r>(la, xv[r / 16][r % 16]); });
     #pragma unroll
@@ -754,18 +799,22 @@
                 }
             {
                 f32x16 m0[2], m1[2];
-                zero<2>(m0);
-                run_layer_m<MODE, HOIST, 2, 65, L_HEAD0>(m0, rh0, W, la, [&](auto tc) -> float { return chain(pool, tc, std::integral_constant<int, 64>{}); });
-                auto rh1 = ring_start_m<MODE, HOIST, 2, 33, L_HEAD1>(W, la);
+                if constexpr (LEAN) load_bias<L_HEAD0, 2>(h, m0);
+                else zero<2>(m0);
+                run_layer_m<MODE, LEVEL, 2, T_HEAD0, L_HEAD0>(m0, rh0, W, la, [&](auto tc) -> float { return chain(pool, tc, std::integral_constant<int, 64>{}); });
+                static_assert(LDS_FIRST == L_HEAD2 + 1 || LDS_FIRST == L_HEAD0 + 1, "the ring is closed behind its last streamed layer");
+                if constexpr (MODE == 1 && LDS_FIRST == L_HEAD0 + 1) ring_close<LEVEL>(W, la);
+                auto rh1 = ring_start_m<MODE, LEVEL, 2, T_HEAD1, L_HEAD1>(W, la);
                 if constexpr (MODE == 0) softplus<2>(m0);
-                zero<2>(m1);
-                run_layer_m<MODE, HOIST, 2, 33, L_HEAD1>(m1, rh1, W, la, [&](auto tc) -> float { return chain_sp(m0, tc, std::integral_constant<int, 32>{}); });
-                auto rh2 = ring_start_m<MODE, HOIST, 1, 33, L_HEAD2>(W, la);
+                if constexpr (LEAN) load_bias<L_HEAD1, 2>(h, m1);
+                else zero<2>(m1);
+                run_layer_m<MODE, LEVEL, 2, T_HEAD1, L_HEAD1>(m1, rh1, W, la, [&](auto tc) -> float { return chain_sp(m0, tc, std::integral_constant<int, 32>{}); });
+                auto rh2 = ring_start_m<MODE, LEVEL, 1, T_HEAD2, L_HEAD2>(W, la);
                 if constexpr (MODE == 0) softplus<2>(m1);
-                zero<1>(head);
-                run_layer_m<MODE, HOIST, 1, 33, L_HEAD2>(head, rh2, W, la, [&](auto tc) -> float { return chain_sp(m1, tc, std::integral_constant<int, 32>{}); });
-                static_assert(LDS_FIRST == L_HEAD2 + 1, "the ring is closed behind its last streamed layer");
-                if constexpr (MODE == 1) ring_close<HOIST>(W, la);
+                if constexpr (LEAN) load_bias<L_HEAD2, 1>(h, head);
+                else zero<1>(head);
+                run_layer_m<MODE, LEVEL, 1, T_HEAD2, L_HEAD2>(head, rh2, W, la, [&](auto tc) -> float { return chain_sp(m1, tc, std::integral_constant<int, 32>{}); });
+                if constexpr (MODE == 1 && LDS_FIRST == L_HEAD2 + 1) ring_close<LEVEL>(W, la);
             }
         } else {
             if constexpr (MODE == 0) tex_gathers();
@@ -778,23 +827,24 @@
         f32x16 lat[1];
         typename RingSel<MODE, 3>::type r_ta;
         if (MODE == 1 && !any_valid) {
-            r_ta = ring_start_m<MODE, HOIST, 3, T_TEX_AT, L_TEX_AT_A>(W, la);
+            r_ta = ring_start_m<MODE, LEVEL, 3, T_TEX_AT, L_TEX_AT_A>(W, la);
             if constexpr (MODE == 1)
                 static_for<16>([&](auto rc) { constexpr int r = decltype(rc)::value; lat[0][r] = __uint_as_float(reinterpret_cast<const lds_u32_t*>((size_t)LDS_LAT0)[h * 16 + r]); });
         } else {
-            auto r_ibr = ring_start_m<MODE, HOIST, 1, 65, L_IBR>(W, la);
-            r_ta = ring_start_m<MODE, HOIST, 3, T_TEX_AT, L_TEX_AT_A>(W, la);
-            zero<1>(lat);
-            run_layer_m<MODE, HOIST, 1, 65, L_IBR>(lat, r_ibr, W, la, [&](auto tc) -> float { return chain(pool, tc, std::integral_constant<int, 64>{}); });
+            auto r_ibr = ring_start_m<MODE, LEVEL, 1, T_IBR, L_IBR>(W, la);
+            r_ta = ring_start_m<MODE, LEVEL, 3, T_TEX_AT, L_TEX_AT_A>(W, la);
+            if constexpr (LEAN) load_bias<L_IBR, 1>(h, lat);
+            else zero<1>(lat);
+            run_layer_m<MODE, LEVEL, 1, T_IBR, L_IBR>(lat, r_ibr, W, la, [&](auto tc) -> float { return chain(pool, tc, std::integral_constant<int, 64>{}); });
         }
         STAMP(8);
         f32x16 rgb[1];
         {
             float q[6];
             q[0] = h ? qt[3] : qi[0]; q[1] = h ? qt[4] : qi[1]; q[2] = h ? qt[5] : qi[2];
-            q[3] = h ? qt[6] : qt[0]; q[4] = h ? qt[7] : qt[1]; q[5] = h ? 0.0f : qt[2];
+            q[3] = h ? qt[6] : qt[0]; q[4] = h ? qt[7] : qt[1]; q[5] = h ? (LEAN ? vis_tw : 0.0f) : qt[2];
             const float t0 = h ? vis_nn : q_vis;
-            const float t1 = h ? 0.0f : vis_tw;
+            [[maybe_unused]] const float t1 = h ? 0.0f : vis_tw;
             f32x16 latg = lat[0];
             auto tex_in = [&](auto tc) -> float {
                 constexpr int t = decltype(tc)::value;
@@ -802,7 +852,7 @@
                 else if constexpr (t < 35) return q[t - 29];
                 else if constexpr (t < 47) return latg[t - 35];
                 else if constexpr (t == 47) return t0;
-                else return t1;
+                else { static_assert(!LEAN || t < 48, "the lean stream has no (vis_twin | -) pair"); return t1; }
             };
             auto from_ta = [&](auto& ta_) { return [&](auto tc) -> float { constexpr int t = decltype(tc)::value; return lazy_act<MODE, ACT_RELU>(ta_[t / 16][t % 16]); }; };
             auto tex_at_in = [&](auto tc) -> float {
@@ -811,18 +861,18 @@
                 else if constexpr (t < 6) return q[t];
                 else if constexpr (t < 18) return latg[t - 6];
                 else if constexpr (t == 18) return t0;
-                else return t1;
+                else { static_assert(!LEAN || t < 19, "the lean stream has no (vis_twin | -) pair"); return t1; }
             };
             f32x16 ta[3];
             if constexpr (HOIST) load_acc<3>(P.vp + VP_P, (unsigned)(nn_idx * (int)VP_P_ROW + 48 * h), ta);
             else zero<3>(ta);
-            run_layer_m<MODE, HOIST, 3, T_TEX_AT, L_TEX_AT_A>(ta, r_ta, W, la, tex_at_in);
-            auto r_tg = ring_start_m<MODE, HOIST, 1, 48, L_TEX_AT_B>(W, la);
+            run_layer_m<MODE, LEVEL, 3, T_TEX_AT, L_TEX_AT_A>(ta, r_ta, W, la, tex_at_in);
+            auto r_tg = ring_start_m<MODE, LEVEL, 1, 48, L_TEX_AT_B>(W, la);
             if constexpr (MODE == 0) relu<3>(ta);
             f32x16 tg[1];
             zero<1>(tg);
-            run_layer_m<MODE, HOIST, 1, 48, L_TEX_AT_B>(tg, r_tg, W, la, from_ta(ta));
-            auto r_tb = ring_start_m<MODE, HOIST, 3, 49, L_TEX_A>(W, la);
+            run_layer_m<MODE, LEVEL, 1, 48, L_TEX_AT_B>(tg, r_tg, W, la, from_ta(ta));
+            auto r_tb = ring_start_m<MODE, LEVEL, 3, T_TEX, L_TEX_A>(W, la);
             float m0 = sigmoid_f(tg[0][0]), m1 = sigmoid_f(tg[0][1]), m2 = sigmoid_f(tg[0][2]), m3 = sigmoid_f(tg[0][3]);
             float o0 = __shfl_xor(m0, 32), o1 = __shfl_xor(m1, 32), o2 = __shfl_xor(m2, 32);
             const float gq = h ? o0 : m0;
@@ -838,15 +888,16 @@
 #pragma unroll
             for (int t = 11; t < 29; ++t) row[t] *= ggf;
 #pragma unroll
-            for (int t = 0; t < 6; ++t) q[t] *= gq;
+            for (int t = 0; t < (LEAN ? 5 : 6); ++t) q[t] *= gq;
+            if constexpr (LEAN) q[5] = h ? q[5] : q[5] * gq;
 #pragma unroll
             for (int r = 0; r < 12; ++r) latg[r] = lat[0][r] * glat;
             zero<3>(ta);
-            run_layer_m<MODE, HOIST, 3, 49, L_TEX_A>(ta, r_tb, W, la, tex_in);
-            auto r_rgb = ring_start_m<MODE, HOIST, 1, 48, L_TEX_B>(W, la);
+            run_layer_m<MODE, LEVEL, 3, T_TEX, L_TEX_A>(ta, r_tb, W, la, tex_in);
+            auto r_rgb = ring_start_m<MODE, LEVEL, 1, 48, L_TEX_B>(W, la);
             if constexpr (MODE == 0) relu<3>(ta);
             zero<1>(rgb);
-            run_layer_m<MODE, HOIST, 1, 48, L_TEX_B>(rgb, r_rgb, W, la, from_ta(ta));
+            run_layer_m<MODE, LEVEL, 1, 48, L_TEX_B>(rgb, r_rgb, W, la, from_ta(ta));
         }
         STAMP(9);
         if constexpr (MODE == 1) asm volatile("s_waitcnt vmcnt(0)" ::: "memory");
@@ -895,9 +946,9 @@
 }
 
 struct QueryLaunch { void (*kernel)(QueryParams); int wpb, blocks_per_cu; unsigned lds_bytes; };
-template <int MODE, bool SPILL = false, bool HOIST = false> QueryLaunch query_launch()
-{
-    return {query_kernel<MODE, SPILL, HOIST>, WPB<MODE>, (SPILL ? WAVES_PER_SIMD_SPILL : WAVES_PER_SIMD) * 4 / WPB<MODE>, MODE == 1 ? DYN_LDS_BYTES<HOIST> : 0u};
+template <int MODE, bool SPILL = false, int LEVEL = 0> QueryLaunch query_launch()
+{
+    return {query_kernel<MODE, SPILL, LEVEL>, WPB<MODE>, (SPILL ? WAVES_PER_SIMD_SPILL : WAVES_PER_SIMD) * 4 / WPB<MODE>, MODE == 1 ? DYN_LDS_BYTES<LEVEL> : 0u};
 }
 
 long long query_blocks(const QueryLaunch& L, int64_t n)
@@ -916,6 +967,12 @@
     if (L.lds_bytes) HIP_CHECK(hipFuncSetAttribute(reinterpret_cast<const void*>(L.kernel), hipFuncAttributeMaxDynamicSharedMemorySize, (int)L.lds_bytes));
     hipLaunchKernelGGL(L.kernel, dim3((unsigned)blocks), dim3(64 * L.wpb), L.lds_bytes, (hipStream_t)stream, P);
     HIP_CHECK(hipGetLastError());
+}
+
+bool lean_stream_enabled()
+{
+    const char* e = std::getenv("VANERF_LEAN_STREAM");
+    return !(e && e[0] == '0' && !e[1]);
 }
 
 }
@@ -937,9 +994,12 @@
         const bool hoist = vertex_products != nullptr;
         if (hoist && (w->mode != 1 || !w->n_floats_h)) throw_error("vanerf_query_samples: a table of vertex products needs a bf16x3 weight handle");
         if (hoist && (reinterpret_cast<uintptr_t>(vertex_products) & 15u)) throw_error("vanerf_query_samples: the table must be 16-byte aligned");
-        QueryParams P = query_params(f, hoist ? w->dev + w->n_floats : w->dev, hoist ? w->n_floats_h : w->n_floats, pts, query_sdf, query_vis, knn_idx, raw, n, out);
+        const bool lean = hoist && w->n_floats_l && lean_stream_enabled();
+        const float* stream_w = lean ? w->dev + w->n_floats + w->n_floats_h : hoist ? w->dev + w->n_floats : w->dev;
+        const size_t stream_floats = lean ? w->n_floats_l + BIAS_TABLE_FLOATS : hoist ? w->n_floats_h : w->n_floats;
+        QueryParams P = query_params(f, stream_w, stream_floats, pts, query_sdf, query_vis, knn_idx, raw, n, out);
         P.noise = noise; P.order = order; P.valid = valid; P.short_groups = w->stats; P.vp = vertex_products;
-        const QueryLaunch L = w->mode == 1 && hoist ? query_launch<1, false, true>() : w->mode == 1 ? query_launch<1>() : query_launch<0>();
+        const QueryLaunch L = lean ? query_launch<1, false, 2>() : w->mode == 1 && hoist ? query_launch<1, false, 1>() : w->mode == 1 ? query_launch<1>() : query_launch<0>();
         launch_query(L, query_blocks(L, n), P, queue_word, stream);
     });
 }
diff --git a/vanerf_amd/csrc/weights_pack.cpp b/vanerf_amd/csrc/weights_pack.cpp
--- a/vanerf_amd/csrc/weights_pack.cpp
+++ b/vanerf_amd/csrc/weights_pack.cpp
@@ -55,7 +55,13 @@
 }
 static_assert(eff_offset(NUM_LAYERS) < (1u << 24), "ids must be exact in fp32");
 
-Mat id_matrix(int l)
+constexpr unsigned EFF_FOLD0 = eff_offset(NUM_LAYERS), EFF_FOLD1 = EFF_FOLD0 + FOLD0_ROWS * FOLD0_COLS, EFF_TOTAL = EFF_FOLD0 + FOLD_FLOATS;
+static_assert(EFF_TOTAL < (1u << 24), "ids must be exact in fp32");
+static_assert(FOLD0_ROWS == (unsigned)kShape[L_MLP0].nout && FOLD0_COLS == (unsigned)kShape[L_GEO_ATED0_B].nout && kShape[L_MLP0].kin == 294 + (int)FOLD0_COLS &&
+              FOLD1_ROWS == (unsigned)kShape[L_MLP2].nout && FOLD1_COLS == (unsigned)kShape[L_GEO_ATED1_B].nout && kShape[L_MLP2].kin == 128 + (int)FOLD1_COLS,
+              "the folded matrices replace the geo columns of mlp0 / mlp2");
+
+Mat id_matrix(int l, int level = 0)
 {
     const Shape sh = kShape[l];
     if (sh.nout != kNOUT[l]) throw_error("internal: layer %d has %d outputs, spec says %d", l, sh.nout, kNOUT[l]);
@@ -65,6 +71,12 @@
     if (sh.bias) {
         m.b.resize(sh.nout);
         for (int o = 0; o < sh.nout; ++o) m.b[o] = (float)(base + m.w.size() + o);
+    }
+    if (level == 2 && (l == L_MLP0 || l == L_MLP2)) {
+        const int c0 = l == L_MLP0 ? 294 : 128, nc = (int)(l == L_MLP0 ? FOLD0_COLS : FOLD1_COLS);
+        const unsigned fold = (l == L_MLP0 ? EFF_FOLD0 : EFF_FOLD1) + 1u;
+        for (int o = 0; o < sh.nout; ++o)
+            for (int k = 0; k < nc; ++k) m.w[(size_t)o * sh.kin + c0 + k] = (float)(fold + (unsigned)(o * nc + k));
     }
     return m;
 }
@@ -90,12 +102,12 @@
         }
 }
 
-void emit_b_ids(std::vector<WordB>& out, int layer, const Mat& m, const Pairs& pairs, bool hoist)
-{
-    const int nb = kNB[layer], T = kT_b(layer, hoist), S = steps_b(layer, hoist);
+void emit_b_ids(std::vector<WordB>& out, int layer, const Mat& m, const Pairs& pairs, int level)
+{
+    const int nb = kNB[layer], T = kT_b(layer, level), S = steps_b(layer, level);
     if ((int)pairs.size() != T) throw_error("internal: layer %d has %d k-pairs, spec says %d", layer, (int)pairs.size(), T);
     size_t base = out.size();
-    out.resize(base + layer_dwords_b(layer, hoist), WordB{0, 0, 0});
+    out.resize(base + layer_dwords_b(layer, level), WordB{0, 0, 0});
     WordB* dst = out.data() + base;
     for (int s = 0; s < S; ++s)
         for (int ob = 0; ob < nb; ++ob)
@@ -127,17 +139,17 @@
     return p;
 }
 
-Pairs tex_input_pairs(bool hoist = false)
+Pairs tex_input_pairs(bool hoist = false, bool merged = false)
 {
     Pairs p;
     if (!hoist) {
         for (int t = 0; t < 11; ++t) p.emplace_back(11 + t, 22 + t);
         for (int t = 0; t < 18; ++t) p.emplace_back(33 + t, 51 + t);
     }
-    for (int u = 0; u < 6; ++u) p.emplace_back(u, u < 5 ? 6 + u : ZERO);
+    for (int u = 0; u < 6; ++u) p.emplace_back(u, u < 5 ? 6 + u : merged ? 95 : ZERO);
     chain(p, 1, 12, 69, 24);
     p.emplace_back(93, 94);
-    p.emplace_back(95, ZERO);
+    if (!merged) p.emplace_back(95, ZERO);
     return p;
 }
 
@@ -145,15 +157,17 @@
 
 namespace {
 
-Pairs layer_pairs(int l, bool hoist = false)
+Pairs layer_pairs(int l, int level = 0)
 {
     Pairs p;
+    const bool hoist = level >= 1, lean = level == 2;
+    auto bias_pair = [&](Pairs& q) { if (!(lean && lean_no_bias_pair(l))) ::bias_pair(q); };
     switch (l) {
     case L_GEO_AT0_A: case L_GEO_ATED0_A: return geo_input_pairs(64, hoist);
     case L_GEO_AT1_A: case L_GEO_ATED1_A: return geo_input_pairs(8);
     case L_GEO_AT0_B: case L_GEO_AT1_B: chain(p, 1, 6, 0, 10); return p;
-    case L_GEO_ATED0_B: chain(p, 2, 16, 0, 64); return p;
-    case L_GEO_ATED1_B: chain(p, 1, 4, 0, 8); return p;
+    case L_GEO_ATED0_B: if (!lean) chain(p, 2, 16, 0, 64); return p;
+    case L_GEO_ATED1_B: if (!lean) chain(p, 1, 4, 0, 8); return p;
     case L_MLP0:
         for (int i = 0; i < PE_KPT_PER_HALF; ++i)
             for (int f = 0; f < PE_FEATS; ++f) p.emplace_back(f * 42 + i, f * 42 + PE_KPT_PER_HALF + i);
@@ -165,8 +179,8 @@
     case L_MLP3: chain(p, 4, 12, 0, 120); bias_pair(p); return p;
     case L_HEAD0: case L_IBR: chain(p, 2, 16, 0, 64); chain(p, 2, 16, 64, 64); bias_pair(p); return p;
     case L_HEAD1: case L_HEAD2: chain(p, 2, 16, 0, 64); bias_pair(p); return p;
-    case L_TEX_AT_A: return tex_input_pairs(hoist);
-    case L_TEX_A: return tex_input_pairs();
+    case L_TEX_AT_A: return tex_input_pairs(hoist, lean);
+    case L_TEX_A: return tex_input_pairs(false, lean);
     case L_TEX_AT_B: case L_TEX_B: chain(p, 3, 16, 0, 96); return p;
     }
     throw_error("internal: no layer %d", l);
@@ -205,7 +219,7 @@
 {
     vanerf::LayerSrc src[NUM_LAYERS];
     sources(w, src);
-    eff.assign(eff_offset(NUM_LAYERS), 0.0f);
+    eff.assign(EFF_TOTAL, 0.0f);
     for (int l = 0; l < NUM_LAYERS; ++l) {
         const vanerf::LayerSrc& s = src[l];
         float* e = eff.data() + s.eff;
@@ -222,6 +236,19 @@
             if (s.b) e[(size_t)s.nout * s.kin + o] = s.b[o];
         }
     }
+    auto fold = [&](int la, int a0, int lb, unsigned dst) {
+        const int kin_a = kShape[la].kin, n = kShape[lb].nout, nc = kShape[lb].kin;
+        const float* a = eff.data() + eff_offset(la);
+        const float* b = eff.data() + eff_offset(lb);
+        for (int o = 0; o < kShape[la].nout; ++o)
+            for (int c = 0; c < nc; ++c) {
+                float acc = 0.0f;
+                for (int k = 0; k < n; ++k) acc = std::fmaf(a[(size_t)o * kin_a + a0 + k], b[(size_t)k * nc + c], acc);
+                eff[dst + (size_t)o * nc + c] = acc;
+            }
+    };
+    fold(L_MLP0, 294, L_GEO_ATED0_B, EFF_FOLD0);
+    fold(L_MLP2, 128, L_GEO_ATED1_B, EFF_FOLD1);
 }
 
 void emit_bwd(std::vector<float>& out, int layer, const Mat& m, const Pairs& pairs)
@@ -283,7 +310,7 @@
     static const PackTables tables = [] {
         PackTables t;
         std::vector<float> fwd, bwd;
-        std::vector<WordB> fwd_b, fwd_bh;
+        std::vector<WordB> fwd_b, fwd_bh, fwd_bl;
         for (int l = 0; l < NUM_LAYERS; ++l) {
             t.offs.off[l] = (unsigned)fwd.size();
             if (fwd.size() != layer_offset(l)) throw_error("internal: layer %d starts at %zu, layer_spec.h says %u", l, fwd.size(), layer_offset(l));
@@ -291,26 +318,38 @@
             const Mat m = id_matrix(l);
             const Pairs p = layer_pairs(l);
             emit(fwd, l, m, p);
-            emit_b_ids(fwd_b, l, m, p, false);
-            if (fwd_bh.size() != layer_offset_b(l, true)) throw_error("internal: layer %d (hoisted bf16x3) starts at %zu, layer_spec.h says %u", l, fwd_bh.size(), layer_offset_b(l, true));
-            emit_b_ids(fwd_bh, l, m, layer_pairs(l, true), true);
+            emit_b_ids(fwd_b, l, m, p, 0);
+            if (fwd_bh.size() != layer_offset_b(l, 1)) throw_error("internal: layer %d (hoisted bf16x3) starts at %zu, layer_spec.h says %u", l, fwd_bh.size(), layer_offset_b(l, 1));
+            emit_b_ids(fwd_bh, l, m, layer_pairs(l, 1), 1);
+            if (fwd_bl.size() != layer_offset_b(l, 2)) throw_error("internal: layer %d (lean bf16x3) starts at %zu, layer_spec.h says %u", l, fwd_bl.size(), layer_offset_b(l, 2));
+            emit_b_ids(fwd_bl, l, id_matrix(l, 2), layer_pairs(l, 2), 2);
+            if (t.bias.size() != bias_table_offset(l)) throw_error("internal: layer %d (bias table) starts at %zu, layer_spec.h says %u", l, t.bias.size(), bias_table_offset(l));
+            if (lean_no_bias_pair(l))
+                for (int h = 0; h < 2; ++h)
+                    for (int ob = 0; ob < kNB[l]; ++ob)
+                        for (int r = 0; r < 16; ++r) {
+                            const int o = 32 * ob + row0(r) + 4 * h;
+                            t.bias.push_back(o < m.nout ? (int)m.b[o] : 0);
+                        }
             emit_bwd(bwd, l, m, p);
         }
         fwd.resize(fwd.size() + 2 * 64 * 4, 0.0f);
         bwd.resize(bwd.size() + 2 * 64 * 4, 0.0f);
         fwd_b.resize(fwd_b.size() + 2 * 64 * 4, WordB{0, 0, 0});
         fwd_bh.resize(fwd_bh.size() + 2 * 64 * 4, WordB{0, 0, 0});
+        fwd_bl.resize(fwd_bl.size() + STREAM_SLACK_DW, WordB{0, 0, 0});
+        if (t.bias.size() != BIAS_TABLE_FLOATS) throw_error("internal: bias table of %zu floats, layer_spec.h says %u", t.bias.size(), BIAS_TABLE_FLOATS);
         t.fwd.assign(fwd.begin(), fwd.end());
         t.bwd.assign(bwd.begin(), bwd.end());
-        for (auto [src, dst] : {std::pair{&fwd_b, &t.fwd_b}, std::pair{&fwd_bh, &t.fwd_bh}}) {
+        for (auto [src, dst] : {std::pair{&fwd_b, &t.fwd_b}, std::pair{&fwd_bh, &t.fwd_bh}, std::pair{&fwd_bl, &t.fwd_bl}}) {
             dst->resize(2 * src->size());
             for (size_t i = 0; i < src->size(); ++i) {
                 (*dst)[2 * i] = (*src)[i].id0 | ((*src)[i].part << 30);
                 (*dst)[2 * i + 1] = (*src)[i].id1;
             }
         }
-        t.n_eff = eff_offset(NUM_LAYERS);
-        for (const std::vector<int>* v : {&t.fwd, &t.bwd, &t.fwd_b, &t.fwd_bh})
+        t.n_eff = EFF_TOTAL;
+        for (const std::vector<int>* v : {&t.fwd, &t.bwd, &t.fwd_b, &t.fwd_bh, &t.fwd_bl, &t.bias})
             for (int id : *v)
                 if ((id & 0x3fffffff) > (int)t.n_eff) throw_error("internal: placement id %d beyond the %u effective weights", id, t.n_eff);
         return t;
@@ -321,9 +360,10 @@
 void layer_sources(const VanerfWeightTable& w, LayerSrc out[NUM_LAYERS]) { sources(w, out); }
 
 unsigned eff_layer_offset(int l) { return eff_offset(l); }
+unsigned eff_fold_offset() { return EFF_FOLD0; }
 
 void pack_weights_host(const VanerfWeightTable& w, std::vector<float>& out, LayerOffsets& offs, int mode, std::vector<float>* bwd, std::vector<float>* hoisted,
-                       std::vector<float>* eff_out)
+                       std::vector<float>* eff_out, std::vector<float>* lean, std::vector<float>* bias)
 {
     const PackTables& t = pack_tables();
     std::vector<float> eff;
@@ -340,6 +380,11 @@
         }
     };
     if (hoisted) place_b(t.fwd_bh, *hoisted);
+    if (lean) place_b(t.fwd_bl, *lean);
+    if (bias) {
+        bias->resize(t.bias.size());
+        for (size_t i = 0; i < bias->size(); ++i) (*bias)[i] = value(t.bias[i]);
+    }
     if (mode) {
         place_b(t.fwd_b, out);
     } else {
diff --git a/vanerf_amd/csrc/weights_update.hip b/vanerf_amd/csrc/weights_update.hip
--- a/vanerf_amd/csrc/weights_update.hip
+++ b/vanerf_amd/csrc/weights_update.hip
@@ -36,6 +36,22 @@
     if (L.b && threadIdx.x == 0) eff[L.eff + (size_t)L.nout * L.kin + o] = L.b[o];
 }
 
+struct FoldProduct { unsigned a, b, dst; int kin_a, a0, n, nc, nout; };
+__global__ __launch_bounds__(256) void fold_products_kernel(FoldProduct p0, FoldProduct p1, float* __restrict__ eff)
+{
+    unsigned idx = blockIdx.x * 256u + threadIdx.x;
+    const unsigned n0 = (unsigned)(p0.nout * p0.nc);
+    const FoldProduct p = idx < n0 ? p0 : p1;
+    if (idx >= n0) idx -= n0;
+    if (idx >= (unsigned)(p.nout * p.nc)) return;
+    const int o = (int)idx / p.nc, c = (int)idx % p.nc;
+    const float* a = eff + p.a + (size_t)o * p.kin_a + p.a0;
+    const float* b = eff + p.b + c;
+    float acc = 0.0f;
+    for (int k = 0; k < p.n; ++k) acc = fmaf(a[k], b[(size_t)k * p.nc], acc);
+    eff[p.dst + idx] = acc;
+}
+
 __global__ void place_f32_kernel(const int* __restrict__ tab, const float* __restrict__ eff, float* __restrict__ out, unsigned n)
 {
     const unsigned i = blockIdx.x * blockDim.x + threadIdx.x;
@@ -71,6 +87,8 @@
     int* bwd = nullptr;
     int* fwd_b = nullptr;
     int* fwd_bh = nullptr;
+    int* fwd_bl = nullptr;
+    int* bias = nullptr;
 };
 const DeviceTables& device_tables(int device)
 {
@@ -90,6 +108,8 @@
         t.bwd = upload(p.bwd);
         t.fwd_b = upload(p.fwd_b);
         t.fwd_bh = upload(p.fwd_bh);
+        t.fwd_bl = upload(p.fwd_bl);
+        t.bias = upload(p.bias);
         t.fwd = upload(p.fwd);
     }
     return t;
@@ -106,7 +126,7 @@
         if (device != h->device) throw_error("vanerf_weights_update: handle packed on device %d, current device %d", h->device, device);
         const PackTables& p = pack_tables();
         if (h->n_floats != (h->mode ? p.fwd_b.size() / 2 : p.fwd.size()) || (h->dev_bwd && h->n_floats_bwd != p.bwd.size()) ||
-            h->n_floats_h != (h->mode ? p.fwd_bh.size() / 2 : 0))
+            h->n_floats_h != (h->mode ? p.fwd_bh.size() / 2 : 0) || h->n_floats_l != (h->mode ? p.fwd_bl.size() / 2 : 0))
             throw_error("internal: handle and placement tables disagree on the stream sizes");
         FoldArgs a;
         layer_sources(*dev, a.l);
@@ -121,6 +141,15 @@
             const unsigned nh = (unsigned)h->n_floats_h;
             hipLaunchKernelGGL(place_b_kernel, dim3((nh + 255) / 256), dim3(256), 0, s, reinterpret_cast<const int2*>(t.fwd_bh), h->dev_eff,
                                reinterpret_cast<unsigned*>(h->dev + h->n_floats), nh);
+            const unsigned f0 = eff_fold_offset(), f1 = f0 + FOLD0_ROWS * FOLD0_COLS;
+            const FoldProduct p0{a.l[L_MLP0].eff, a.l[L_GEO_ATED0_B].eff, f0, a.l[L_MLP0].kin, 294, (int)FOLD0_COLS, (int)FOLD0_COLS, (int)FOLD0_ROWS};
+            const FoldProduct p1{a.l[L_MLP2].eff, a.l[L_GEO_ATED1_B].eff, f1, a.l[L_MLP2].kin, 128, (int)FOLD1_COLS, (int)FOLD1_COLS, (int)FOLD1_ROWS};
+            hipLaunchKernelGGL(fold_products_kernel, dim3((FOLD_FLOATS + 255u) / 256u), dim3(256), 0, s, p0, p1, h->dev_eff);
+            const unsigned nl = (unsigned)h->n_floats_l;
+            float* lean = h->dev + h->n_floats + h->n_floats_h;
+            hipLaunchKernelGGL(place_b_kernel, dim3((nl + 255) / 256), dim3(256), 0, s, reinterpret_cast<const int2*>(t.fwd_bl), h->dev_eff,
+                               reinterpret_cast<unsigned*>(lean), nl);
+            hipLaunchKernelGGL(place_f32_kernel, dim3((BIAS_TABLE_FLOATS + 255u) / 256u), dim3(256), 0, s, t.bias, h->dev_eff, lean + nl, BIAS_TABLE_FLOATS);
         } else
             hipLaunchKernelGGL(place_f32_kernel, dim3((n + 255) / 256), dim3(256), 0, s, t.fwd, h->dev_eff, h->dev, n);
         if (h->dev_bwd) {
diff --git a/vanerf_amd/renderer.py b/vanerf_amd/renderer.py
--- a/vanerf_amd/renderer.py
+++ b/vanerf_amd/renderer.py
@@ -156,6 +156,25 @@
     out = torch.empty(n.value, dtype=torch.float32)
     check(lib.vanerf_weights_download(weights.handle, which, c_void_p(out.data_ptr()), n.value, byref(n)))
     return out.view(torch.int32)
+
+
+LEAN_BIAS_TABLE, LEAN_FOLDED = 5, 6
+
+
+def bias_table(weights_or_sd):
+    if isinstance(weights_or_sd, PackedWeights):
+        return stream_device(weights_or_sd, LEAN_BIAS_TABLE).view(torch.float32)
+    return stream_host(weights_or_sd, LEAN_BIAS_TABLE).view(torch.float32)
+
+
+def folded_matrices(weights_or_sd):
+    get = stream_device if isinstance(weights_or_sd, PackedWeights) else stream_host
+    f = get(weights_or_sd, LEAN_FOLDED).view(torch.float32)
+    return f[:128 * 64].view(128, 64), f[128 * 64:].view(120, 8)
+
+
+def lean_stream_enabled():
+    return os.environ.get("VANERF_LEAN_STREAM", "1") != "0"
 
 
 def pack_weights_host(sd):
```

New measurement: 12.56 million rays/s, median of 6. +4.0%, better.
